# jinhojsk515/spmm

Measured on AMD Instinct MI355X. Metric: pretrain molecules/sec, higher is better.
Workload: dtype bf16; 1 GPU; SPMM pretrain step, text 12 layers (fusion at 6) + PV 6 layers, H=768, 12 heads, queue 36864, train mode (dropout 0.1), fwd+bwd+clip+AdamW+EMA; global_batch=128, seq_len=128, parallelism=dp1, schedule=eager launches on three HIP streams, packed text rows

## Files before the change

### include/spmm_hip.h

```cpp
#ifndef SPMM_HIP_H
#define SPMM_HIP_H

#include <stdint.h>

#ifdef __HIPCC__
#include <hip/hip_runtime.h>
typedef hipStream_t spmm_stream_t;
#else
typedef void* spmm_stream_t;
#endif

#ifdef __cplusplus
extern "C" {
#endif

int spmm_version(void);
const char* spmm_last_error(void);

#define SPMM_EPI_BF16 0
#define SPMM_EPI_GELU 1
#define SPMM_EPI_F32 2
#define SPMM_EPI_F32_ATOMIC 3
#define SPMM_EPI_GELU_GRAD 4
#define SPMM_EPI_F32_ACC 5
#define SPMM_EPI_GELU_DERIV 6
#define SPMM_EPI_MUL 7

#define SPMM_GEMM_AUTO 0
#define SPMM_GEMM_K128 1
#define SPMM_GEMM_K256x128 2
#define SPMM_GEMM_K256 3
#define SPMM_GEMM_K128PC 5
#define SPMM_GEMM_K256P8 8
#define SPMM_GEMM_K256P8_TILES 9
#define SPMM_GEMM_AUTO_TILES 16
int spmm_gemm_nt(const void* A, long lda, const void* W, long ldw, int M, int N, int K, int splits, const float* bias,
                 const float* div_ptr, float alpha, const void* R, long ldr, const void* G, long ldg, void* C, long ldc,
                 void* C2, long ldc2, int epi, float* colsum, int kernel, const int* M_dev, spmm_stream_t stream);
long spmm_gemm_tn_workspace_bytes(int M, int N, int K, int splits);
int spmm_gemm_tn_splits(int M, int N, int K, int kernel);
int spmm_gemm_tn(const void* A, long lda, const void* B, long ldb, int M, int N, int K, int splits, float alpha, float* C,
                 long ldc, float* workspace, int kernel, const int* M_dev, spmm_stream_t stream);
int spmm_gemm_tn_reduce(const float* ws, int ns, int N, int K, float* C, long ldc, spmm_stream_t stream);
int spmm_colsum_bf16(const void* x, long ld, int R, int C, float* out, const int* R_dev, spmm_stream_t stream);

int spmm_attn_fwd(const void* Q, long ldq, const void* K, long ldk, const void* V, long ldv, const int* kmask,
                  const int* kv_seq, const int* q_row0, const int* q_len, const int* kv_row0, const int* kv_len, void* O,
                  long ldo, float* LSE, int nseq, int nH, int Lq, int Lkv, int causal_from, int is_cross, float dropout_p,
                  const uint64_t* seed_ptr, uint64_t seed_salt, int q_off, int kv_off, spmm_stream_t stream);
int spmm_attn_bwd(const void* Q, long ldq, const void* K, long ldk, const void* V, long ldv, const int* kmask,
                  const int* kv_seq, const int* q_row0, const int* q_len, const int* kv_row0, const int* kv_len,
                  const void* O, long ldo, const float* LSE, const void* dO, long lddo, void* dQ,
                  long lddq, void* dK, long lddk, void* dV, long lddv, int nseq, int nH, int Lq, int Lkv, int causal_from,
                  int is_cross, float dropout_p, const uint64_t* seed_ptr, uint64_t seed_salt, int q_off, int kv_off, int d_mode,
                  float* Dbuf, spmm_stream_t stream);

int spmm_xattn_supported(int H, int nH, int Lq, int Lkv);
int spmm_xattn_pack_wo(const void* W, long ldw, void* out, int H, spmm_stream_t stream);
int spmm_xattn_fwd(const void* Q, long ldq, const void* K, long ldk, const void* V, long ldv, const int* kmask,
                   const int* kv_seq, const int* q_row0, const int* q_len, const int* kv_row0, const int* kv_len,
                   const void* WoF, const float* bo, const void* R, long ldr, const float* gamma, const float* beta, float eps,
                   void* Y, long ldy, void* Z, long ldz, float* mean, float* rstd, void* CTX, long ldc, float* LSE,
                   int nseq, int nH, int Lq, int Lkv, float attn_dropout_p, uint64_t salt_a, float hidden_dropout_p,
                   uint64_t salt_h, const uint64_t* seed_ptr, long row_base, spmm_stream_t stream);
int spmm_segment_sum_bf16(const void* src, const int* start, const int* list, void* out, int U, long W, spmm_stream_t stream);

int spmm_ln_fwd(const void* x, const void* res, const float* gamma, const float* beta, void* y, void* zout, float* mean,
                float* rstd, long rows, int H, float eps, float dropout_p, const uint64_t* seed_ptr, uint64_t salt,
                const int* rows_dev, spmm_stream_t stream);
int spmm_ln_fwd_r32(const void* x, const float* res32, const float* gamma, const float* beta, void* y, float* y32, void* zout,
                    float* mean, float* rstd, long rows, int H, float eps, float dropout_p, const uint64_t* seed_ptr,
                    uint64_t salt, spmm_stream_t stream);
int spmm_ln_bwd(const void* dy, const void* dy2, const void* z, const float* mean, const float* rstd, const float* gamma,
                void* dz, void* dx, float* dgamma, float* dbeta, long rows, int H, float dropout_p,
                const uint64_t* seed_ptr, uint64_t salt, int drop_on_dy, float* dxsum, const int* rows_dev,
                const float* beta_from_y, spmm_stream_t stream);

int spmm_embed_step_ln_fwd(const int* ids, int pos_index, const int* pos_ptr, const float* word, const float* pos, const float* type0,
                           const float* gamma, const float* beta, void* y, long rows, int H, float eps, spmm_stream_t stream);

int spmm_decode_attn(const void* q, long ldq, const void* K, const void* V, long seq_stride, long tok_stride, long head_stride, const int* anc,
                     int anc_ld, int kv_div, int group, void* out, long ldo, int R, int nH, int Lkv, float scale,
                     const int* t_ptr, const void* knew, const void* vnew, long ldn, const int* rowmap, spmm_stream_t stream);

int spmm_decode_xattn(const void* q, long ldq, const void* K, const void* V, long ldkv, const int* kv_seq, const int* kv_row0,
                      const int* kv_len, int group, void* out, long ldo, int R, int nH, int Lkv_max, float scale, spmm_stream_t stream);

int spmm_beam_step(const float* logits, long ldl, int N, int k, int V, int Lmax, int F, int t, const int* t_ptr, int t_off,
                   int* tokens, float* cur_p, float* fin_p, int* fin_len, int* fin_tok, int* fin_n, unsigned char* done,
                   int* anc, int anc_ld, int* ids_out, int* parent_out, int* n_done, const int* mol, const int* rowmap,
                   spmm_stream_t stream);

int spmm_beam_step_until(const float* logits, long ldl, int N, int k, int V, int Lmax, int F, int t, const int* t_ptr, int t_off,
                         int* tokens, float* cur_p, float* fin_p, int* fin_len, int* fin_tok, int* fin_n, unsigned char* done,
                         int* anc, int anc_ld, int* ids_out, int* parent_out, int* n_done, const int* mol, const int* rowmap,
                         int need, spmm_stream_t stream);

int spmm_beam_step_sampled(const float* logits, long ldl, int N, int k, int V, int Lmax, int F, int t, const int* t_ptr, int t_off,
                           int* tokens, float* cur_p, float* fin_p, int* fin_len, int* fin_tok, int* fin_n, unsigned char* done,
                           int* anc, int anc_ld, int* ids_out, int* parent_out, int* n_done, const int* mol, const int* rowmap,
                           const float* noise, long ldn, spmm_stream_t stream);

int spmm_gumbel_noise(const uint64_t* seed_ptr, uint64_t salt, int N, int k, int V, int Lmax, int t, const int* t_ptr, int t_off,
                      const int* mol, long mol_base, float* out, long ldo, spmm_stream_t stream);

int spmm_logit_warp(const float* lc, const float* lu, long ld, int R, int V, float w, float temperature, int top_k, float top_p,
                    int min_keep, float* out, long ldo, spmm_stream_t stream);

#define SPMM_SYNTAX_MASKED (-1e30f)
int spmm_smiles_mask(float* logits, float* logits2, long ld, int R, int V, const int* tokens, long tok_ld, int hist_rows, int k,
                     const int* mol, int Lmax, int t, const int* t_ptr, int t_off, int t_last, const int* table, int* state_out,
                     spmm_stream_t stream);

int spmm_kv_prefill(const void* K, const void* V, long ld, long src_rows, const int* row0, const int* len, const int* dst_row, int E,
                    void* Kc, void* Vc, int R, int nH, int Lmax, spmm_stream_t stream);

int spmm_embed_ln_fwd(int mode, const int* ids, const float* word, const float* pos, const float* type0, const float* pv_x,
                      const float* pv_mask, const float* pv_w, const float* pv_b, const float* pv_cls,
                      const float* pv_masktok, int src_mod, const float* gamma, const float* beta, void* y, void* zout,
                      float* mean, float* rstd, long nseq, int L, int H, float eps, float dropout_p,
                      const uint64_t* seed_ptr, uint64_t salt, spmm_stream_t stream);
int spmm_embed_bwd(int mode, const void* dz, const int* ids, const float* pv_x, const float* pv_mask, int src_mod,
                   float* dword, float* dpos, float* dtype0, float* d_w, float* d_b, float* d_cls, float* d_masktok,
                   long nseq, int L, int H, spmm_stream_t stream);

int spmm_transpose_bf16(const void* in, long ldi, void* out, long ldo, int R, int C, int Rpad, float* colsum,
                        spmm_stream_t stream);
int spmm_cast_transpose(const float* in, void* out, void* outT, int R, int C, spmm_stream_t stream);
long spmm_cast_transpose_desc_bytes(void);
int spmm_cast_transpose_multi(const void* descs_dev, int ndesc, int total_tiles, spmm_stream_t stream);
int spmm_cast_f32_bf16(const float* in, void* out, long n, spmm_stream_t stream);
int spmm_cast_bf16_f32(const void* in, float* out, long n, spmm_stream_t stream);
int spmm_acc_rows(float* dst, long ldd, const void* src, long lds, const long* idx, long rows, int H, int atomic,
                  spmm_stream_t stream);
int spmm_gather_rows(void* dst, const void* src, const long* idx, long rows, int H, spmm_stream_t stream);

int spmm_gather_rows2(void* dst, const void* srcA, const void* srcB, const long* idx, long rows, int H, spmm_stream_t stream);
int spmm_add_rows_bf16(void* dst, const long* idx, const void* src, long rows, int H, spmm_stream_t stream);
int spmm_zero_bytes(void* p, long nbytes, spmm_stream_t stream);
int spmm_zero_rows(void* p, long rows, long row_bytes, long stride_bytes, spmm_stream_t stream);
int spmm_gelu_bwd(const void* dz, const void* pre, void* out, long n, spmm_stream_t stream);
int spmm_pack_plan(const int* mask, int B, int Lt, int M, int* lens32, int* row0_32, long* row0_64, long* rows, long* gidx2,
                   long* gidx4, long* inv, long* idx_m, int* bad, spmm_stream_t stream);
int spmm_fusion_plan(const long* neg, const int* lens32, const int* row0_32, int B, int Lt, int Lp, int M,
                     long* idx6, long* neg_rows, long* idx_top, int* small32, spmm_stream_t stream);

int spmm_l2norm_fwd(const float* x, long ldx, float* y, float* nrm, void* a3, void* w3, void* yT, long ldt, int rows, int E,
                    spmm_stream_t stream);
int spmm_l2norm_bwd(const float* dy, const float* y, const float* nrm, const float* gscale, void* dx, int rows, int E,
                    spmm_stream_t stream);
int spmm_ita_rows(const float* S, const float* SM, long ldj, int nrows, int B, int J, const float* alpha_ptr,
                  const float* temp_ptr, void* dS, long ldd, int Jpad, float* losses, int loss_slot, float* dtemp,
                  int* nan_flag, spmm_stream_t stream);
int spmm_sample_neg(const float* S, long ldj, int B, const long* forced, const uint64_t* seed_ptr, uint64_t salt, long* out,
                    long out_offset, spmm_stream_t stream);
int spmm_lm_loss(const float* logits, const float* logits_m, long ldl, const int* ids, long nseq, int L, int V,
                 const float* alpha_ptr, int* n_nonpad_ws, const float* gscale, void* dlogits, long ldd, int Vpad,
                 float* losses, int loss_slot, spmm_stream_t stream);
int spmm_s2s_loss(const float* logits, long ldl, const int* ids, const long* row_of, long rows, long nseq, int L, int V,
                  int* n_label_ws, const float* gscale, void* dlogits, long ldd, int Vpad, float* losses, int loss_slot,
                  spmm_stream_t stream);
int spmm_lm_score(const void* y, long ldy, const void* Wd, long ldw, const float* bias, const int* ids, const long* row_of, long rows,
                  long nseq, int L, int V, int H, const int* seq_row0, const int* seq_len, float* tok_lp, float* seq_lp, int* seq_n,
                  spmm_stream_t stream);
int spmm_itm_head(const void* xa, long stride_a, const void* xb, long stride_b, int H, const float* W, const float* bias,
                  int n, int B, const float* gscale, float* losses, int loss_slot, float* logits_out, void* dxa, void* dxb,
                  float* dW, float* db, int do_bwd, int x_is_f32, spmm_stream_t stream);
int spmm_task_head(const void* A, long lda, int B, int W, const float* W2, const float* b2, int C, int kind, const void* target,
                   const float* gscale, float* logits, float* loss, void* dA, long ldda, float* dW2, float* db2, int do_bwd,
                   spmm_stream_t stream);
int spmm_s2p_append(const void* y, long ldy, const float* w3, const float* b3, const float* pe_w, const float* pe_b, const float* pos,
                    const float* type0, const float* gamma, const float* beta, float eps, float* pred, long ldp, void* xcache,
                    long rows, int H, int n_props, int i, spmm_stream_t stream);
int spmm_mpm_head(const void* h, int Lp, int H, const float* w, const float* bias, const float* target, const float* mask,
                  int B, int* n_keep_ws, const float* gscale, float* losses, int loss_slot, float* pred_out, void* dh,
                  float* dw, float* db, int do_bwd, int x_is_f32, spmm_stream_t stream);
int spmm_rows_linear(const void* x, int x_is_bf16, long ldx, const float* W, const float* bias, float* out, long ldo, long rows,
                     int N, int K, int act, spmm_stream_t stream);
long spmm_sim_topk_workspace_bytes(int Q, long n, int k);
int spmm_sim_topk(const float* q, long ldq, const float* f, long ldf, long base, int Q, long n, int E, int k, float* scores, long* index,
                  int merge, const float* cut_scores, const long* cut_index, void* workspace, long workspace_bytes, spmm_stream_t stream);
int spmm_enqueue(const float* feats, int n, int E, float* queue, int Q, void* w3, void* qT, long ldt, int Bloc, long* ptr,
                 int advance, const int* skip_flag, spmm_stream_t stream);
int spmm_queue_shadow(const float* queue, int E, int Q, void* w3, void* qT, long ldt, int Bloc, spmm_stream_t stream);
int spmm_clamp_scalar(float* p, float lo, float hi, spmm_stream_t stream);

long spmm_adam_scalars_bytes(void);
long spmm_grad_sqnorm_workspace_bytes(void);
int spmm_grad_sqnorm(const float* g, long n, float* out_zeroed, float* workspace, spmm_stream_t stream);
int spmm_adamw_step(float* p, const float* g, float* m, float* v, void* bf16_shadow, long n, const float* lr_ptr,
                    float beta1, float beta2, float eps, float weight_decay, const float* normsq, float max_norm, int* step,
                    const int* nan_flag, void* scalars_ws, spmm_stream_t stream);
int spmm_ema_update(float* pm, const float* p, void* bf16_shadow, long n, float momentum, spmm_stream_t stream);
int spmm_axpy_scalar(float* dst, const float* src, const float* scale_ptr, float scale, int n, spmm_stream_t stream);

#ifdef __cplusplus
}
#endif
#endif
```

### spmm_amd/csrc/gemm.hip

```cpp
#include "common.h"
#include "../../include/spmm_hip.h"

namespace {

constexpr int BM = 128, BN = 128, BK = 64;
constexpr int TILE_BYTES = BM * BK * 2;
constexpr int STAGE_BYTES = 2 * TILE_BYTES;

enum Epi { EPI_BF16 = 0, EPI_GELU = 1, EPI_F32 = 2, EPI_F32_ATOMIC = 3, EPI_GELU_GRAD = 4, EPI_F32_ACC = 5, EPI_GELU_DERIV = 6, EPI_MUL = 7 };
constexpr bool epi_is_bf16(int e) { return e == EPI_BF16 || e == EPI_GELU || e == EPI_GELU_GRAD || e == EPI_GELU_DERIV || e == EPI_MUL; }

struct GemmP {
  const bf16* A; long lda;
  const bf16* W; long ldw;
  int M, N, K;
  int ksplit;
  const float* bias;
  const float* div_ptr;
  float alpha;
  const bf16* R; long ldr;
  const bf16* G; long ldg;
  void* C; long ldc;
  bf16* C2; long ldc2;
  float* colsum;
  int order;
  const int* M_ptr;
};

#define GEMM_DYN_M(P)                                          \
  do {                                                         \
    if ((P).M_ptr) {                                           \
      const int m_ = *(P).M_ptr;                               \
      (P).M = m_ < (P).M ? (m_ > 0 ? m_ : 1) : (P).M;          \
    }                                                          \
  } while (0)

__device__ __forceinline__ void stage_tile_dma(const bf16* __restrict__ src, long ld, int row0, int nrows, int k0,
                                               char* lds_tile, int tid) {
#pragma unroll
  for (int c = 0; c < 4; ++c) {
    const int id = c * 256 + tid;
    const int row = id >> 3, ps = id & 7;
    const int ls = ps ^ ((row >> 1) & 7);
    int grow = row0 + row;
    grow = grow < nrows ? grow : nrows - 1;
    const bf16* g = src + (long)grow * ld + k0 + ls * 8;
    const int wave_base = __builtin_amdgcn_readfirstlane((c * 256 + (tid & ~63)) * 16);
    __builtin_amdgcn_global_load_lds((const GLOBAL_AS void*)g, (LDS_AS void*)(lds_tile + wave_base), 16, 0, 0);
  }
}

template <int EPI>
__device__ __forceinline__ void epi_convert(const GemmP& p, f32x16 (&acc)[2][2], char* t0, char* t1, int n_base, int lane) {
  float scale = p.alpha;
  if (p.div_ptr) scale /= *p.div_ptr;
#pragma unroll
  for (int ni = 0; ni < 2; ++ni)
#pragma unroll
    for (int mi = 0; mi < 2; ++mi) {
      const int row = mi * 32 + (lane & 31);
#pragma unroll
      for (int g = 0; g < 4; ++g) {
        const int col = ni * 32 + 8 * g + 4 * (lane >> 5);
        float v[4];
#pragma unroll
        for (int j = 0; j < 4; ++j) v[j] = acc[ni][mi][g * 4 + j] * scale;
        if (p.bias) {
          const int n = n_base + col;
          if (n < p.N) {
            const f32x4 b = *(const f32x4*)(p.bias + n);
#pragma unroll
            for (int j = 0; j < 4; ++j) v[j] += b[j];
          }
        }
        const int off = row * 128 + ((((col >> 3) ^ (row & 7)) << 4) | ((col & 4) << 1));
        if constexpr (EPI == EPI_GELU) {
          if (p.C2) *(bf16x4*)(t1 + off) = to_bf16x4(v[0], v[1], v[2], v[3]);
          *(bf16x4*)(t0 + off) = to_bf16x4(gelu_erf(v[0]), gelu_erf(v[1]), gelu_erf(v[2]), gelu_erf(v[3]));
        } else if constexpr (EPI == EPI_GELU_DERIV) {
          float gv[4], dv[4];
#pragma unroll
          for (int j = 0; j < 4; ++j) gelu_erf_both(v[j], gv[j], dv[j]);
          if (p.C2) *(bf16x4*)(t1 + off) = to_bf16x4(dv[0], dv[1], dv[2], dv[3]);
          *(bf16x4*)(t0 + off) = to_bf16x4(gv[0], gv[1], gv[2], gv[3]);
        } else {
          *(bf16x4*)(t0 + off) = to_bf16x4(v[0], v[1], v[2], v[3]);
        }
      }
    }
}

template <int EPI>
__device__ __forceinline__ void epi_store(const GemmP& p, const char* t0, const char* t1, int m_base, int n_base, int lane,
                                          float* cs_carry = nullptr, bool flush = true) {
  bf16x8 rr[8], gg[8];
  if (p.R || EPI == EPI_GELU_GRAD || EPI == EPI_MUL) {
#pragma unroll
    for (int it = 0; it < 8; ++it) {
      const int row = it * 8 + (lane >> 3), c16 = lane & 7;
      const int m = m_base + row, n = n_base + c16 * 8;
#pragma unroll
      for (int e = 0; e < 8; ++e) { rr[it][e] = (bf16)0.f; gg[it][e] = (bf16)0.f; }
      if (m >= p.M || n >= p.N) continue;
      const bool full = n + 8 <= p.N;
      if (p.R) {
        if (full) rr[it] = *(const bf16x8*)(p.R + (long)m * p.ldr + n);
        else { const bf16x4 h4 = *(const bf16x4*)(p.R + (long)m * p.ldr + n); rr[it][0] = h4[0]; rr[it][1] = h4[1]; rr[it][2] = h4[2]; rr[it][3] = h4[3]; }
      }
      if constexpr (EPI == EPI_GELU_GRAD || EPI == EPI_MUL) {
        if (full) gg[it] = *(const bf16x8*)(p.G + (long)m * p.ldg + n);
// ... 65 lines not shown

template <int EPI>
__device__ __forceinline__ void epilogue_bf16(const GemmP& p, f32x16 (&acc)[2][2], char* wtile, int m_base, int n_base, int lane,
                                              float* cs_carry = nullptr, bool flush = true) {
  epi_convert<EPI>(p, acc, wtile, wtile + 8192, n_base, lane);
  epi_store<EPI>(p, wtile, wtile + 8192, m_base, n_base, lane, cs_carry, flush);
}

template <int EPI>
__device__ __forceinline__ void tile128_out(const GemmP& p, f32x16 (&acc)[2][2], char* smem, int wave, int m0, int n0, int wm, int wn, int lane) {
  if constexpr (epi_is_bf16(EPI)) {
    epilogue_bf16<EPI>(p, acc, smem + wave * 16384, m0 + wm * 64, n0 + wn * 64, lane);
    return;
  }
  float scale = p.alpha;
  if (p.div_ptr) scale /= *p.div_ptr;
#pragma unroll
  for (int ni = 0; ni < 2; ++ni)
#pragma unroll
    for (int mi = 0; mi < 2; ++mi) {
      const int m = m0 + wm * 64 + mi * 32 + (lane & 31);
      if (m >= p.M) continue;
#pragma unroll
      for (int g = 0; g < 4; ++g) {
        const int n = n0 + wn * 64 + ni * 32 + 8 * g + 4 * (lane >> 5);
        if (n >= p.N) continue;
        float v[4];
#pragma unroll
        for (int j = 0; j < 4; ++j) v[j] = acc[ni][mi][g * 4 + j] * scale;
        if (p.bias && (EPI != EPI_F32_ATOMIC || blockIdx.z == 0)) {
          const f32x4 b = *(const f32x4*)(p.bias + n);
#pragma unroll
          for (int j = 0; j < 4; ++j) v[j] += b[j];
        }
        if (p.R && (EPI != EPI_F32_ATOMIC || blockIdx.z == 0)) {
          const bf16x4 r = *(const bf16x4*)(p.R + (long)m * p.ldr + n);
#pragma unroll
          for (int j = 0; j < 4; ++j) v[j] += (float)r[j];
        }
        if constexpr (EPI == EPI_BF16) {
          *(bf16x4*)((bf16*)p.C + (long)m * p.ldc + n) = to_bf16x4(v[0], v[1], v[2], v[3]);
        } else if constexpr (EPI == EPI_GELU) {
          *(bf16x4*)(p.C2 + (long)m * p.ldc2 + n) = to_bf16x4(v[0], v[1], v[2], v[3]);
          *(bf16x4*)((bf16*)p.C + (long)m * p.ldc + n) =
              to_bf16x4(gelu_erf(v[0]), gelu_erf(v[1]), gelu_erf(v[2]), gelu_erf(v[3]));
        } else if constexpr (EPI == EPI_GELU_GRAD) {
          const bf16x4 x = *(const bf16x4*)(p.G + (long)m * p.ldg + n);
          *(bf16x4*)((bf16*)p.C + (long)m * p.ldc + n) =
              to_bf16x4(v[0] * gelu_erf_grad((float)x[0]), v[1] * gelu_erf_grad((float)x[1]),
                        v[2] * gelu_erf_grad((float)x[2]), v[3] * gelu_erf_grad((float)x[3]));
        } else if constexpr (EPI == EPI_F32) {
          f32x4 o = {v[0], v[1], v[2], v[3]};
          *(f32x4*)((float*)p.C + (long)m * p.ldc + n) = o;
        } else if constexpr (EPI == EPI_F32_ACC) {
          f32x4* dst = (f32x4*)((float*)p.C + (long)m * p.ldc + n);
          f32x4 o = *dst;
          o[0] += v[0]; o[1] += v[1]; o[2] += v[2]; o[3] += v[3];
          *dst = o;
        } else {
          float* dst = (float*)p.C + (long)m * p.ldc + n;
#pragma unroll
          for (int j = 0; j < 4; ++j) atomicAdd(dst + j, v[j]);
        }
      }
    }
}

template <int EPI>
__global__ __launch_bounds__(256) void gemm_nt_kernel(GemmP p) {
  __shared__ __attribute__((aligned(16))) char smem[2 * STAGE_BYTES];
  const int tid = threadIdx.x, lane = tid & 63, wave = tid >> 6;
  const int wm = wave >> 1, wn = wave & 1;

  GEMM_DYN_M(p);
  const int ntm = (p.M + BM - 1) / BM, ntn = (p.N + BN - 1) / BN, nt = ntm * ntn;
  int t;
  {
    const int b = blockIdx.x, q = nt >> 3, r = nt & 7, xcd = b & 7, i = b >> 3;
    if (i >= (xcd < r ? q + 1 : q)) return;
    t = (xcd < r ? xcd * (q + 1) : r * (q + 1) + (xcd - r) * q) + i;
  }
  const int tile_m = t / ntn, tile_n = t % ntn;
  const int m0 = tile_m * BM, n0 = tile_n * BN;
  const int kbeg = blockIdx.z * p.ksplit;
  const int kend = min(p.K, kbeg + p.ksplit);
  const int nk = (kend - kbeg) / BK;

  f32x16 acc[2][2];
#pragma unroll
  for (int i = 0; i < 2; ++i)
#pragma unroll
    for (int j = 0; j < 2; ++j)
#pragma unroll
      for (int r = 0; r < 16; ++r) acc[i][j][r] = 0.f;

  if (nk > 0) {
    stage_tile_dma(p.A, p.lda, m0, p.M, kbeg, smem, tid);
    stage_tile_dma(p.W, p.ldw, n0, p.N, kbeg, smem + TILE_BYTES, tid);
  }
  for (int kt = 0; kt < nk; ++kt) {
    __syncthreads();
    char* cur = smem + (kt & 1) * STAGE_BYTES;
    char* nxt = smem + ((kt + 1) & 1) * STAGE_BYTES;
    if (kt + 1 < nk) {
      stage_tile_dma(p.A, p.lda, m0, p.M, kbeg + (kt + 1) * BK, nxt, tid);
      stage_tile_dma(p.W, p.ldw, n0, p.N, kbeg + (kt + 1) * BK, nxt + TILE_BYTES, tid);
    }
    const char* As = cur;
    const char* Ws = cur + TILE_BYTES;
#pragma unroll
    for (int kk = 0; kk < 4; ++kk) {
      const int s = kk * 2 + (lane >> 5);
      bf16x8 af[2], wf[2];
#pragma unroll
      for (int i = 0; i < 2; ++i) {
        const int ar = wm * 64 + i * 32 + (lane & 31);
        af[i] = *(const bf16x8*)(As + ar * 128 + ((s ^ ((ar >> 1) & 7)) << 4));
        const int wr = wn * 64 + i * 32 + (lane & 31);
        wf[i] = *(const bf16x8*)(Ws + wr * 128 + ((s ^ ((wr >> 1) & 7)) << 4));
      }
#pragma unroll
      for (int ni = 0; ni < 2; ++ni)
#pragma unroll
        for (int mi = 0; mi < 2; ++mi)
          acc[ni][mi] = __builtin_amdgcn_mfma_f32_32x32x16_bf16(wf[ni], af[mi], acc[ni][mi], 0, 0, 0);
    }
  }

  if constexpr (epi_is_bf16(EPI)) __syncthreads();
  tile128_out<EPI>(p, acc, smem, wave, m0, n0, wm, wn, lane);
}

#ifndef PC_AUTO
#define PC_AUTO 1
#endif
constexpr int PC_STAGES = 4;
constexpr int PC_LDS = PC_STAGES * STAGE_BYTES;
#ifndef PC_LOADERS
#define PC_LOADERS 4
#endif
constexpr int PC_LT = PC_LOADERS * 64;
constexpr int PC_NC = 1024 / PC_LT;
constexpr int PC_THREADS = 256 + PC_LT;

template <int EPI>
__global__ __launch_bounds__(PC_THREADS) void gemm_nt_pc_kernel(GemmP p) {
  extern __shared__ __attribute__((aligned(16))) char smem_pc[];
  const int tid = threadIdx.x, lane = tid & 63;
  const int wave = __builtin_amdgcn_readfirstlane(tid >> 6);
  GEMM_DYN_M(p);
  const int ntm = (p.M + BM - 1) / BM, ntn = (p.N + BN - 1) / BN, nt = ntm * ntn;
  int t;
  {
    const int b = blockIdx.x, q = nt >> 3, r = nt & 7, xcd = b & 7, i = b >> 3;
    if (i >= (xcd < r ? q + 1 : q)) return;
    t = (xcd < r ? xcd * (q + 1) : r * (q + 1) + (xcd - r) * q) + i;
  }
  const int tile_m = t / ntn, tile_n = t % ntn;
  const int m0 = tile_m * BM, n0 = tile_n * BN;
  const int kbeg = blockIdx.z * p.ksplit;
  const int kend = min(p.K, kbeg + p.ksplit);
  const int nk = (kend - kbeg) / BK;

  if (wave >= 4) {
    const int ltid = tid - 256;
    uint32_t offA[PC_NC], offW[PC_NC], dst[PC_NC];
#pragma unroll
    for (int c = 0; c < PC_NC; ++c) {
      const int id = c * PC_LT + ltid;
      const int row = id >> 3, ps = id & 7;
      const int ls = ps ^ ((row >> 1) & 7);
      int ga = m0 + row, gw = n0 + row;
      ga = ga < p.M ? ga : p.M - 1;
      gw = gw < p.N ? gw : p.N - 1;
      offA[c] = (uint32_t)ga * (uint32_t)(p.lda * 2) + (uint32_t)(ls * 16);
      offW[c] = (uint32_t)gw * (uint32_t)(p.ldw * 2) + (uint32_t)(ls * 16);
      dst[c] = (uint32_t)((c * PC_LT + (ltid & ~63)) * 16);
    }
    const uint32_t lds0 = (uint32_t)(uintptr_t)(LDS_AS char*)smem_pc;
    const char* gA = (const char*)p.A + (size_t)kbeg * 2;
    const char* gW = (const char*)p.W + (size_t)kbeg * 2;
#define PC_DMA(VOFF, SBASE, LDSDST)                                                                                          \
    asm volatile("s_mov_b32 m0, %2\n\ts_nop 0\n\tglobal_load_lds_dwordx4 %0, %1" ::"v"(VOFF), "s"(SBASE), "s"(LDSDST) : "memory", "m0")
#define PC_STAGE(KT)                                                                                                         \
    do {                                                                                                                     \
      const uint32_t st_ = lds0 + (uint32_t)(((KT) % PC_STAGES) * STAGE_BYTES);                                              \
      const char* a_ = gA + (size_t)(KT) * (BK * 2);                                                                         \
      const char* w_ = gW + (size_t)(KT) * (BK * 2);                                                                         \
      _Pragma("unroll") for (int c = 0; c < PC_NC; ++c) {                                                                    \
        const uint32_t d_ = __builtin_amdgcn_readfirstlane(st_ + dst[c]);                                                    \
        PC_DMA(offA[c], a_, d_);                                                                                             \
      }                                                                                                                      \
      _Pragma("unroll") for (int c = 0; c < PC_NC; ++c) {                                                                    \
        const uint32_t d_ = __builtin_amdgcn_readfirstlane(st_ + (uint32_t)TILE_BYTES + dst[c]);                             \
        PC_DMA(offW[c], w_, d_);                                                                                             \
      }                                                                                                                      \
    } while (0)
#define PC_WAIT(NEWER)                                                                                                       \
    do {                                                                                                                     \
      if ((NEWER) >= 3) asm volatile("s_waitcnt vmcnt(%0)" ::"n"(6 * PC_NC) : "memory");                                     \
      else if ((NEWER) == 2) asm volatile("s_waitcnt vmcnt(%0)" ::"n"(4 * PC_NC) : "memory");                                \
      else if ((NEWER) == 1) asm volatile("s_waitcnt vmcnt(%0)" ::"n"(2 * PC_NC) : "memory");                                \
      else asm volatile("s_waitcnt vmcnt(0)" ::: "memory");                                                                  \
    } while (0)
    constexpr int AHEAD = PC_STAGES - 1;
    const int pre = nk < AHEAD ? nk : AHEAD;
    for (int k = 0; k < pre; ++k) PC_STAGE(k);
    PC_WAIT(pre - 1);
    __builtin_amdgcn_s_barrier();
    for (int kt = 0; kt < nk; ++kt) {
      if (kt + AHEAD < nk) PC_STAGE(kt + AHEAD);
      const int last = kt + AHEAD < nk ? kt + AHEAD : nk - 1;
      PC_WAIT(last - (kt + 1));
      __builtin_amdgcn_s_barrier();
    }
#undef PC_DMA
#undef PC_STAGE
#undef PC_WAIT
    return;
  }

  const int wm = wave >> 1, wn = wave & 1;
  f32x16 acc[2][2];
#pragma unroll
  for (int i = 0; i < 2; ++i)
#pragma unroll
    for (int j = 0; j < 2; ++j)
#pragma unroll
      for (int r = 0; r < 16; ++r) acc[i][j][r] = 0.f;
  int aoff[2], woff[2];
#pragma unroll
  for (int i = 0; i < 2; ++i) {
    aoff[i] = (wm * 64 + i * 32 + (lane & 31)) * 128;
    woff[i] = TILE_BYTES + (wn * 64 + i * 32 + (lane & 31)) * 128;
  }
  const int sw0 = ((wm * 64 + (lane & 31)) >> 1) & 7, sw1 = ((wn * 64 + (lane & 31)) >> 1) & 7;
  const int hi = lane >> 5;
#define PC_FRAGS(KK, BUF)                                                                                          \
  do {                                                                                                             \
    const int sa_ = (((KK) * 2 + hi) ^ sw0) << 4, sw_ = (((KK) * 2 + hi) ^ sw1) << 4;                              \
    _Pragma("unroll") for (int i = 0; i < 2; ++i) {                                                                \
      af[BUF][i] = *(const bf16x8*)(st + aoff[i] + sa_);                                                           \
      wf[BUF][i] = *(const bf16x8*)(st + woff[i] + sw_);                                                           \
    }                                                                                                              \
  } while (0)
  __builtin_amdgcn_s_barrier();
  for (int kt = 0; kt < nk; ++kt) {
    const char* st = smem_pc + (kt % PC_STAGES) * STAGE_BYTES;
    bf16x8 af[2][2], wf[2][2];
    PC_FRAGS(0, 0);
#pragma unroll
    for (int kk = 0; kk < 4; ++kk) {
      if (kk < 3) PC_FRAGS(kk + 1, (kk + 1) & 1);
#pragma unroll
      for (int ni = 0; ni < 2; ++ni)
#pragma unroll
        for (int mi = 0; mi < 2; ++mi)
          acc[ni][mi] = __builtin_amdgcn_mfma_f32_32x32x16_bf16(wf[kk & 1][ni], af[kk & 1][mi], acc[ni][mi], 0, 0, 0);
    }
    __builtin_amdgcn_s_barrier();
  }
#undef PC_FRAGS
  tile128_out<EPI>(p, acc, smem_pc, wave, m0, n0, wm, wn, lane);
}

constexpr int BM2 = 256;
constexpr int A2_BYTES = BM2 * BK * 2;
constexpr int STAGE2_BYTES = A2_BYTES + TILE_BYTES;
constexpr int LDS2_BYTES = 3 * STAGE2_BYTES;

__device__ __forceinline__ void stage2_dma(const bf16* __restrict__ src, long ld, int row0, int nrows, int k0, char* lds_tile, int tid,
                                           int nchunks_per_thread) {
  for (int c = 0; c < nchunks_per_thread; ++c) {
    const int id = c * 512 + tid;
    const int row = id >> 3, ps = id & 7;
    const int ls = ps ^ ((row >> 1) & 7);
    int grow = row0 + row;
    grow = grow < nrows ? grow : nrows - 1;
    const bf16* g = src + (long)grow * ld + k0 + ls * 8;
    const int wave_base = __builtin_amdgcn_readfirstlane((c * 512 + (tid & ~63)) * 16);
    __builtin_amdgcn_global_load_lds((const GLOBAL_AS void*)g, (LDS_AS void*)(lds_tile + wave_base), 16, 0, 0);
  }
}

template <int EPI>
__global__ __launch_bounds__(512) void gemm_nt_v2_kernel(GemmP p) {
  extern __shared__ __attribute__((aligned(16))) char smem2[];
  const int tid = threadIdx.x, lane = tid & 63, wave = tid >> 6;
  const int wm = wave >> 1, wn = wave & 1;
  GEMM_DYN_M(p);
  const int ntm = (p.M + BM2 - 1) / BM2, ntn = (p.N + BN - 1) / BN, nt = ntm * ntn;
  int t;
  {
    const int b = blockIdx.x, q = nt >> 3, r = nt & 7, xcd = b & 7, i = b >> 3;
    if (i >= (xcd < r ? q + 1 : q)) return;
    t = (xcd < r ? xcd * (q + 1) : r * (q + 1) + (xcd - r) * q) + i;
  }
  const int tile_m = t / ntn, tile_n = t % ntn;
  const int m0 = tile_m * BM2, n0 = tile_n * BN;
  const int nk = p.K / BK;

  f32x16 acc[2][2];
#pragma unroll
  for (int i = 0; i < 2; ++i)
#pragma unroll
    for (int j = 0; j < 2; ++j)
#pragma unroll
      for (int r = 0; r < 16; ++r) acc[i][j][r] = 0.f;

#define STAGE2(kt_)                                                                           \
  do {                                                                                        \
    char* b_ = smem2 + ((kt_) % 3) * STAGE2_BYTES;                                            \
    stage2_dma(p.A, p.lda, m0, p.M, (kt_) * BK, b_, tid, 4);                                  \
    stage2_dma(p.W, p.ldw, n0, p.N, (kt_) * BK, b_ + A2_BYTES, tid, 2);                       \
  } while (0)

  STAGE2(0);
  if (nk > 1) STAGE2(1);
  for (int kt = 0; kt < nk; ++kt) {
    if (kt + 1 < nk) asm volatile("s_waitcnt vmcnt(6)" ::: "memory");
    else asm volatile("s_waitcnt vmcnt(0)" ::: "memory");
    __builtin_amdgcn_s_barrier();
    if (kt + 2 < nk) STAGE2(kt + 2);
    const char* As = smem2 + (kt % 3) * STAGE2_BYTES;
    const char* Ws = As + A2_BYTES;
    const int ar0 = wm * 64 + (lane & 31), wr0 = wn * 64 + (lane & 31);
#pragma unroll
    for (int kk = 0; kk < 4; ++kk) {
      const int s = kk * 2 + (lane >> 5);
      bf16x8 af[2], wf[2];
#pragma unroll
      for (int i = 0; i < 2; ++i) {
        const int ar = ar0 + i * 32, wr = wr0 + i * 32;
        af[i] = *(const bf16x8*)(As + ar * 128 + ((s ^ ((ar >> 1) & 7)) << 4));
        wf[i] = *(const bf16x8*)(Ws + wr * 128 + ((s ^ ((wr >> 1) & 7)) << 4));
      }
#pragma unroll
      for (int ni = 0; ni < 2; ++ni)
#pragma unroll
        for (int mi = 0; mi < 2; ++mi)
          acc[ni][mi] = __builtin_amdgcn_mfma_f32_32x32x16_bf16(wf[ni], af[mi], acc[ni][mi], 0, 0, 0);
    }
  }
#undef STAGE2

  if constexpr (epi_is_bf16(EPI)) {
    __builtin_amdgcn_s_barrier();
    epilogue_bf16<EPI>(p, acc, smem2 + wave * 16384, m0 + wm * 64, n0 + wn * 64, lane);
    return;
  }
  float scale = p.alpha;
  if (p.div_ptr) scale /= *p.div_ptr;
#pragma unroll
  for (int ni = 0; ni < 2; ++ni)
#pragma unroll
    for (int mi = 0; mi < 2; ++mi) {
      const int m = m0 + wm * 64 + mi * 32 + (lane & 31);
      if (m >= p.M) continue;
#pragma unroll
      for (int g = 0; g < 4; ++g) {
        const int n = n0 + wn * 64 + ni * 32 + 8 * g + 4 * (lane >> 5);
        if (n >= p.N) continue;
        float v[4];
#pragma unroll
        for (int j = 0; j < 4; ++j) v[j] = acc[ni][mi][g * 4 + j] * scale;
        if (p.bias) {
          const f32x4 b = *(const f32x4*)(p.bias + n);
#pragma unroll
          for (int j = 0; j < 4; ++j) v[j] += b[j];
        }
        if (p.R) {
          const bf16x4 r = *(const bf16x4*)(p.R + (long)m * p.ldr + n);
#pragma unroll
          for (int j = 0; j < 4; ++j) v[j] += (float)r[j];
        }
        if constexpr (EPI == EPI_BF16) {
          *(bf16x4*)((bf16*)p.C + (long)m * p.ldc + n) = to_bf16x4(v[0], v[1], v[2], v[3]);
        } else if constexpr (EPI == EPI_GELU) {
          *(bf16x4*)(p.C2 + (long)m * p.ldc2 + n) = to_bf16x4(v[0], v[1], v[2], v[3]);
          *(bf16x4*)((bf16*)p.C + (long)m * p.ldc + n) =
              to_bf16x4(gelu_erf(v[0]), gelu_erf(v[1]), gelu_erf(v[2]), gelu_erf(v[3]));
        } else if constexpr (EPI == EPI_GELU_GRAD) {
          const bf16x4 x = *(const bf16x4*)(p.G + (long)m * p.ldg + n);
          *(bf16x4*)((bf16*)p.C + (long)m * p.ldc + n) =
              to_bf16x4(v[0] * gelu_erf_grad((float)x[0]), v[1] * gelu_erf_grad((float)x[1]),
                        v[2] * gelu_erf_grad((float)x[2]), v[3] * gelu_erf_grad((float)x[3]));
        } else if constexpr (EPI == EPI_F32) {
          f32x4 o = {v[0], v[1], v[2], v[3]};
          *(f32x4*)((float*)p.C + (long)m * p.ldc + n) = o;
        } else {
          f32x4* dst = (f32x4*)((float*)p.C + (long)m * p.ldc + n);
          f32x4 o = *dst;
          o[0] += v[0]; o[1] += v[1]; o[2] += v[2]; o[3] += v[3];
          *dst = o;
        }
      }
    }
}

__device__ __forceinline__ void tile_of(int t, int ntm, int ntn, int order, int& tm, int& tn) {
  if (order == 1) { tn = t / ntm; tm = t - tn * ntm; return; }
  if (order == 2) {
    const int gn = (ntn % 4 == 0) ? 4 : (ntn % 3 == 0 ? 3 : (ntn % 2 == 0 ? 2 : 1));
    const int sr = t / (8 * ntn);
    const int rows = min(8, ntm - sr * 8);
    const int r = t - sr * 8 * ntn;
    const int nb = r / (rows * gn), rr = r - nb * rows * gn;
    tm = sr * 8 + rr % rows;
    tn = nb * gn + rr / rows;
    return;
  }
  if (order >= 3 && ntn >= 8) {
    const int ng = order == 3 ? 2 : 4, base = ntn / ng, rem = ntn - base * ng;
    int c0 = 0, u = t;
#pragma unroll
    for (int g = 0; g < 4; ++g) {
      if (g >= ng) break;
      const int cg = base + (g < rem ? 1 : 0), sz = ntm * cg;
      if (u < sz || g == ng - 1) { tm = u / cg; tn = c0 + (u - tm * cg); return; }
      u -= sz; c0 += cg;
    }
  }
  tm = t / ntn; tn = t - tm * ntn;
}

constexpr int BM3 = 256, BN3 = 256;
constexpr int T3_BYTES = 256 * BK * 2;
constexpr int STAGE3_BYTES = 2 * T3_BYTES;
constexpr int LDS3_BYTES = 2 * STAGE3_BYTES;

template <int EPI>
__global__ __launch_bounds__(512) void gemm_nt_v3_kernel(GemmP p) {
  extern __shared__ __attribute__((aligned(16))) char smem3[];
  const int tid = threadIdx.x, lane = tid & 63, wave = tid >> 6;
  const int wm = wave >> 2, wn = wave & 3;
  GEMM_DYN_M(p);
  const int ntm = (p.M + BM3 - 1) / BM3, ntn = (p.N + BN3 - 1) / BN3, nt = ntm * ntn;
  int t;
  {
    const int b = blockIdx.x, q = nt >> 3, r = nt & 7, xcd = b & 7, i = b >> 3;
    if (i >= (xcd < r ? q + 1 : q)) return;
    t = (xcd < r ? xcd * (q + 1) : r * (q + 1) + (xcd - r) * q) + i;
  }
  int tile_m, tile_n;
  tile_of(t, ntm, ntn, p.order, tile_m, tile_n);
  const int m0 = tile_m * BM3, n0 = tile_n * BN3;
  const int nk = p.K / BK;

  f32x16 acc[2][2][2];
#pragma unroll
  for (int h = 0; h < 2; ++h)
#pragma unroll
    for (int i = 0; i < 2; ++i)
#pragma unroll
      for (int j = 0; j < 2; ++j)
#pragma unroll
        for (int r = 0; r < 16; ++r) acc[h][i][j][r] = 0.f;

#define STAGE3(kt_)                                                                           \
  do {                                                                                        \
    char* b_ = smem3 + ((kt_) & 1) * STAGE3_BYTES;                                            \
    stage2_dma(p.A, p.lda, m0, p.M, (kt_) * BK, b_, tid, 4);                                  \
    stage2_dma(p.W, p.ldw, n0, p.N, (kt_) * BK, b_ + T3_BYTES, tid, 4);                       \
  } while (0)

  STAGE3(0);
  for (int kt = 0; kt < nk; ++kt) {
    __syncthreads();
    if (kt + 1 < nk) STAGE3(kt + 1);
    const char* As = smem3 + (kt & 1) * STAGE3_BYTES;
    const char* Ws = As + T3_BYTES;
#pragma unroll
    for (int kk = 0; kk < 4; ++kk) {
      const int s = kk * 2 + (lane >> 5);
      bf16x8 af[4], wf[2];
#pragma unroll
      for (int i = 0; i < 4; ++i) {
        const int ar = wm * 128 + i * 32 + (lane & 31);
        af[i] = *(const bf16x8*)(As + ar * 128 + ((s ^ ((ar >> 1) & 7)) << 4));
      }
#pragma unroll
      for (int i = 0; i < 2; ++i) {
        const int wr = wn * 64 + i * 32 + (lane & 31);
        wf[i] = *(const bf16x8*)(Ws + wr * 128 + ((s ^ ((wr >> 1) & 7)) << 4));
      }
#pragma unroll
      for (int h = 0; h < 2; ++h)
#pragma unroll
        for (int ni = 0; ni < 2; ++ni)
#pragma unroll
          for (int mi = 0; mi < 2; ++mi)
            acc[h][ni][mi] = __builtin_amdgcn_mfma_f32_32x32x16_bf16(wf[ni], af[h * 2 + mi], acc[h][ni][mi], 0, 0, 0);
    }
  }
#undef STAGE3
  __syncthreads();
  char* wt = smem3 + wave * 16384;
  float cs_carry[8] = {0.f, 0.f, 0.f, 0.f, 0.f, 0.f, 0.f, 0.f};
#pragma unroll
  for (int h = 0; h < 2; ++h)
    epilogue_bf16<EPI>(p, acc[h], wt, m0 + wm * 128 + h * 64, n0 + wn * 64, lane, cs_carry, h == 1);
}

constexpr int P8_HT = 128 * BK * 2;
constexpr int P8_BUF = 4 * P8_HT;
constexpr int P8_LDS = 2 * P8_BUF;
constexpr int P8_XLDS = 8 * 4096;

template <int OFF>
__device__ __forceinline__ void p8_dsr(bf16x8& d, uint32_t addr) {
  asm volatile("ds_read_b128 %0, %1 offset:%2" : "=v"(d) : "v"(addr), "n"(OFF) : "memory");
}

struct P8Out { uint32_t d[4]; };
__device__ __forceinline__ uint32_t p8_pack2(float a, float b) {
  typedef __bf16 bf16x2 __attribute__((ext_vector_type(2)));
  bf16x2 v; v[0] = (bf16)a; v[1] = (bf16)b;
  return __builtin_bit_cast(uint32_t, v);
}
__device__ __forceinline__ float p8_lo(uint32_t w) { return __builtin_bit_cast(float, w << 16); }
__device__ __forceinline__ float p8_hi(uint32_t w) { return __builtin_bit_cast(float, w & 0xffff0000u); }
typedef uint32_t u32x2 __attribute__((ext_vector_type(2)));
typedef uint32_t u32x4 __attribute__((ext_vector_type(4)));
template <int OFF>
__device__ __forceinline__ void p8_dsw64(uint32_t addr, uint32_t a, uint32_t b) {
  u32x2 v = {a, b};
  asm volatile("ds_write_b64 %0, %1 offset:%2" :: "v"(addr), "v"(v), "n"(OFF) : "memory");
}
template <int OFF>
// ... 121 lines not shown
        if (p.colsum) {
#pragma unroll
          for (int d = 0; d < 4; ++d) {
            if (ok1) { cs[2 * d] += p8_lo(o1[d]); cs[2 * d + 1] += p8_hi(o1[d]); }
            if (ok2) { cs[2 * d] += p8_lo(o2[d]); cs[2 * d + 1] += p8_hi(o2[d]); }
          }
        }
      }
#ifdef P8_NOSTORE
      if (p.M < 0) {
#endif
#ifdef P8_STORE_POLICY
      if (ok1) asm volatile("global_store_dwordx4 %0, %1, off " P8_STORE_POLICY :: "v"(cp + (long)blk * 16 * p.ldc), "v"(o1) : "memory");
      if (ok2) asm volatile("global_store_dwordx4 %0, %1, off " P8_STORE_POLICY :: "v"(cp + (long)blk * 16 * p.ldc + 8 * p.ldc), "v"(o2) : "memory");
#else
      if (ok1) *(u32x4*)(cp + (long)blk * 16 * p.ldc) = o1;
      if (ok2) *(u32x4*)(cp + (long)blk * 16 * p.ldc + 8 * p.ldc) = o2;
#endif
#ifdef P8_NOSTORE
      }
#endif
      hook(blk);
      if constexpr (HAS_EX && EPI == EPI_GELU_GRAD) {
        if (blk == 3) { P8_LOAD_EX(1); }
      } else if constexpr (HAS_EX) {
        if (h == 0) {
#pragma unroll
          for (int i_ = 2 * mi; i_ < 2 * mi + 2; ++i_) {
            long r_ = row0 + 64 + i_ * 8;
            if (!INTERIOR) r_ = r_ < p.M ? r_ : p.M - 1;
            P8_EX_LOAD1(i_, r_);
          }
        }
      }
    }
#undef P8_LOAD_EX
#undef P8_EX_LOAD1
  if constexpr (!GELU2) {
    if (p.colsum) {
#pragma unroll
      for (int e = 0; e < 8; ++e) {
        float t = cs[e];
        t += __shfl_xor(t, 8, 64);
        t += __shfl_xor(t, 16, 64);
        t += __shfl_xor(t, 32, 64);
        cs[e] = t;
      }
      if (lane < 8 && n_ok) {
#pragma unroll
        for (int e = 0; e < 8; ++e) atomicAdd(p.colsum + n + e, cs[e]);
      }
    }
  }
}

template <int EPI>
__global__ __launch_bounds__(512) void gemm_nt_p8_kernel(GemmP p) {
  extern __shared__ __attribute__((aligned(16))) char smem8[];
  const int tid = threadIdx.x, lane = tid & 63;
  const int wave = __builtin_amdgcn_readfirstlane(tid >> 6);
  const int wr = wave >> 2, wc = wave & 3;
  GEMM_DYN_M(p);
  const int ntm = (p.M + BM3 - 1) / BM3, ntn = (p.N + BN3 - 1) / BN3, nt = ntm * ntn;
  if ((int)blockIdx.x >= nt) return;
  const int nk = p.K / BK;

  f32x4 acc[2][4][4];
#define P8_ZERO()                                                              \
  _Pragma("unroll") for (int h_ = 0; h_ < 2; ++h_)                             \
  _Pragma("unroll") for (int i_ = 0; i_ < 4; ++i_)                             \
  _Pragma("unroll") for (int j_ = 0; j_ < 4; ++j_) acc[h_][i_][j_] = f32x4{0.f, 0.f, 0.f, 0.f}
  P8_ZERO();

  uint32_t offA[2][2], offW[2][2];
  const uint32_t ls16 = (uint32_t)(((tid & 7) ^ ((tid >> 4) & 7)) * 16);
  int m0, n0;
#define P8_TILE(VB)                                                                                           \
  do {                                                                                                        \
    const int b_ = (VB), q_ = nt >> 3, r_ = nt & 7, xcd_ = b_ & 7, i_ = b_ >> 3;                              \
    const int t_ = (xcd_ < r_ ? xcd_ * (q_ + 1) : r_ * (q_ + 1) + (xcd_ - r_) * q_) + i_;                     \
    int tm_, tn_;                                                                                             \
    tile_of(t_, ntm, ntn, p.order, tm_, tn_);                                                                 \
    m0 = tm_ * BM3; n0 = tn_ * BN3;                                                                           \
    _Pragma("unroll") for (int h_ = 0; h_ < 2; ++h_)                                                          \
    _Pragma("unroll") for (int j_ = 0; j_ < 2; ++j_) {                                                        \
      int row_ = m0 + j_ * 128 + h_ * 64 + (tid >> 3);                                                        \
      row_ = row_ < p.M ? row_ : p.M - 1;                     \
      offA[h_][j_] = (uint32_t)row_ * (uint32_t)(p.lda * 2) + ls16;                                                      \
      int col_ = n0 + (j_ * 2 + (tid >> 8)) * 64 + h_ * 32 + ((tid >> 3) & 31);                               \
      col_ = col_ < p.N ? col_ : p.N - 1;                                                                     \
      offW[h_][j_] = (uint32_t)col_ * (uint32_t)(p.ldw * 2) + ls16;                                                      \
    }                                                                                                         \
  } while (0)
  const char* gA = (const char*)p.A;
  const char* gW = (const char*)p.W;
  const uint32_t lds0 = (uint32_t)(uintptr_t)(LDS_AS char*)smem8;
#define P8_STG(GB, O, SLOT)                                                                                               \
  do {                                                                                                                    \
    const uint32_t d_ = lds0 + (SLOT) + wave * 1024;                                                                      \
    asm volatile("s_mov_b32 m0, %2\n\ts_nop 0\n\tglobal_load_lds_dwordx4 %0, %1" :: "v"((O)[0]), "s"(GB), "s"(d_) : "memory", "m0");          \
    asm volatile("s_mov_b32 m0, %2\n\ts_nop 0\n\tglobal_load_lds_dwordx4 %0, %1" :: "v"((O)[1]), "s"(GB), "s"(d_ + 8192) : "memory", "m0");   \
  } while (0)
#define P8_STG_A(H, BUF, KT) P8_STG((const char*)(gA + (size_t)(KT) * (BK * 2)), offA[H], (BUF) * P8_BUF + (H) * P8_HT)
#define P8_STG_W(H, BUF, KT) P8_STG((const char*)(gW + (size_t)(KT) * (BK * 2)), offW[H], (BUF) * P8_BUF + (2 + (H)) * P8_HT)
#define P8_PROLOGUE()                                                                        \
  do {                                                                                       \
    P8_STG_A(0, 0, 0); P8_STG_W(0, 0, 0); P8_STG_W(1, 0, 0); P8_STG_A(1, 0, 0);              \
    P8_STG_W(0, 1, 1); P8_STG_A(0, 1, 1); P8_STG_W(1, 1, 1);                                 \
  } while (0)

  uint32_t aad[2][2], wad[2][2];
  {
    const uint32_t sw = (uint32_t)((lane >> 1) & 7), r16 = (uint32_t)(lane & 15), q = (uint32_t)(lane >> 4);
#pragma unroll
    for (int kk = 0; kk < 2; ++kk) {
      const uint32_t slot = ((((uint32_t)kk * 4 + q) ^ sw) << 4);
      aad[0][kk] = lds0 + ((uint32_t)wr * 64 + r16) * 128 + slot;
      wad[0][kk] = lds0 + 2 * P8_HT + ((uint32_t)wc * 32 + r16) * 128 + slot;
      aad[1][kk] = aad[0][kk] + P8_BUF;
      wad[1][kk] = wad[0][kk] + P8_BUF;
    }
  }
  bf16x8 fa[4][2], fw0[2][2], fw1[2][2];
#define P8_RD_A(BUF, H)                                                                       \
  do {                                                                                        \
    p8_dsr<(H) * P8_HT + 0 * 2048>(fa[0][0], aad[BUF][0]);                                    \
    p8_dsr<(H) * P8_HT + 1 * 2048>(fa[1][0], aad[BUF][0]);                                    \
    p8_dsr<(H) * P8_HT + 2 * 2048>(fa[2][0], aad[BUF][0]);                                    \
    p8_dsr<(H) * P8_HT + 3 * 2048>(fa[3][0], aad[BUF][0]);                                    \
    p8_dsr<(H) * P8_HT + 0 * 2048>(fa[0][1], aad[BUF][1]);                                    \
    p8_dsr<(H) * P8_HT + 1 * 2048>(fa[1][1], aad[BUF][1]);                                    \
    p8_dsr<(H) * P8_HT + 2 * 2048>(fa[2][1], aad[BUF][1]);                                    \
    p8_dsr<(H) * P8_HT + 3 * 2048>(fa[3][1], aad[BUF][1]);                                    \
  } while (0)
#define P8_RD_W(BUF, H, FW)                                                                   \
  do {                                                                                        \
    p8_dsr<(H) * P8_HT + 0 * 2048>(FW[0][0], wad[BUF][0]);                                    \
    p8_dsr<(H) * P8_HT + 1 * 2048>(FW[1][0], wad[BUF][0]);                                    \
    p8_dsr<(H) * P8_HT + 0 * 2048>(FW[0][1], wad[BUF][1]);                                    \
    p8_dsr<(H) * P8_HT + 1 * 2048>(FW[1][1], wad[BUF][1]);                                    \
  } while (0)
#define P8_MM(H, NH, FW)                                                                                        \
  do {                                                                                                          \
    _Pragma("unroll") for (int kk_ = 0; kk_ < 2; ++kk_)                                                         \
    _Pragma("unroll") for (int mi_ = 0; mi_ < 4; ++mi_)                                                         \
    _Pragma("unroll") for (int ni_ = 0; ni_ < 2; ++ni_)                                                         \
      acc[H][mi_][(NH) * 2 + ni_] =                                                                             \
          __builtin_amdgcn_mfma_f32_16x16x32_bf16(FW[ni_][kk_], fa[mi_][kk_], acc[H][mi_][(NH) * 2 + ni_], 0, 0, 0); \
  } while (0)
#define P8_BAR() __builtin_amdgcn_s_barrier()
#define P8_SB() __builtin_amdgcn_sched_barrier(0)
#define P8_LGKM0() asm volatile("s_waitcnt lgkmcnt(0)" ::: "memory")
#define P8_COMPUTE(H, NH, FW)                    \
  do {                                           \
    P8_BAR();                                    \
    P8_LGKM0();                                  \
    P8_SB();                                     \
    __builtin_amdgcn_s_setprio(1);               \
    P8_MM(H, NH, FW);                            \
    __builtin_amdgcn_s_setprio(0);               \
    P8_SB();                                     \
    P8_BAR();                                    \
    P8_SB();                                     \
  } while (0)

#ifdef P8_PROFILE
  unsigned long long* prof = (unsigned long long*)p.colsum + (size_t)blockIdx.x * 16 * 8;
  p.colsum = nullptr;
  int prof_i = 0;
#define P8_STAMP(K) do { if (prof && tid == 0 && prof_i < 16) prof[prof_i * 8 + (K)] = __builtin_readcyclecounter(); } while (0)
#else
#define P8_STAMP(K) do { } while (0)
#endif
  int vb = blockIdx.x;
  bool pre = false;
  P8_TILE(vb);
  P8_PROLOGUE();
  asm volatile("s_waitcnt vmcnt(6)" ::: "memory");
  P8_BAR();
  P8_SB();
  if (wr == 1) P8_BAR();
  for (;;) {
    P8_STAMP(0);
    const int cm0 = m0, cn0 = n0;
    const int vbn = vb + (int)gridDim.x;
    const bool has_next = vbn < nt;
    const bool pre_next = has_next && cm0 + BM3 <= p.M && cn0 + BN3 <= p.N;
    for (int kt = 0; kt < nk; kt += 2) {
      const bool last = kt + 2 >= nk;
      const bool more = !last || has_next;
      int kn = kt + 2;
      P8_RD_W(0, 0, fw0); P8_SB(); P8_RD_A(0, 0);
      if (!(pre && kt == 0)) P8_STG_A(1, 1, kt + 1);
      asm volatile("s_waitcnt lgkmcnt(8)" ::: "memory");
      P8_COMPUTE(0, 0, fw0);
      if (last && has_next) { P8_TILE(vbn); kn = 0; }
      P8_RD_W(0, 1, fw1);
      if (more) P8_STG_W(0, 0, kn);
      P8_COMPUTE(0, 1, fw1);
      P8_RD_A(0, 1);
      if (more) P8_STG_A(0, 0, kn);
      P8_COMPUTE(1, 1, fw1);
      if (more) {
        P8_STG_W(1, 0, kn);
        if (pre && kt == 0) asm volatile("s_waitcnt vmcnt(22)" ::: "memory");
        else asm volatile("s_waitcnt vmcnt(6)" ::: "memory");
      } else {
        asm volatile("s_waitcnt vmcnt(0)" ::: "memory");
      }
      P8_COMPUTE(1, 0, fw0);
      P8_RD_W(1, 0, fw0); P8_SB(); P8_RD_A(1, 0);
      if (more) P8_STG_A(1, 0, kn);
      asm volatile("s_waitcnt lgkmcnt(8)" ::: "memory");
      P8_COMPUTE(0, 0, fw0);
      P8_RD_W(1, 1, fw1);
      if (more) P8_STG_W(0, 1, kn + 1);
      P8_COMPUTE(0, 1, fw1);
      P8_RD_A(1, 1);
      if (more) P8_STG_A(0, 1, kn + 1);
      P8_COMPUTE(1, 1, fw1);
      if (more) {
        P8_STG_W(1, 1, kn + 1);
        if (last && pre_next) {
          P8_STG_A(1, 1, kn + 1);
          asm volatile("s_waitcnt vmcnt(8)" ::: "memory");
        } else {
          asm volatile("s_waitcnt vmcnt(6)" ::: "memory");
        }
      }
      P8_COMPUTE(1, 0, fw0);
    }
    P8_STAMP(2);

    if (wr == 0) P8_BAR();
    P8_SB();
    {
      int lane_e = lane;
      asm volatile("" : "+v"(lane_e));
      GemmP q = p;
      asm volatile("" : "+s"(q.C), "+s"(q.ldc), "+s"(q.C2), "+s"(q.ldc2));
      asm volatile("" : "+s"(q.R), "+s"(q.ldr), "+s"(q.G), "+s"(q.ldg));
      asm volatile("" : "+s"(q.bias), "+s"(q.colsum), "+s"(q.div_ptr), "+s"(q.alpha), "+s"(q.M), "+s"(q.N));
      auto hook = [](int) {};
      const uint32_t xb = lds0 + P8_LDS + wave * 4096;
      const int mb = cm0 + wr * 128, nb = cn0 + wc * 64;
      const bool interior = cm0 + BM3 <= q.M && cn0 + BN3 <= q.N;
      if constexpr (EPI == EPI_GELU_GRAD || EPI == EPI_MUL) {
        if (interior) p8_epilogue_blocks<EPI, true, true>(q, acc, xb, mb, nb, lane_e, hook);
        else p8_epilogue_blocks<EPI, false, true>(q, acc, xb, mb, nb, lane_e, hook);
      } else if (EPI == EPI_BF16 && q.R != nullptr) {
        if (interior) p8_epilogue_blocks<EPI, true, true>(q, acc, xb, mb, nb, lane_e, hook);
        else p8_epilogue_blocks<EPI, false, true>(q, acc, xb, mb, nb, lane_e, hook);
      } else {
        if (interior) p8_epilogue_blocks<EPI, true, false>(q, acc, xb, mb, nb, lane_e, hook);
        else p8_epilogue_blocks<EPI, false, false>(q, acc, xb, mb, nb, lane_e, hook);
      }
    }
    P8_SB();
    if (wr == 1) P8_BAR();
    P8_STAMP(4);
#ifdef P8_PROFILE
    ++prof_i;
#endif
    if (!has_next) break;
    vb = vbn;
    pre = pre_next;
    P8_SB();
  }
  if (wr == 0) P8_BAR();
#undef P8_ZERO
#undef P8_STAMP
#undef P8_TILE
#undef P8_PROLOGUE
#undef P8_STG
#undef P8_STG_A
#undef P8_STG_W
#undef P8_RD_A
#undef P8_RD_W
#undef P8_MM
#undef P8_COMPUTE
#undef P8_BAR
#undef P8_SB
#undef P8_LGKM0
}

template <typename K>
int raise_lds(K kernel, int bytes, const char* what) {
  hipError_t e = hipFuncSetAttribute((const void*)kernel, hipFuncAttributeMaxDynamicSharedMemorySize, bytes);
  if (e != hipSuccess) {
    spmm_set_error("spmm_gemm_nt: cannot raise the dynamic LDS of %s to %d: %s", what, bytes, hipGetErrorString(e));
    return SPMM_ERR_LAUNCH;
  }
  return SPMM_OK;
}

template <int EPI>
int launch_p8_one(const GemmP& p, hipStream_t st, bool persist) {
  static const int rc = raise_lds(gemm_nt_p8_kernel<EPI>, P8_LDS + P8_XLDS, "the 8-phase kernel");
  if (rc != SPMM_OK) return rc;
  const int nt = ((p.M + BM3 - 1) / BM3) * ((p.N + BN3 - 1) / BN3);
  static const int ncu = [] { int dev = 0, n = 0; (void)hipGetDevice(&dev); (void)hipDeviceGetAttribute(&n, hipDeviceAttributeMultiprocessorCount, dev); return n > 0 ? n & ~7 : 256; }();
  dim3 grid(persist && nt > ncu ? ncu : nt);
  hipLaunchKernelGGL((gemm_nt_p8_kernel<EPI>), grid, dim3(512), P8_LDS + P8_XLDS, st, p);
  return SPMM_OK;
}
int launch_p8(int epi, const GemmP& p, hipStream_t st, bool persist) {
  switch (epi) {
    case EPI_BF16: return launch_p8_one<EPI_BF16>(p, st, persist);
    case EPI_GELU: return launch_p8_one<EPI_GELU>(p, st, persist);
    case EPI_GELU_GRAD: return launch_p8_one<EPI_GELU_GRAD>(p, st, persist);
    case EPI_GELU_DERIV: return launch_p8_one<EPI_GELU_DERIV>(p, st, persist);
    case EPI_MUL: return launch_p8_one<EPI_MUL>(p, st, persist);
    default: return -1;
  }
}

template <int EPI>
int launch_v3_one(const GemmP& p, hipStream_t st) {
  static const int rc = raise_lds(gemm_nt_v3_kernel<EPI>, LDS3_BYTES, "the 256x256 kernel");
  if (rc != SPMM_OK) return rc;
  dim3 grid(((p.M + BM3 - 1) / BM3) * ((p.N + BN3 - 1) / BN3));
  hipLaunchKernelGGL((gemm_nt_v3_kernel<EPI>), grid, dim3(512), LDS3_BYTES, st, p);
  return SPMM_OK;
}
int launch_v3(int epi, const GemmP& p, hipStream_t st) {
  switch (epi) {
    case EPI_BF16: return launch_v3_one<EPI_BF16>(p, st);
    case EPI_GELU: return launch_v3_one<EPI_GELU>(p, st);
    case EPI_GELU_GRAD: return launch_v3_one<EPI_GELU_GRAD>(p, st);
    case EPI_GELU_DERIV: return launch_v3_one<EPI_GELU_DERIV>(p, st);
    case EPI_MUL: return launch_v3_one<EPI_MUL>(p, st);
    default: return -1;
  }
}

template <int EPI>
int launch_v2_one(const GemmP& p, hipStream_t st) {
  static const int rc = raise_lds(gemm_nt_v2_kernel<EPI>, LDS2_BYTES, "the 256x128 kernel");
  if (rc != SPMM_OK) return rc;
  dim3 grid(((p.M + BM2 - 1) / BM2) * ((p.N + BN - 1) / BN));
  hipLaunchKernelGGL((gemm_nt_v2_kernel<EPI>), grid, dim3(512), LDS2_BYTES, st, p);
  return SPMM_OK;
}
int launch_v2(int epi, const GemmP& p, hipStream_t st) {
  switch (epi) {
    case EPI_BF16: return launch_v2_one<EPI_BF16>(p, st);
    case EPI_GELU: return launch_v2_one<EPI_GELU>(p, st);
    case EPI_F32: return launch_v2_one<EPI_F32>(p, st);
    case EPI_GELU_GRAD: return launch_v2_one<EPI_GELU_GRAD>(p, st);
    case EPI_GELU_DERIV: return launch_v2_one<EPI_GELU_DERIV>(p, st);
    case EPI_MUL: return launch_v2_one<EPI_MUL>(p, st);
    case EPI_F32_ACC: return launch_v2_one<EPI_F32_ACC>(p, st);
    default: return -1;
  }
}

template <typename K>
int pc_attr(K kernel) {
  static const hipError_t e = hipFuncSetAttribute((const void*)kernel, hipFuncAttributeMaxDynamicSharedMemorySize, PC_LDS);
  return e == hipSuccess ? 0 : 1;
}
#define PC_LAUNCH(E)                                                                                   \
  case E:                                                                                              \
    if (pc_attr(gemm_nt_pc_kernel<E>)) { spmm_set_error("spmm_gemm_nt: cannot raise the LDS limit of the loader/compute kernel"); return SPMM_ERR_LAUNCH; } \
    hipLaunchKernelGGL((gemm_nt_pc_kernel<E>), grid, dim3(PC_THREADS), PC_LDS, st, p);                        \
    break
int launch_pc(int epi, const GemmP& p, dim3 grid, hipStream_t st) {
  switch (epi) {
    PC_LAUNCH(EPI_BF16); PC_LAUNCH(EPI_GELU); PC_LAUNCH(EPI_F32); PC_LAUNCH(EPI_F32_ATOMIC); PC_LAUNCH(EPI_GELU_GRAD); PC_LAUNCH(EPI_F32_ACC);
    PC_LAUNCH(EPI_GELU_DERIV); PC_LAUNCH(EPI_MUL);
    default: return -1;
  }
  return 0;
}
#undef PC_LAUNCH

int launch_v1(int epi, const GemmP& p, dim3 grid, hipStream_t st) {
  switch (epi) {
    case EPI_BF16: hipLaunchKernelGGL((gemm_nt_kernel<EPI_BF16>), grid, dim3(256), 0, st, p); break;
    case EPI_GELU: hipLaunchKernelGGL((gemm_nt_kernel<EPI_GELU>), grid, dim3(256), 0, st, p); break;
    case EPI_F32: hipLaunchKernelGGL((gemm_nt_kernel<EPI_F32>), grid, dim3(256), 0, st, p); break;
    case EPI_F32_ATOMIC: hipLaunchKernelGGL((gemm_nt_kernel<EPI_F32_ATOMIC>), grid, dim3(256), 0, st, p); break;
    case EPI_GELU_GRAD: hipLaunchKernelGGL((gemm_nt_kernel<EPI_GELU_GRAD>), grid, dim3(256), 0, st, p); break;
    case EPI_F32_ACC: hipLaunchKernelGGL((gemm_nt_kernel<EPI_F32_ACC>), grid, dim3(256), 0, st, p); break;
    case EPI_GELU_DERIV: hipLaunchKernelGGL((gemm_nt_kernel<EPI_GELU_DERIV>), grid, dim3(256), 0, st, p); break;
    case EPI_MUL: hipLaunchKernelGGL((gemm_nt_kernel<EPI_MUL>), grid, dim3(256), 0, st, p); break;
    default: return -1;
  }
  return SPMM_OK;
}

inline bool is_bf16_epi(int epi) { return epi_is_bf16(epi); }
inline bool p8_ok(const GemmP& p, int epi) {
  return is_bf16_epi(epi) && p.K % 128 == 0 && p.N % 8 == 0 && (unsigned long)p.M * (unsigned long)p.lda * 2ul < (1ul << 32) &&
         (unsigned long)p.N * (unsigned long)p.ldw * 2ul < (1ul << 32);
}

int pick_tile(int M, int N, int epi) {
  const bool bf = is_bf16_epi(epi);
  if (M >= 6000) {
    const long t3 = (long)((M + 255) / 256) * ((N + 255) / 256);
    if (bf && t3 >= 96) return 3;
    return (epi != EPI_F32_ATOMIC) ? 2 : 1;
  }
  auto tiles = [&](int bm, int bn) { return (double)((M + bm - 1) / bm) * ((N + bn - 1) / bn); };
  auto fill = [](double t) { const double w = (double)(long)((t + 255) / 256); return t / (256.0 * w); };
  const double t3 = tiles(256, 256), t2 = tiles(256, 128), t1 = tiles(128, 128);
  const double s3 = bf ? 1.20 * fill(t3) : 0.0;
  const double s2 = (M >= 512 && epi != EPI_F32_ATOMIC) ? 0.85 * fill(t2) : 0.0;
  const double s1 = 0.80 * (t1 < 256 ? t1 / 256.0 : 1.0);
  if (s3 >= s2 && s3 >= s1) return 3;
  return s2 >= s1 ? 2 : 1;
}

}

extern "C" int spmm_gemm_nt(const void* A, long lda, const void* W, long ldw, int M, int N, int K, int splits,
                            const float* bias, const float* div_ptr, float alpha, const void* R, long ldr,
                            const void* G, long ldg, void* C, long ldc, void* C2, long ldc2, int epi, float* colsum,
                            int kernel, const int* M_dev, hipStream_t stream) {
  SPMM_CHECK_SHAPE(M > 0 && N > 0 && K > 0, "spmm_gemm_nt: empty problem M=%d N=%d K=%d", M, N, K);
  SPMM_CHECK_SHAPE(K % 64 == 0, "spmm_gemm_nt: K=%d must be a multiple of 64", K);
  SPMM_CHECK_SHAPE(N % 4 == 0, "spmm_gemm_nt: N=%d must be a multiple of 4", N);
  SPMM_CHECK_SHAPE(lda % 8 == 0 && ldw % 8 == 0, "spmm_gemm_nt: lda/ldw must be multiples of 8 elements");
  SPMM_CHECK_SHAPE(ldc % 4 == 0, "spmm_gemm_nt: ldc must be a multiple of 4");
  SPMM_CHECK_SHAPE(!is_bf16_epi(epi) || (ldc % 8 == 0 && (!R || ldr % 8 == 0) && (!G || ldg % 8 == 0) && (!C2 || ldc2 % 8 == 0) && (uintptr_t)C % 16 == 0),
                   "spmm_gemm_nt: bf16 outputs need 16-B aligned rows (ldc/ldr/ldg/ldc2 multiples of 8)");
  SPMM_CHECK_SHAPE(is_bf16_epi(epi) || !R || (ldr % 4 == 0 && (uintptr_t)R % 8 == 0),
                   "spmm_gemm_nt: R of an fp32-output epilogue is read 4 columns at a time (ldr a multiple of 4, R 8-B aligned)");
  SPMM_CHECK_SHAPE(((uintptr_t)A % 16 == 0) && ((uintptr_t)W % 16 == 0), "spmm_gemm_nt: A/W must be 16-B aligned");
  SPMM_CHECK_SHAPE(epi >= EPI_BF16 && epi <= EPI_MUL, "spmm_gemm_nt: unknown epilogue %d", epi);
  if (splits < 1) splits = 1;
  SPMM_CHECK_SHAPE(splits == 1 || epi == EPI_F32_ATOMIC, "spmm_gemm_nt: split-K needs the atomic epilogue");
  SPMM_CHECK_SHAPE((epi != EPI_GELU_GRAD && epi != EPI_MUL) || G != nullptr, "spmm_gemm_nt: the GELU-grad / multiply epilogues need G");
  SPMM_CHECK_SHAPE(colsum == nullptr || epi == EPI_BF16 || epi == EPI_GELU_GRAD || epi == EPI_MUL, "spmm_gemm_nt: colsum is only fused into the bf16 / GELU-grad / multiply epilogues");
  int ksplit = ((K / 64 + splits - 1) / splits) * 64;
  splits = (K + ksplit - 1) / ksplit;
  GemmP p;
  p.A = (const bf16*)A; p.lda = lda; p.W = (const bf16*)W; p.ldw = ldw;
  p.M = M; p.N = N; p.K = K; p.ksplit = ksplit; p.bias = bias; p.div_ptr = div_ptr; p.alpha = alpha;
  p.R = (const bf16*)R; p.ldr = ldr; p.G = (const bf16*)G; p.ldg = ldg; p.C = C; p.ldc = ldc;
  p.C2 = (bf16*)C2; p.ldc2 = ldc2; p.colsum = colsum;
  p.M_ptr = nullptr;
  p.order = K > 1024 ? 0 : 2;

  int k = kernel == SPMM_GEMM_AUTO_TILES ? 0 : kernel;
  if (k == 0) {
    const int tile = splits > 1 ? 1 : pick_tile(M, N, epi);
    k = tile == 3 ? (p8_ok(p, epi) ? (kernel == SPMM_GEMM_AUTO_TILES ? 9 : 8) : 3) : tile;
    if (k == 2 && (epi == EPI_F32_ATOMIC || M < 512)) k = 1;
  }
  const bool pc_fits = (unsigned long)p.M * (unsigned long)p.lda * 2ul < (1ul << 32) && (unsigned long)p.N * (unsigned long)p.ldw * 2ul < (1ul << 32);
  const long t128 = (long)((M + BM - 1) / BM) * ((N + BN - 1) / BN) * splits;
  if (k == 1 && kernel != 1 && pc_fits && PC_AUTO && t128 <= 256 && ksplit >= 4 * BK) k = 5;
  SPMM_CHECK_SHAPE(k == 1 || k == 2 || k == 3 || k == 5 || k == 8 || k == 9, "spmm_gemm_nt: unknown kernel selector %d", kernel);
  SPMM_CHECK_SHAPE(k != 5 || pc_fits, "spmm_gemm_nt: kernel 5 addresses its operands with 32-bit byte offsets (< 4 GiB each)");
  SPMM_CHECK_SHAPE((k != 8 && k != 9) || p8_ok(p, epi), "spmm_gemm_nt: the 8-phase kernel needs a bf16-output epilogue, K %% 128 == 0, N %% 8 == 0 and operands < 4 GiB");
  SPMM_CHECK_SHAPE(k != 3 || is_bf16_epi(epi), "spmm_gemm_nt: the 256x256 kernel has bf16-output epilogues only");
  SPMM_CHECK_SHAPE(k != 2 || epi != EPI_F32_ATOMIC, "spmm_gemm_nt: the 256x128 kernel has no atomic epilogue");
  SPMM_CHECK_SHAPE(k == 1 || k == 5 || splits == 1, "spmm_gemm_nt: split-K runs on the 128x128 kernels only");
  p.M_ptr = M_dev;
  int rc;
  if (k == 8 || k == 9) rc = launch_p8(epi, p, stream, k == 8);
  else if (k == 3) rc = launch_v3(epi, p, stream);
  else if (k == 2) rc = launch_v2(epi, p, stream);
  else if (k == 5) rc = launch_pc(epi, p, dim3(((M + BM - 1) / BM) * ((N + BN - 1) / BN), 1, splits), stream);
  else rc = launch_v1(epi, p, dim3(((M + BM - 1) / BM) * ((N + BN - 1) / BN), 1, splits), stream);
  if (rc > 0) return rc;
  if (rc < 0) { spmm_set_error("spmm_gemm_nt: epilogue %d is not built for kernel %d", epi, k); return SPMM_ERR_UNSUPPORTED; }
  SPMM_LAUNCH_CHECK("spmm_gemm_nt");
  return SPMM_OK;
}
```

### spmm_amd/csrc/rowops.hip

```cpp
#include "common.h"
#include <stdlib.h>
#include "../../include/spmm_hip.h"

namespace {

constexpr int MAXC = 4;

struct RowVec {
  float v[MAXC][4];
};

__device__ __forceinline__ void load_row_bf16(const bf16* __restrict__ p, int H, int lane, RowVec& r) {
#pragma unroll
  for (int i = 0; i < MAXC; ++i) {
    const int c = (lane + 64 * i) * 4;
    if (c < H) {
      const bf16x4 t = *(const bf16x4*)(p + c);
      r.v[i][0] = (float)t[0]; r.v[i][1] = (float)t[1]; r.v[i][2] = (float)t[2]; r.v[i][3] = (float)t[3];
    } else {
      r.v[i][0] = r.v[i][1] = r.v[i][2] = r.v[i][3] = 0.f;
    }
  }
}
__device__ __forceinline__ void store_row_bf16(bf16* __restrict__ p, int H, int lane, const RowVec& r) {
// ... 460 lines not shown
    float acc = 0.f, accw = 0.f, accb = 0.f, accm = 0.f;
    for (long s = s_beg; s < s_end; ++s) {
      const long row = s * p.L + l;
      const float g = (float)p.dz[row * p.H + c];
      acc += g;
      if (p.mode == 0) {
        const int id = p.ids[row];
        if (id != 0) atomicAdd(p.dword + (long)id * p.H + c, g);
      } else if (l > 0) {
        const long src = (s % p.src_mod) * (p.L - 1) + (l - 1);
        const float m = p.pv_mask[src];
        accw += g * (1.f - m) * p.pv_x[src];
        accb += g * (1.f - m);
        accm += g * m;
      }
    }
    atomicAdd(p.dpos + (long)l * p.H + c, acc);
    atomicAdd(p.dtype0 + c, acc);
    if (p.mode == 1) {
      if (l == 0) {
        atomicAdd(p.d_cls + c, acc);
      } else {
        atomicAdd(p.d_w + c, accw);
        atomicAdd(p.d_b + c, accb);
        atomicAdd(p.d_masktok + c, accm);
      }
    }
  }
}

__global__ __launch_bounds__(256) void transpose_bf16_kernel(const bf16* __restrict__ in, long ldi, bf16* __restrict__ out,
                                                             long ldo, int R, int C, int Rpad, float* __restrict__ colsum) {
  __shared__ bf16 tile[64][66];
  const int r0 = blockIdx.y * 64, c0 = blockIdx.x * 64;
  const int tx = threadIdx.x & 63, ty = threadIdx.x >> 6;
  float cs = 0.f;
#pragma unroll
  for (int i = 0; i < 16; ++i) {
    const int r = r0 + ty * 16 + i, c = c0 + tx;
    const bf16 v = (r < R && c < C) ? in[(long)r * ldi + c] : (bf16)0.f;
    tile[ty * 16 + i][tx] = v;
    cs += (float)v;
  }
  if (colsum) {
    __shared__ float part[4][64];
    part[ty][tx] = cs;
    __syncthreads();
    if (ty == 0 && c0 + tx < C) atomicAdd(colsum + c0 + tx, part[0][tx] + part[1][tx] + part[2][tx] + part[3][tx]);
  } else {
    __syncthreads();
  }
#pragma unroll
  for (int i = 0; i < 16; ++i) {
    const int c = c0 + ty * 16 + i, r = r0 + tx;
    if (c < C && r < Rpad) out[(long)c * ldo + r] = tile[tx][ty * 16 + i];
  }
}

__global__ __launch_bounds__(256) void cast_transpose_kernel(const float* __restrict__ in, bf16* __restrict__ out,
                                                             bf16* __restrict__ outT, int R, int C) {
  __shared__ bf16 tile[64][66];
  const int r0 = blockIdx.y * 64, c0 = blockIdx.x * 64;
  const int tx = threadIdx.x & 63, ty = threadIdx.x >> 6;
#pragma unroll
  for (int i = 0; i < 16; ++i) {
    const int r = r0 + ty * 16 + i, c = c0 + tx;
    bf16 v = (bf16)0.f;
    if (r < R && c < C) {
      v = (bf16)in[(long)r * C + c];
      if (out) out[(long)r * C + c] = v;
    }
    tile[ty * 16 + i][tx] = v;
  }
  __syncthreads();
  if (outT) {
#pragma unroll
    for (int i = 0; i < 16; ++i) {
      const int c = c0 + ty * 16 + i, r = r0 + tx;
      if (c < C && r < R) outT[(long)c * R + r] = tile[tx][ty * 16 + i];
    }
  }
}

struct CtDesc { const float* src; bf16* dstT; int R, C; int tile0, ntc; };
__global__ __launch_bounds__(256) void cast_transpose_multi_kernel(const CtDesc* __restrict__ descs, int ndesc) {
  __shared__ bf16 tile[64][66];
  int lo = 0, hi = ndesc - 1;
  while (lo < hi) {
    const int mid = (lo + hi + 1) >> 1;
    if (descs[mid].tile0 <= (int)blockIdx.x) lo = mid; else hi = mid - 1;
  }
  const CtDesc d = descs[lo];
  const int tt = blockIdx.x - d.tile0;
  const int r0 = (tt / d.ntc) * 64, c0 = (tt % d.ntc) * 64;
  const int tx = threadIdx.x & 63, ty = threadIdx.x >> 6;
#pragma unroll
  for (int i = 0; i < 16; ++i) {
    const int r = r0 + ty * 16 + i, c = c0 + tx;
    tile[ty * 16 + i][tx] = (r < d.R && c < d.C) ? (bf16)d.src[(long)r * d.C + c] : (bf16)0.f;
  }
  __syncthreads();
#pragma unroll
  for (int i = 0; i < 16; ++i) {
    const int c = c0 + ty * 16 + i, r = r0 + tx;
    if (c < d.C && r < d.R) d.dstT[(long)c * d.R + r] = tile[tx][ty * 16 + i];
  }
}

__global__ void cast_f32_bf16_kernel(const float* __restrict__ in, bf16* __restrict__ out, long n4) {
  for (long i = (long)blockIdx.x * blockDim.x + threadIdx.x; i < n4; i += (long)gridDim.x * blockDim.x) {
    const f32x4 v = *(const f32x4*)(in + i * 4);
    *(bf16x4*)(out + i * 4) = to_bf16x4(v[0], v[1], v[2], v[3]);
  }
}
__global__ void cast_bf16_f32_kernel(const bf16* __restrict__ in, float* __restrict__ out, long n4) {
  for (long i = (long)blockIdx.x * blockDim.x + threadIdx.x; i < n4; i += (long)gridDim.x * blockDim.x) {
    const bf16x4 v = *(const bf16x4*)(in + i * 4);
    f32x4 o = {(float)v[0], (float)v[1], (float)v[2], (float)v[3]};
    *(f32x4*)(out + i * 4) = o;
  }
}

__global__ void acc_rows_kernel(float* __restrict__ dst, long ldd, const bf16* __restrict__ src, long lds,
                                const long* __restrict__ idx, long rows, int H, int atomic) {
  const int h4 = H / 4;
  for (long i = (long)blockIdx.x * blockDim.x + threadIdx.x; i < rows * h4; i += (long)gridDim.x * blockDim.x) {
    const long r = i / h4;
    const int c = (int)(i - r * h4) * 4;
    const long dr = idx ? idx[r] : r;
    if (dr < 0) continue;
    const bf16x4 v = *(const bf16x4*)(src + r * lds + c);
    float* d = dst + dr * ldd + c;
    if (atomic) {
#pragma unroll
      for (int j = 0; j < 4; ++j) atomicAdd(d + j, (float)v[j]);
    } else {
      f32x4 o = *(f32x4*)d;
      o[0] += (float)v[0]; o[1] += (float)v[1]; o[2] += (float)v[2]; o[3] += (float)v[3];
      *(f32x4*)d = o;
    }
  }
}
__global__ void gather_rows_kernel(bf16* __restrict__ dst, const bf16* __restrict__ src, const long* __restrict__ idx,
                                   long rows, int H) {
  const int h8 = H / 8;
  for (long i = (long)blockIdx.x * blockDim.x + threadIdx.x; i < rows * h8; i += (long)gridDim.x * blockDim.x) {
    const long r = i / h8;
    const int c = (int)(i - r * h8) * 8;
    *(bf16x8*)(dst + r * H + c) = *(const bf16x8*)(src + idx[r] * H + c);
  }
}

int grid_for(long work, int block) {
  long g = (work + block - 1) / block;
  return (int)(g < 1 ? 1 : (g > 2048 ? 2048 : g));
}


}

extern "C" int spmm_ln_fwd(const void* x, const void* res, const float* gamma, const float* beta, void* y, void* zout,
                           float* mean, float* rstd, long rows, int H, float eps, float dropout_p,
                           const uint64_t* seed_ptr, uint64_t salt, const int* rows_dev, hipStream_t stream) {
  SPMM_CHECK_SHAPE(rows > 0 && H > 0 && H % 4 == 0 && H <= 1024, "spmm_ln_fwd: rows=%ld H=%d (need H%%4==0, H<=1024)", rows, H);
  SPMM_CHECK_SHAPE(dropout_p == 0.f || seed_ptr, "spmm_ln_fwd: dropout needs a device seed");
  SPMM_CHECK_SHAPE(x && gamma && beta && y, "spmm_ln_fwd: null x / gamma / beta / y");
  SPMM_CHECK_SHAPE((mean == nullptr) == (rstd == nullptr), "spmm_ln_fwd: mean and rstd come together");
  const uint32_t th = (uint32_t)(dropout_p * 65536.f + 0.5f);
  const float ds = 1.f / (1.f - dropout_p);
#define LN_FWD16(NC)                                                                                                          \
  hipLaunchKernelGGL(ln_fwd16_kernel<NC>, dim3((rows + 7) / 8), dim3(256), 0, stream, (const bf16*)x, (const bf16*)res, gamma, \
                     beta, (bf16*)y, (bf16*)zout, mean, rstd, rows, eps, th, ds, seed_ptr, salt, rows_dev)
  if (H == 768) LN_FWD16(3);
  else if (H == 1024) LN_FWD16(4);
  else if (H == 512) LN_FWD16(2);
  else if (H == 256) LN_FWD16(1);
  else
    hipLaunchKernelGGL(ln_fwd_kernel, dim3((rows + 3) / 4), dim3(256), 0, stream, (const bf16*)x, (const bf16*)res, gamma, beta,
                       (bf16*)y, (bf16*)zout, mean, rstd, rows, H, eps, th, ds, seed_ptr, salt, rows_dev);
#undef LN_FWD16
  SPMM_LAUNCH_CHECK("spmm_ln_fwd");
  return SPMM_OK;
}

extern "C" int spmm_ln_fwd_r32(const void* x, const float* res32, const float* gamma, const float* beta, void* y, float* y32, void* zout,
                               float* mean, float* rstd, long rows, int H, float eps, float dropout_p, const uint64_t* seed_ptr,
                               uint64_t salt, hipStream_t stream) {
  SPMM_CHECK_SHAPE(rows > 0 && H > 0 && H % 4 == 0 && H <= 1024, "spmm_ln_fwd_r32: rows=%ld H=%d (need H%%4==0, H<=1024)", rows, H);
  SPMM_CHECK_SHAPE(dropout_p == 0.f || seed_ptr, "spmm_ln_fwd_r32: dropout needs a device seed");
  SPMM_CHECK_SHAPE((mean == nullptr) == (rstd == nullptr), "spmm_ln_fwd_r32: mean and rstd come together");
  hipLaunchKernelGGL(ln_fwd_r32_kernel, dim3((rows + 3) / 4), dim3(256), 0, stream, (const bf16*)x, res32, gamma, beta, (bf16*)y, y32,
                     (bf16*)zout, mean, rstd, rows, H, eps, (uint32_t)(dropout_p * 65536.f + 0.5f), 1.f / (1.f - dropout_p), seed_ptr, salt);
  SPMM_LAUNCH_CHECK("spmm_ln_fwd_r32");
  return SPMM_OK;
}

extern "C" int spmm_ln_bwd(const void* dy, const void* dy2, const void* z, const float* mean, const float* rstd,
                           const float* gamma, void* dz, void* dx, float* dgamma, float* dbeta, long rows, int H,
                           float dropout_p, const uint64_t* seed_ptr, uint64_t salt, int drop_on_dy, float* dxsum, const int* rows_dev,
                           const float* beta_from_y, hipStream_t stream) {
  SPMM_CHECK_SHAPE(rows > 0 && H > 0 && H % 4 == 0 && H <= 1024, "spmm_ln_bwd: rows=%ld H=%d", rows, H);
  SPMM_CHECK_SHAPE(beta_from_y != nullptr || mean != nullptr, "spmm_ln_bwd: the row means are required unless `z` holds the LayerNorm output (beta_from_y)");
  SPMM_CHECK_SHAPE(beta_from_y == nullptr || !drop_on_dy, "spmm_ln_bwd: the output of a LayerNorm followed by dropout does not determine the normalised values");
  SPMM_CHECK_SHAPE(dropout_p == 0.f || seed_ptr, "spmm_ln_bwd: dropout needs a device seed");
  SPMM_CHECK_SHAPE(dy && z && rstd && gamma && dz, "spmm_ln_bwd: null dy / z / rstd / gamma / dz");
  long g = (rows + 3) / 4;
  static const long genv = getenv("SPMM_LN_BWD_GRID") ? atol(getenv("SPMM_LN_BWD_GRID")) : 0;
  long gmax = genv > 0 ? genv : rows / 64;
  if (genv <= 0) gmax = gmax < 256 ? 256 : (gmax > 512 ? 512 : gmax);
  if (g > gmax) g = gmax;
  const uint32_t th = (uint32_t)(dropout_p * 65536.f + 0.5f);
  const float ds = 1.f / (1.f - dropout_p);
  const bool hot = !dy2 && dx && dgamma && dbeta && dxsum && th && !drop_on_dy;
#define LN_BWD_LAUNCH(NC, EX, HOT, FY)                                                                                                \
  hipLaunchKernelGGL((ln_bwd_kernel<NC, EX, HOT, FY>), dim3(g), dim3(256), 0, stream, (const bf16*)dy, (const bf16*)dy2, (const bf16*)z, \
                     mean, rstd, gamma, beta_from_y, (bf16*)dz, (bf16*)dx, dgamma, dbeta, rows, H, th, ds, seed_ptr, salt, drop_on_dy, dxsum, rows_dev)
  if (beta_from_y != nullptr) {
    if (H == 768 && hot) LN_BWD_LAUNCH(3, true, true, true);
    else if (H <= 768) LN_BWD_LAUNCH(3, false, false, true);
    else LN_BWD_LAUNCH(4, false, false, true);
  } else {
    if (H == 768 && hot) LN_BWD_LAUNCH(3, true, true, false);
    else if (H <= 768) LN_BWD_LAUNCH(3, false, false, false);
    else LN_BWD_LAUNCH(4, false, false, false);
  }
#undef LN_BWD_LAUNCH
  SPMM_LAUNCH_CHECK("spmm_ln_bwd");
  return SPMM_OK;
}

extern "C" int spmm_embed_ln_fwd(int mode, const int* ids, const float* word, const float* pos, const float* type0,
                                 const float* pv_x, const float* pv_mask, const float* pv_w, const float* pv_b,
                                 const float* pv_cls, const float* pv_masktok, int src_mod, const float* gamma,
                                 const float* beta, void* y, void* zout, float* mean, float* rstd, long nseq, int L, int H,
                                 float eps, float dropout_p, const uint64_t* seed_ptr, uint64_t salt, hipStream_t stream) {
  SPMM_CHECK_SHAPE(nseq > 0 && L > 0 && H > 0 && H % 4 == 0 && H <= 1024, "spmm_embed_ln_fwd: nseq=%ld L=%d H=%d (need 0 < H <= 1024, H%%4==0)", nseq, L, H);
  SPMM_CHECK_SHAPE(mode >= 0 && mode <= 2, "spmm_embed_ln_fwd: unknown mode %d", mode);
  SPMM_CHECK_SHAPE(pos && type0 && gamma && beta && y, "spmm_embed_ln_fwd: null pos / type0 / gamma / beta / y");
  SPMM_CHECK_SHAPE((mean == nullptr) == (rstd == nullptr), "spmm_embed_ln_fwd: mean and rstd come together");
  SPMM_CHECK_SHAPE(mode == 0 ? (ids && word) : mode == 2 ? (pv_x != nullptr) : (pv_x && pv_mask && pv_w && pv_b && pv_cls && pv_masktok && src_mod > 0),
                   "spmm_embed_ln_fwd: missing inputs for mode %d", mode);
  SPMM_CHECK_SHAPE(dropout_p == 0.f || seed_ptr, "spmm_embed_ln_fwd: dropout needs a device seed");
  EmbedP p = {};
  p.ids = ids; p.word = word; p.pos = pos; p.type0 = type0; p.pv_x = pv_x; p.pv_mask = pv_mask; p.pv_w = pv_w; p.pv_b = pv_b;
  p.pv_cls = pv_cls; p.pv_masktok = pv_masktok; p.src_mod = src_mod; p.gamma = gamma; p.beta = beta; p.y = (bf16*)y;
  p.zout = (bf16*)zout; p.mean_o = mean; p.rstd_o = rstd; p.nseq = nseq; p.L = L; p.H = H; p.mode = mode; p.eps = eps;
  p.thresh16 = (uint32_t)(dropout_p * 65536.f + 0.5f); p.dscale = 1.f / (1.f - dropout_p); p.seed_ptr = seed_ptr; p.salt = salt;
  hipLaunchKernelGGL(embed_ln_fwd_kernel, dim3((nseq * L + 3) / 4), dim3(256), 0, stream, p);
  SPMM_LAUNCH_CHECK("spmm_embed_ln_fwd");
  return SPMM_OK;
}

extern "C" int spmm_embed_step_ln_fwd(const int* ids, int pos_index, const int* pos_ptr, const float* word, const float* pos, const float* type0,
                                      const float* gamma, const float* beta, void* y, long rows, int H, float eps,
                                      hipStream_t stream) {
  SPMM_CHECK_SHAPE(rows > 0 && pos_index >= 0 && H % 4 == 0 && H <= 1024, "spmm_embed_step_ln_fwd: rows=%ld pos=%d H=%d", rows, pos_index, H);
  SPMM_CHECK_SHAPE(ids && word && pos && type0 && gamma && beta && y, "spmm_embed_step_ln_fwd: null argument");
  EmbedP p = {};
  p.ids = ids; p.word = word; p.pos = pos; p.type0 = type0; p.gamma = gamma; p.beta = beta; p.y = (bf16*)y;
  p.nseq = rows; p.L = 1; p.H = H; p.mode = 0; p.eps = eps; p.pos0 = pos_index; p.pos_ptr = pos_ptr; p.dscale = 1.f;
  hipLaunchKernelGGL(embed_ln_fwd_kernel, dim3((rows + 3) / 4), dim3(256), 0, stream, p);
  SPMM_LAUNCH_CHECK("spmm_embed_step_ln_fwd");
  return SPMM_OK;
}

extern "C" int spmm_embed_bwd(int mode, const void* dz, const int* ids, const float* pv_x, const float* pv_mask, int src_mod,
                              float* dword, float* dpos, float* dtype0, float* d_w, float* d_b, float* d_cls,
                              float* d_masktok, long nseq, int L, int H, hipStream_t stream) {
  SPMM_CHECK_SHAPE(nseq > 0 && L > 0 && H > 0, "spmm_embed_bwd: nseq=%ld L=%d H=%d", nseq, L, H);
  SPMM_CHECK_SHAPE(mode == 0 || mode == 1, "spmm_embed_bwd: mode %d (0 = text, 1 = PV; inputs_embeds has no backward)", mode);
  SPMM_CHECK_SHAPE(dz && dpos && dtype0, "spmm_embed_bwd: null dz / dpos / dtype0");
  SPMM_CHECK_SHAPE(mode != 0 || (ids && dword), "spmm_embed_bwd: mode 0 needs ids and dword");
  SPMM_CHECK_SHAPE(mode != 1 || (pv_x && pv_mask && d_w && d_b && d_cls && d_masktok), "spmm_embed_bwd: mode 1 needs pv_x, pv_mask, d_w, d_b, d_cls and d_masktok");
  SPMM_CHECK_SHAPE(mode != 1 || src_mod > 0, "spmm_embed_bwd: mode 1 needs src_mod > 0, got src_mod=%d", src_mod);
  EmbedBwdP p = {(const bf16*)dz, ids, pv_x, pv_mask, src_mod, dword, dpos, dtype0, d_w, d_b, d_cls, d_masktok, nseq, L, H, mode};
  hipLaunchKernelGGL(embed_bwd_kernel, dim3(L, nseq >= 32 ? 16 : 1), dim3(256), 0, stream, p);
  SPMM_LAUNCH_CHECK("spmm_embed_bwd");
  return SPMM_OK;
}

namespace {
__global__ __launch_bounds__(256) void segment_sum_kernel(const bf16* __restrict__ src, const int* __restrict__ start,
                                                          const int* __restrict__ list, bf16* __restrict__ out, long W) {
  const int u = blockIdx.y;
  const long c = ((long)blockIdx.x * 256 + threadIdx.x) * 8;
  if (c >= W) return;
  const int k0 = start[u], k1 = start[u + 1];
  float acc[8] = {0.f, 0.f, 0.f, 0.f, 0.f, 0.f, 0.f, 0.f};
  for (int k = k0; k < k1; ++k) {
    const bf16x8 v = *(const bf16x8*)(src + (long)list[k] * W + c);
#pragma unroll
    for (int e = 0; e < 8; ++e) acc[e] += (float)v[e];
  }
  bf16x8 o;
#pragma unroll
  for (int e = 0; e < 8; ++e) o[e] = (bf16)acc[e];
  *(bf16x8*)(out + (long)u * W + c) = o;
}
}

extern "C" int spmm_segment_sum_bf16(const void* src, const int* start, const int* list, void* out, int U, long W, hipStream_t stream) {
  SPMM_CHECK_SHAPE(U > 0 && U <= 65535 && W > 0 && W % 8 == 0, "spmm_segment_sum_bf16: U=%d W=%ld (W %% 8 == 0)", U, W);
  SPMM_CHECK_SHAPE(src && start && list && out, "spmm_segment_sum_bf16: null src / start / list / out");
  hipLaunchKernelGGL(segment_sum_kernel, dim3((unsigned)((W / 8 + 255) / 256), U), dim3(256), 0, stream, (const bf16*)src, start, list,
                     (bf16*)out, W);
  SPMM_LAUNCH_CHECK("spmm_segment_sum_bf16");
  return SPMM_OK;
}

extern "C" int spmm_transpose_bf16(const void* in, long ldi, void* out, long ldo, int R, int C, int Rpad, float* colsum,
                                   hipStream_t stream) {
  SPMM_CHECK_SHAPE(R > 0 && C > 0 && Rpad >= R && ldo >= Rpad, "spmm_transpose_bf16: R=%d C=%d Rpad=%d ldo=%ld", R, C, Rpad, ldo);
  SPMM_CHECK_SHAPE(ldi >= C, "spmm_transpose_bf16: ldi=%ld is shorter than a row of C=%d", ldi, C);
  SPMM_CHECK_SHAPE(in && out, "spmm_transpose_bf16: null in / out");
  hipLaunchKernelGGL(transpose_bf16_kernel, dim3((C + 63) / 64, (Rpad + 63) / 64), dim3(256), 0, stream, (const bf16*)in, ldi,
                     (bf16*)out, ldo, R, C, Rpad, colsum);
  SPMM_LAUNCH_CHECK("spmm_transpose_bf16");
  return SPMM_OK;
}

extern "C" int spmm_cast_transpose(const float* in, void* out, void* outT, int R, int C, hipStream_t stream) {
  SPMM_CHECK_SHAPE(R > 0 && C > 0, "spmm_cast_transpose: R=%d C=%d", R, C);
  SPMM_CHECK_SHAPE(in && (out || outT), "spmm_cast_transpose: null in, or neither out nor outT");
  hipLaunchKernelGGL(cast_transpose_kernel, dim3((C + 63) / 64, (R + 63) / 64), dim3(256), 0, stream, in, (bf16*)out, (bf16*)outT, R, C);
  SPMM_LAUNCH_CHECK("spmm_cast_transpose");
  return SPMM_OK;
}

extern "C" long spmm_cast_transpose_desc_bytes(void) { return sizeof(CtDesc); }
extern "C" int spmm_cast_transpose_multi(const void* descs_dev, int ndesc, int total_tiles, hipStream_t stream) {
  SPMM_CHECK_SHAPE(ndesc > 0 && total_tiles > 0, "spmm_cast_transpose_multi: ndesc=%d tiles=%d", ndesc, total_tiles);
  hipLaunchKernelGGL(cast_transpose_multi_kernel, dim3(total_tiles), dim3(256), 0, stream, (const CtDesc*)descs_dev, ndesc);
  SPMM_LAUNCH_CHECK("spmm_cast_transpose_multi");
  return SPMM_OK;
}

extern "C" int spmm_cast_f32_bf16(const float* in, void* out, long n, hipStream_t stream) {
  SPMM_CHECK_SHAPE(n > 0 && n % 4 == 0, "spmm_cast_f32_bf16: n=%ld must be a positive multiple of 4", n);
  SPMM_CHECK_SHAPE(in && out, "spmm_cast_f32_bf16: null in / out");
  hipLaunchKernelGGL(cast_f32_bf16_kernel, dim3(grid_for(n / 4, 256)), dim3(256), 0, stream, in, (bf16*)out, n / 4);
  SPMM_LAUNCH_CHECK("spmm_cast_f32_bf16");
  return SPMM_OK;
}
extern "C" int spmm_cast_bf16_f32(const void* in, float* out, long n, hipStream_t stream) {
  SPMM_CHECK_SHAPE(n > 0 && n % 4 == 0, "spmm_cast_bf16_f32: n=%ld must be a positive multiple of 4", n);
  SPMM_CHECK_SHAPE(in && out, "spmm_cast_bf16_f32: null in / out");
  hipLaunchKernelGGL(cast_bf16_f32_kernel, dim3(grid_for(n / 4, 256)), dim3(256), 0, stream, (const bf16*)in, out, n / 4);
  SPMM_LAUNCH_CHECK("spmm_cast_bf16_f32");
  return SPMM_OK;
}

extern "C" int spmm_acc_rows(float* dst, long ldd, const void* src, long lds, const long* idx, long rows, int H, int atomic,
                             hipStream_t stream) {
  SPMM_CHECK_SHAPE(rows > 0 && H > 0 && H % 4 == 0, "spmm_acc_rows: rows=%ld H=%d", rows, H);
  SPMM_CHECK_SHAPE(dst && src, "spmm_acc_rows: null dst / src");
  SPMM_CHECK_SHAPE(rows == 1 || (ldd >= H && lds >= H), "spmm_acc_rows: ldd=%ld lds=%ld are shorter than a row of H=%d", ldd, lds, H);
  hipLaunchKernelGGL(acc_rows_kernel, dim3(grid_for(rows * (H / 4), 256)), dim3(256), 0, stream, dst, ldd, (const bf16*)src, lds,
                     idx, rows, H, atomic);
  SPMM_LAUNCH_CHECK("spmm_acc_rows");
  return SPMM_OK;
}
extern "C" int spmm_gather_rows(void* dst, const void* src, const long* idx, long rows, int H, hipStream_t stream) {
  SPMM_CHECK_SHAPE(rows > 0 && H > 0 && H % 8 == 0 && idx, "spmm_gather_rows: rows=%ld H=%d", rows, H);
  SPMM_CHECK_SHAPE(dst && src, "spmm_gather_rows: null dst / src");
  hipLaunchKernelGGL(gather_rows_kernel, dim3(grid_for(rows * (H / 8), 256)), dim3(256), 0, stream, (bf16*)dst, (const bf16*)src,
                     idx, rows, H);
  SPMM_LAUNCH_CHECK("spmm_gather_rows");
  return SPMM_OK;
}
```

### spmm_amd/engine.py

```python
from __future__ import annotations

import contextlib
import functools
from dataclasses import dataclass
from typing import List, NamedTuple, Optional

import numpy as np
import torch

from . import ops, streams
from .config import BertConfig, SPMMConfig
from .options import EngineOptions
from .params import ParamStore

BF = torch.bfloat16
LOSS_MLM, LOSS_MPM, LOSS_ITA, LOSS_ITM = 0, 1, 2, 3


def _ceil(x, m):
    return (x + m - 1) // m * m


class KVSource:

    def __init__(self, kv: torch.Tensor, U: int, Lkv: int, row0=None, length=None, pack_idx=None, proj=None):
        self.kv, self.U, self.Lkv, self.row0, self.len, self.pack_idx = kv, U, Lkv, row0, length, pack_idx
        self.proj = proj
        self._idx: List[torch.Tensor] = []
        self.nseq = 0
        self.start = self.list = None

    def add(self, idx: torch.Tensor) -> int:
        off = self.nseq
        self._idx.append(idx)
        self.nseq += idx.numel()
        return off

    def preset(self, nseq: int, start: torch.Tensor, lst: torch.Tensor):
        self.nseq, self.start, self.list = nseq, start, lst
        return self

    def finalize(self):
        idx = torch.cat(self._idx)
        order = torch.sort(idx, stable=True).indices
        start = torch.zeros(self.U + 1, dtype=torch.int32, device=idx.device)
        counts = torch.zeros(self.U, dtype=torch.int64, device=idx.device).index_add_(0, idx, torch.ones_like(idx))
        start[1:] = torch.cumsum(counts, 0)
        self.start, self.list = start, order.to(torch.int32)
        return self


@dataclass
class SelfKV:
    x: torch.Tensor
    dx: Optional[torch.Tensor] = None
    rows_dev: Optional[torch.Tensor] = None


@dataclass
class Group:
    row0: int
    nseq: int
    L: int
    kmask: Optional[torch.Tensor]
    causal_from: int
    kv: Optional[torch.Tensor] = None
    Lkv: int = 0
    kv_mask: Optional[torch.Tensor] = None
    q_row0: Optional[torch.Tensor] = None
    q_len: Optional[torch.Tensor] = None
    nrows: int = -1
    src: Optional[KVSource] = None
    kv_idx: Optional[torch.Tensor] = None
    kv_off: int = 0
    self_src: Optional[SelfKV] = None
    skv_row0: Optional[torch.Tensor] = None
    skv_len: Optional[torch.Tensor] = None
    skv_L: int = 0

    @property
    def rows(self):
        n = self.nrows if self.nrows >= 0 else self.nseq * self.L
        return slice(self.row0, self.row0 + n)

    def bind(self, src: KVSource, kv_idx: torch.Tensor, kv_off: int) -> "Group":
        self.src, self.Lkv, self.kv_idx, self.kv_off = src, src.Lkv, kv_idx, kv_off
        return self

    def attend(self, src: KVSource, idx: torch.Tensor) -> "Group":
        self.src, self.Lkv = src, src.Lkv
        self.kv_off = src.add(idx)
        self.kv_idx = idx.to(torch.int32)
        return self

    def cross_layout(self) -> dict:
        src = self.src
        return dict(kmask=self.kv_mask, kv_seq=self.kv_idx, q_row0=self.q_row0, q_len=self.q_len,
                    kv_row0=None if src is None else src.row0, kv_len=None if src is None else src.len)


@dataclass
class Batch:
    groups: List[Group]
    rows_dev: Optional[torch.Tensor] = None

    def __iter__(self):
        return iter(self.groups)

    def __len__(self):
        return len(self.groups)


@dataclass
class LnTape:
    z: Optional[torch.Tensor]
    y: Optional[torch.Tensor]
    mean: Optional[torch.Tensor]
    rstd: Optional[torch.Tensor]
    salt: int = 0


@dataclass
class HeadTape:
    dense: str
    norm: str
    X: torch.Tensor
    pre: Optional[torch.Tensor]
    ln: LnTape


def _prefix_lens(mask_h: torch.Tensor) -> Optional[torch.Tensor]:
    lens = mask_h.sum(1)
# ... 251 lines not shown
                           zout=x if (save and not from_y) else None, mean=mean, rstd=rstd, eps=eps, dropout_p=ph, seed=self.seed, salt=salt)
        return y, LnTape(None if from_y else x, y, mean, rstd, salt), y32

    def _proj_ln_bwd(self, op, tape, dY, A, ph, md=None):
        P, (M, H) = self.P, dY.shape
        dz = self._new(M, H)
        dx = self._new(M, H) if ph > 0 else dz
        from_y = tape.z is None
        ops.ln_bwd(dY, tape.y if from_y else tape.z, tape.mean, tape.rstd, P.w(op + "LayerNorm.weight"), dz, dx=dx if ph > 0 else None,
                   dgamma=P.g(op + "LayerNorm.weight"), dbeta=P.g(op + "LayerNorm.bias"), dropout_p=ph, seed=self.seed, salt=tape.salt,
                   dxsum=P.g(op + "dense.bias"), rows_dev=md, beta_from_y=P.w(op + "LayerNorm.bias") if from_y else None)
        self._wgrad(dx, A, P.g(op + "dense.weight"), md=md)
        return dz, dx

    def _attn_block_fwd(self, pfx, c, X, groups, save, cross, X32=None, kv_tap=None):
        P, H, nH = self.P, c.hidden_size, c.num_attention_heads
        salts_a = [self._next_salt() for _ in groups]
        salt_h = self._next_salt()
        sv = {"X": X, "salt_a": salts_a, "cross": cross}
        if not cross:
            ctx, core = self._self_attn_fwd(pfx, c, X, groups, save, salts_a, kv_tap)
        else:
            sv["Qc"] = Qc = ops.gemm_nt(X, P.wb(pfx + ".self.query.weight"), self._new(X.shape[0], H), bias=P.w(pfx + ".self.query.bias"),
                                        M_dev=groups.rows_dev)
            done = {id(g.src): g.src.proj[pfx] for g in groups if g.src is not None and g.src.proj and pfx in g.src.proj}
            kv_of = functools.partial(self._xattn_kv, P.fused(pfx + ".self.", ("key", "value"), "weight"),
                                      P.fused(pfx + ".self.", ("key", "value"), "bias", what="w"), done)
            fx = self.opt.fused_xattn
            fused = ((fx is True or fx == "all" or (fx == "nograd" and not save)) and not self._xattn_off and X32 is None
                     and groups.rows_dev is None and all(ops.xattn_supported(H, nH, g.L, g.Lkv) for g in groups))
            if fused:
                y, out = self._xattn_fused_fwd(pfx, c, X, Qc, kv_of, groups, save, salts_a, salt_h)
                g0 = groups.groups[0]
                if not self._xattn_checked and not ops._DRY_RUN and g0.row0 == 0:
                    self._xattn_checked = True
                    agrees, dmax, dmean = self._xattn_agrees(pfx, c, X, Qc, out["KV"][0], g0, y, salts_a[0], salt_h)
                    if not agrees:
                        import warnings
                        warnings.warn(f"spmm_amd: the fused cross-attention kernel disagrees with the composite launches (max |dy| {dmax:.3g}, "
                                      f"mean {dmean:.3g}); falling back to the composite for this process (SPMM_FUSED_XATTN=off)")
                        streams.note("fused cross-attention kernel failed its one-time self-check: composite launches used instead")
                        self._xattn_off = True
                        fused = False
                if fused:
                    sv.update(out)
                    return y, (sv if save else None), None
            ctx, core = self._xattn_core_fwd(c, Qc, kv_of, groups, save, salts_a)
        y, ln, y32 = self._proj_ln(pfx + ".output.", ctx, X, X32, save=save, eps=c.layer_norm_eps, ph=self._p_hidden(c), salt=salt_h,
                                   md=groups.rows_dev)
        sv.update(core, ctx=ctx, ln=ln)
        return y, (sv if save else None), y32

    def _self_attn_fwd(self, pfx, c, X, groups, save, salts, kv_tap=None):
        P, H, nH, M = self.P, c.hidden_size, c.num_attention_heads, X.shape[0]
        Wqkv = P.fused(pfx + ".self.", ("query", "key", "value"), "weight")
        bqkv = P.fused(pfx + ".self.", ("query", "key", "value"), "bias", what="w")
        QKV = ops.gemm_nt(X, Wqkv, self._new(M, 3 * H), bias=bqkv, M_dev=groups.rows_dev)
        if kv_tap is not None:
            kv_tap(QKV)
        ctx, lses = self._new(M, H), []
        skv = {}
        for g, salt in zip(groups, salts):
            lse = self._new(g.nseq, nH, g.L, dtype=torch.float32) if save else None
            r = g.rows
            kw = dict(nseq=g.nseq, nH=nH, Lq=g.L, dropout_p=self._p_attn(c), seed=self.seed, salt=salt, q_row0=g.q_row0, q_len=g.q_len)
            if g.self_src is not None:
                if id(g.self_src) not in skv:
                    skv[id(g.self_src)] = ops.gemm_nt(g.self_src.x, Wqkv[H:], self._new(g.self_src.x.shape[0], 2 * H), bias=bqkv[H:],
                                                      M_dev=g.self_src.rows_dev)
                KVs = skv[id(g.self_src)]
                ops.attn_fwd_long(QKV[r, :H], KVs[:, :H], KVs[:, H:], ctx[r], lse, Lkv=g.skv_L, kmask=None, causal_from=g.nseq,
                                  kv_row0=g.skv_row0, kv_len=g.skv_len, **kw)
            else:
                ops.attn_fwd_long(QKV[r, :H], QKV[r, H:2 * H], QKV[r, 2 * H:], ctx[r], lse, Lkv=g.L, kmask=g.kmask, causal_from=g.causal_from,
                                  kv_row0=g.q_row0, kv_len=g.q_len, **kw)
            lses.append(lse)
        return ctx, dict(QKV=QKV, SKV=skv, lse=lses)

    def _xattn_kv(self, Wkv, bkv, done, g):
        key, kv = (id(g), g.kv) if g.src is None else (id(g.src), g.src.kv)
        if key not in done:
            done[key] = ops.gemm_nt(kv, Wkv, self._new(kv.shape[0], Wkv.shape[0]), bias=bkv)
        return done[key]

    def _xattn_core_fwd(self, c, Qc, kv_of, groups, save, salts):
        H, nH = c.hidden_size, c.num_attention_heads
        ctx, KVs, lses = self._new(Qc.shape[0], H), [], []
        for g, salt in zip(groups, salts):
            KV = kv_of(g)
            lse = self._new(g.nseq, nH, g.L, dtype=torch.float32) if save else None
            ops.attn_fwd_long(Qc[g.rows], KV[:, :H], KV[:, H:], ctx[g.rows], lse, nseq=g.nseq, nH=nH, Lq=g.L, Lkv=g.Lkv, is_cross=True,
                              dropout_p=self._p_attn(c), seed=self.seed, salt=salt, **g.cross_layout())
            KVs.append(KV)
            lses.append(lse)
        return ctx, dict(KV=KVs, lse=lses)

    def _xattn_fused_fwd(self, pfx, c, X, Qc, kv_of, groups, save, salts, salt_h):
        P, H, nH, M = self.P, c.hidden_size, c.num_attention_heads, X.shape[0]
        y = self._new(M, H)
        z, ctx = (self._new(M, H), self._new(M, H)) if save else (None, None)
        mean, rstd = self._stats(M, save)
        WoF = P.wF(pfx + ".output.dense.weight")
        KVs, lses = [], []
        for g, salt in zip(groups, salts):
            KV = kv_of(g)
            lse = self._new(g.nseq, nH, g.L, dtype=torch.float32) if save else None
            r = g.rows
            ops.xattn_fwd(Qc[r], KV[:, :H], KV[:, H:], WoF, P.w(pfx + ".output.dense.bias"), X[r], P.w(pfx + ".output.LayerNorm.weight"),
                          P.w(pfx + ".output.LayerNorm.bias"), y[r], nseq=g.nseq, nH=nH, Lq=g.L, Lkv=g.Lkv, eps=c.layer_norm_eps,
                          Z=None if z is None else z[r], mean=None if mean is None else mean[r.start:r.stop],
                          rstd=None if rstd is None else rstd[r.start:r.stop], CTX=None if ctx is None else ctx[r], lse=lse,
                          attn_dropout_p=self._p_attn(c), salt_a=salt, hidden_dropout_p=self._p_hidden(c), salt_h=salt_h, seed=self.seed,
                          row_base=r.start, **g.cross_layout())
            KVs.append(KV)
            lses.append(lse)
        return y, dict(KV=KVs, lse=lses, ctx=ctx, ln=LnTape(z, y, mean, rstd, salt_h))

    def _xattn_agrees(self, pfx, c, X, Qc, KV, g, y, salt_a, salt_h):
        H, r = c.hidden_size, g.rows
        c2 = self._new(r.stop, H)
        ops.attn_fwd_long(Qc[r], KV[:, :H], KV[:, H:], c2, None, nseq=g.nseq, nH=c.num_attention_heads, Lq=g.L, Lkv=g.Lkv, is_cross=True,
                          dropout_p=self._p_attn(c), seed=self.seed, salt=salt_a, **g.cross_layout())
        y2, _, _ = self._proj_ln(pfx + ".output.", c2, X[r], None, save=False, eps=c.layer_norm_eps, ph=self._p_hidden(c), salt=salt_h)
        d = (y[r].float() - y2.float()).abs()
        dmax, dmean = float(d.max()), float(d.mean())
        scale = max(1.0, float(y2.float().abs().max()) / 8.0)
        return dmax < 0.25 * scale and dmean < 5e-3 * scale, dmax, dmean

    def _attn_block_bwd(self, pfx, c, sv, dY, groups, dkv_acc):
        P, H, nH = self.P, c.hidden_size, c.num_attention_heads
        X, M, md = sv["X"], sv["X"].shape[0], groups.rows_dev
        pa, ph = self._p_attn(c), self._p_hidden(c)
        dz, dx = self._proj_ln_bwd(pfx + ".output.", sv["ln"], dY, sv["ctx"], ph, md)
        dctx = self._new(M, H)
        ops.gemm_nt(dx, self._wT(pfx + ".output.dense", P.w(pfx + ".output.dense.weight")), dctx, M_dev=md)
        dX = self._new(M, H)
        if not sv["cross"]:
            QKV = sv["QKV"]
            dQKV = self._new(M, 3 * H)
            gWqkv = P.fused(pfx + ".self.", ("query", "key", "value"), "weight", what="g")
            gbqkv = P.fused(pfx + ".self.", ("query", "key", "value"), "bias", what="g")
            dskv = {}
            for i, g in enumerate(groups):
                r = g.rows
                kw = dict(nseq=g.nseq, nH=nH, Lq=g.L, dropout_p=pa, seed=self.seed, salt=sv["salt_a"][i], q_row0=g.q_row0, q_len=g.q_len)
                if g.self_src is not None:
                    if id(g.self_src) not in dskv:
                        dskv[id(g.self_src)] = (g.self_src, self._zeros(g.self_src.x.shape[0], 2 * H))
                    KVs, dKVs = sv["SKV"][id(g.self_src)], dskv[id(g.self_src)][1]
                    ops.attn_bwd_long(QKV[r, :H], KVs[:, :H], KVs[:, H:], sv["ctx"][r], sv["lse"][i], dctx[r], dQKV[r, :H], dKVs[:, :H], dKVs[:, H:],
                                      Lkv=g.skv_L, kmask=None, causal_from=g.nseq, kv_row0=g.skv_row0, kv_len=g.skv_len, **kw)
                    ops.zero_(dQKV[r, H:])
                    continue
                ops.attn_bwd_long(QKV[r, :H], QKV[r, H:2 * H], QKV[r, 2 * H:], sv["ctx"][r], sv["lse"][i], dctx[r], dQKV[r, :H],
                                  dQKV[r, H:2 * H], dQKV[r, 2 * H:], Lkv=g.L, kmask=g.kmask, causal_from=g.causal_from,
                                  kv_row0=g.q_row0, kv_len=g.q_len, **kw)
            self._wgrad(dQKV, X, gWqkv, gbqkv, md=md)
            WT = self._wT(pfx + ".self.qkv", P.fused(pfx + ".self.", ("query", "key", "value"), "weight", what="w"))
            for src, dKVs in dskv.values():
                self._wgrad(dKVs, src.x, gWqkv[H:], gbqkv[H:], md=src.rows_dev)
                ops.gemm_nt(dKVs, WT[:, H:], src.dx, M_dev=src.rows_dev)
            ops.gemm_nt(dQKV, WT, dX, R=dz, M_dev=md)
        else:
            Qc = sv["Qc"]
            dQc = self._new(M, H)
            gWkv = P.fused(pfx + ".self.", ("key", "value"), "weight", what="g")
            gbkv = P.fused(pfx + ".self.", ("key", "value"), "bias", what="g")
            WkvT = self._wT(pfx + ".self.kv", P.fused(pfx + ".self.", ("key", "value"), "weight", what="w"))
            pool = {}
            for i, g in enumerate(groups):
                r = g.rows
                KV = sv["KV"][i]
                src = g.src
                if src is not None:
                    if id(src) not in pool:
                        pool[id(src)] = (src, self._new(src.nseq * src.Lkv, 2 * H))
                    dKV = pool[id(src)][1][g.kv_off * g.Lkv:(g.kv_off + g.nseq) * g.Lkv]
                else:
                    dKV = self._new(g.nseq * g.Lkv, 2 * H)
                ops.attn_bwd_long(Qc[r], KV[:, :H], KV[:, H:], sv["ctx"][r], sv["lse"][i], dctx[r], dQc[r], dKV[:, :H], dKV[:, H:],
                                  nseq=g.nseq, nH=nH, Lq=g.L, Lkv=g.Lkv, is_cross=True, dropout_p=pa, seed=self.seed, salt=sv["salt_a"][i],
                                  **g.cross_layout())
                if src is None:
                    self._wgrad(dKV, g.kv, gWkv, gbkv)
                    ops.gemm_nt(dKV, WkvT, dkv_acc[i], epi=ops.EPI_F32_ACC)
            for src, dKV in pool.values():
                W = src.Lkv * 2 * H
                dKVu = ops.segment_sum_bf16(dKV.view(src.nseq, W), src.start, src.list, self._new(src.U, W)).view(-1, 2 * H)
                if src.pack_idx is not None:
                    dKVu = ops.gather_rows(self._new(src.pack_idx.numel(), 2 * H), dKVu, src.pack_idx)
                self._wgrad(dKVu, src.kv, gWkv, gbkv)
                ops.gemm_nt(dKVu, WkvT, dkv_acc[id(src)], epi=ops.EPI_F32_ACC)
            self._wgrad(dQc, X, P.g(pfx + ".self.query.weight"), P.g(pfx + ".self.query.bias"), md=md)
            ops.gemm_nt(dQc, self._wT(pfx + ".self.query", P.w(pfx + ".self.query.weight")), dX, R=dz, M_dev=md)
        return dX

    def _layer_fwd(self, lp, c, has_cross, X, groups, save, X32=None, kv_tap=None):
        P, H, I, M = self.P, c.hidden_size, c.intermediate_size, X.shape[0]
        tap = {} if kv_tap is None else {"kv_tap": kv_tap}
        a, sv1, a32 = self._attn_block_fwd(lp + "attention", c, X, groups, save, cross=False, X32=X32, **tap)
        sv2 = None
        if has_cross:
            a, sv2, a32 = self._attn_block_fwd(lp + "crossattention", c, a, groups, save, cross=True, X32=a32)
        h = self._new(M, I)
        dact = self._new(M, I) if save else None
        ops.gemm_nt(a, P.wb(lp + "intermediate.dense.weight"), h, bias=P.w(lp + "intermediate.dense.bias"),
                    epi=ops.EPI_GELU_DERIV if save else ops.EPI_GELU, C2=dact, M_dev=groups.rows_dev)
        salt = self._next_salt()
        y, ln, y32 = self._proj_ln(lp + "output.", h, a, a32, save=save, eps=c.layer_norm_eps, ph=self._p_hidden(c), salt=salt, md=groups.rows_dev)
        sv = dict(att=sv1, cross=sv2, a=a, h=h, dact=dact, ln=ln) if save else None
        return y, sv, y32

    def _layer_bwd(self, lp, c, sv, dY, groups, dkv_acc):
        P, H, I, M, md = self.P, c.hidden_size, c.intermediate_size, dY.shape[0], groups.rows_dev
        dz, dx = self._proj_ln_bwd(lp + "output.", sv["ln"], dY, sv["h"], self._p_hidden(c), md)
        dpre = self._new(M, I)
        ops.gemm_nt(dx, self._wT(lp + "output.dense", P.w(lp + "output.dense.weight")), dpre,
                    epi=ops.EPI_MUL, G=sv["dact"], colsum=P.g(lp + "intermediate.dense.bias"), M_dev=md)
        self._wgrad(dpre, sv["a"], P.g(lp + "intermediate.dense.weight"), md=md)
        da = self._new(M, H)
        ops.gemm_nt(dpre, self._wT(lp + "intermediate.dense", P.w(lp + "intermediate.dense.weight")), da, R=dz, M_dev=md)
        if sv["cross"] is not None:
            da = self._attn_block_bwd(lp + "crossattention", c, sv["cross"], da, groups, dkv_acc)
        return self._attn_block_bwd(lp + "attention", c, sv["att"], da, groups, None)

    def stack_fwd(self, pfx, c, layers, has_cross, X, groups, save, X32=None, kv_tap=None):
        tape = []
        for i in layers:
            tap = None if kv_tap is None else functools.partial(kv_tap, i)
            X, sv, X32 = self._layer_fwd(f"{pfx}encoder.layer.{i}.", c, has_cross and i >= c.fusion_layer, X, groups, save, X32=X32, kv_tap=tap)
            tape.append(sv)
        return X, tape, X32

    def stack_bwd(self, pfx, c, layers, tape, dY, groups, dkv_acc=None):
        for i, sv in zip(reversed(list(layers)), reversed(tape)):
            dY = self._layer_bwd(f"{pfx}encoder.layer.{i}.", c, sv, dY, groups, dkv_acc)
            if self.layer_done_cb is not None:
                self._layer_done(f"{pfx}encoder.layer.{i}.")
        return dY

    def _layer_done(self, prefix):
        ws = self._wg_stream if (self._wg_pending and self.wgrad_async) else None
        if ws is None:
            self.wgrad_join()
            return self.layer_done_cb(prefix)
        streams.after(ws, torch.cuda.current_stream())
        with torch.cuda.stream(ws):
            return self.layer_done_cb(prefix)

    def _embed(self, mode, pfx, c, nseq, L, save, salt, **src):
        P, H = self.P, c.hidden_size
        y = self._new(nseq * L, H)
        z = self._new(nseq * L, H) if save else None
        mean, rstd = self._stats(nseq * L, save)
        ops.embed_ln_fwd(mode, y, nseq=nseq, L=L, H=H, pos=P.w(pfx + "embeddings.position_embeddings.weight"),
                         type0=P.w(pfx + "embeddings.token_type_embeddings.weight"), gamma=P.w(pfx + "embeddings.LayerNorm.weight"),
                         beta=P.w(pfx + "embeddings.LayerNorm.bias"), zout=z, mean=mean, rstd=rstd, eps=c.layer_norm_eps,
                         dropout_p=self._p_hidden(c), seed=self.seed, salt=salt, **src)
        return y, LnTape(z, None, mean, rstd, salt)

    def embed_text(self, pfx, c, ids32, nseq, L, save):
        return self._embed(0, pfx, c, nseq, L, save, self._next_salt(), ids=ids32, word=self.P.w(pfx + "embeddings.word_embeddings.weight"))

    def embed_pv(self, pfx, c, prop, mpm_mask, nseq, src_mod, save):
        P = self.P
        return self._embed(1, pfx, c, nseq, self.cfg.n_props + 1, save, self._next_salt(), pv_x=prop, pv_mask=mpm_mask,
                           pv_w=P.w("property_embed.weight"), pv_b=P.w("property_embed.bias"), pv_cls=P.w("property_cls"),
                           pv_masktok=P.w("property_mask"), src_mod=src_mod)

    def embed_generic(self, pfx, c, inputs_embeds_f32, nseq, L):
        return self._embed(2, pfx, c, nseq, L, False, self._next_salt(), pv_x=inputs_embeds_f32)[0]

    def _embed_ln_bwd(self, pfx, c, tape, dY):
        P = self.P
        dz = self._new(*dY.shape)
# ... 86 lines not shown
```

### spmm_amd/ops.py

```python
import ctypes
import os

import torch

from ._lib import lib

EPI_BF16, EPI_GELU, EPI_F32, EPI_F32_ATOMIC, EPI_GELU_GRAD, EPI_F32_ACC, EPI_GELU_DERIV, EPI_MUL = range(8)
BF16 = torch.bfloat16


_DRY_RUN = False
_dry_log = []


def _p(t):
    return None if t is None else ctypes.c_void_p(t.data_ptr())


def _st():
    if _DRY_RUN:
        return None
    return ctypes.c_void_p(torch.cuda.current_stream().cuda_stream)


_DEBUG_SYNC = os.environ.get("SPMM_DEBUG_SYNC") == "1"


def _call(name, *args):
    if not _DRY_RUN:
        if _DEBUG_SYNC:
            import sys
            r = lib().call(name, *args)
            print(f"[launch] {name} {[a for a in args if isinstance(a, int) and not isinstance(a, bool)][:8]}", file=sys.stderr, flush=True)
            torch.cuda.synchronize()
            return r
        return lib().call(name, *args)
    res, argtypes = lib().protos[name]
    if len(args) != len(argtypes):
        raise TypeError(f"{name}: {len(args)} arguments, header declares {len(argtypes)}")
    for i, (a, t) in enumerate(zip(args, argtypes)):
        try:
            t(a) if not isinstance(a, ctypes.c_void_p) else None
        except Exception as e:
            raise TypeError(f"{name}: argument {i} = {a!r} is not a {t.__name__}") from e
        if t is ctypes.c_void_p and not (a is None or isinstance(a, (ctypes.c_void_p, int))):
            raise TypeError(f"{name}: argument {i} must be a pointer, got {type(a)}")
    _dry_log.append(name)


def _row_stride(t):
    assert t.dim() == 2 and (t.stride(1) == 1 or t.shape[1] == 1), (t.shape, t.stride())
    return t.stride(0)


GEMM_AUTO, GEMM_AUTO_TILES = 0, 16
_nt_auto = GEMM_AUTO


class nt_tiles_per_workgroup:

    def __init__(self, on=True):
        self.on = on

    def __enter__(self):
        global _nt_auto
        self._prev = _nt_auto
        if self.on:
            _nt_auto = GEMM_AUTO_TILES
        return self

    def __exit__(self, *exc):
        global _nt_auto
        _nt_auto = self._prev
        return False


def gemm_nt(A, W, C, *, bias=None, epi=EPI_BF16, R=None, G=None, C2=None, alpha=1.0, div=None, splits=1, K=None, colsum=None, kernel=0,
            M_dev=None):
    if kernel == 0:
        kernel = _nt_auto
    M, Ka = A.shape
    N = W.shape[0]
    K = Ka if K is None else K
    assert A.dtype == BF16 and W.dtype == BF16 and W.shape[1] >= K and C.shape[0] >= M and C.shape[1] >= N
    if epi in (EPI_BF16, EPI_GELU, EPI_GELU_GRAD, EPI_GELU_DERIV, EPI_MUL):
        assert C.dtype == BF16
    else:
        assert C.dtype == torch.float32
    _call("spmm_gemm_nt", _p(A), _row_stride(A), _p(W), _row_stride(W), M, N, K, splits, _p(bias), _p(div),
               float(alpha), _p(R), 0 if R is None else _row_stride(R), _p(G), 0 if G is None else _row_stride(G),
               _p(C), _row_stride(C), _p(C2), 0 if C2 is None else _row_stride(C2), epi, _p(colsum), int(kernel), _p(M_dev), _st())
    return C


def gemm_tn(A, B, C, *, alpha=1.0, splits=None, kernel=0, M_dev=None):
    M, N = A.shape
    K = B.shape[1]
    assert A.dtype == BF16 and B.dtype == BF16 and C.dtype == torch.float32 and B.shape[0] == M and tuple(C.shape) == (N, K)
    if splits is None:
        splits = 1 if _DRY_RUN else lib().cdll.spmm_gemm_tn_splits(M, N, K, int(kernel))
    ws = torch.empty(splits * N * K, dtype=torch.float32, device=C.device) if splits > 1 else None
    _call("spmm_gemm_tn", _p(A), _row_stride(A), _p(B), _row_stride(B), M, N, K, splits, float(alpha), _p(C), _row_stride(C), _p(ws),
          int(kernel), _p(M_dev), _st())
    return C


def colsum_bf16(x, out, *, R_dev=None):
    R, C = x.shape
    _call("spmm_colsum_bf16", _p(x), _row_stride(x), R, C, _p(out), _p(R_dev), _st())
    return out


def attn_fwd(Q, K, V, O, lse, *, nseq, nH, Lq, Lkv, kmask=None, causal_from=None, is_cross=False, dropout_p=0.0,
             seed=None, salt=0, kv_seq=None, q_row0=None, q_len=None, kv_row0=None, kv_len=None, q_off=0, kv_off=0):
    cf = nseq if causal_from is None else causal_from
    _call("spmm_attn_fwd", _p(Q), _row_stride(Q), _p(K), _row_stride(K), _p(V), _row_stride(V), _p(kmask), _p(kv_seq), _p(q_row0),
               _p(q_len), _p(kv_row0), _p(kv_len), _p(O),
               _row_stride(O), _p(lse), nseq, nH, Lq, Lkv, cf, int(is_cross), float(dropout_p), _p(seed), salt, int(q_off), int(kv_off), _st())
    return O


def attn_bwd(Q, K, V, O, lse, dO, dQ, dK, dV, *, nseq, nH, Lq, Lkv, kmask=None, causal_from=None, is_cross=False,
             dropout_p=0.0, seed=None, salt=0, kv_seq=None, q_row0=None, q_len=None, kv_row0=None, kv_len=None, q_off=0, kv_off=0,
             d_mode=0, dbuf=None):
    cf = nseq if causal_from is None else causal_from
    _call("spmm_attn_bwd", _p(Q), _row_stride(Q), _p(K), _row_stride(K), _p(V), _row_stride(V), _p(kmask), _p(kv_seq), _p(q_row0),
               _p(q_len), _p(kv_row0), _p(kv_len), _p(O),
               _row_stride(O), _p(lse), _p(dO), _row_stride(dO), _p(dQ), _row_stride(dQ), _p(dK), _row_stride(dK), _p(dV),
               _row_stride(dV), nseq, nH, Lq, Lkv, cf, int(is_cross), float(dropout_p), _p(seed), salt, int(q_off), int(kv_off), int(d_mode),
               _p(dbuf), _st())


def xattn_supported(H, nH, Lq, Lkv):
    return bool(_DRY_RUN or lib().cdll.spmm_xattn_supported(int(H), int(nH), int(Lq), int(Lkv)))


def xattn_pack_wo(W, out=None):
    H = W.shape[0]
    assert W.dtype == BF16 and W.shape[1] == H
    out = torch.empty(H * H, dtype=BF16, device=W.device) if out is None else out
    _call("spmm_xattn_pack_wo", _p(W), _row_stride(W), _p(out), H, _st())
    return out


def xattn_fwd(Q, K, V, WoF, bo, R, gamma, beta, Y, *, nseq, nH, Lq, Lkv, eps=1e-12, kmask=None, kv_seq=None, q_row0=None, q_len=None,
              kv_row0=None, kv_len=None, Z=None, mean=None, rstd=None, CTX=None, lse=None, attn_dropout_p=0.0, salt_a=0,
              hidden_dropout_p=0.0, salt_h=0, seed=None, row_base=0):
    _call("spmm_xattn_fwd", _p(Q), _row_stride(Q), _p(K), _row_stride(K), _p(V), _row_stride(V), _p(kmask), _p(kv_seq), _p(q_row0), _p(q_len),
          _p(kv_row0), _p(kv_len), _p(WoF), _p(bo), _p(R), _row_stride(R), _p(gamma), _p(beta), float(eps), _p(Y), _row_stride(Y), _p(Z),
          0 if Z is None else _row_stride(Z), _p(mean), _p(rstd), _p(CTX), 0 if CTX is None else _row_stride(CTX), _p(lse), nseq, nH, Lq, Lkv,
          float(attn_dropout_p), salt_a, float(hidden_dropout_p), salt_h, _p(seed), int(row_base), _st())
    return Y


def ln_fwd(x, res, gamma, beta, y, *, zout=None, mean=None, rstd=None, eps=1e-12, dropout_p=0.0, seed=None, salt=0, rows_dev=None):
    rows, H = x.shape
    _call("spmm_ln_fwd", _p(x), _p(res), _p(gamma), _p(beta), _p(y), _p(zout), _p(mean), _p(rstd), rows, H, float(eps),
               float(dropout_p), _p(seed), salt, _p(rows_dev), _st())
    return y


def ln_fwd_r32(x, res32, gamma, beta, y, *, y32=None, zout=None, mean=None, rstd=None, eps=1e-12, dropout_p=0.0, seed=None, salt=0):
    rows, H = x.shape
    assert res32 is None or res32.dtype == torch.float32
    assert y32 is None or y32.dtype == torch.float32
    _call("spmm_ln_fwd_r32", _p(x), _p(res32), _p(gamma), _p(beta), _p(y), _p(y32), _p(zout), _p(mean), _p(rstd), rows, H, float(eps),
          float(dropout_p), _p(seed), salt, _st())
    return y


def ln_bwd(dy, z, mean, rstd, gamma, dz, *, dy2=None, dx=None, dgamma=None, dbeta=None, dropout_p=0.0, seed=None, salt=0,
           drop_on_dy=False, dxsum=None, rows_dev=None, beta_from_y=None):
    rows, H = dy.shape
    _call("spmm_ln_bwd", _p(dy), _p(dy2), _p(z), _p(mean), _p(rstd), _p(gamma), _p(dz), _p(dx), _p(dgamma), _p(dbeta),
               rows, H, float(dropout_p), _p(seed), salt, int(drop_on_dy), _p(dxsum), _p(rows_dev), _p(beta_from_y), _st())
    return dz


def embed_ln_fwd(mode, y, *, nseq, L, H, pos, type0, gamma, beta, ids=None, word=None, pv_x=None, pv_mask=None, pv_w=None,
                 pv_b=None, pv_cls=None, pv_masktok=None, src_mod=1, zout=None, mean=None, rstd=None, eps=1e-12,
                 dropout_p=0.0, seed=None, salt=0):
    _call("spmm_embed_ln_fwd", mode, _p(ids), _p(word), _p(pos), _p(type0), _p(pv_x), _p(pv_mask), _p(pv_w), _p(pv_b),
               _p(pv_cls), _p(pv_masktok), src_mod, _p(gamma), _p(beta), _p(y), _p(zout), _p(mean), _p(rstd), nseq, L, H,
               float(eps), float(dropout_p), _p(seed), salt, _st())
    return y


def embed_bwd(mode, dz, *, nseq, L, H, dpos, dtype0, ids=None, dword=None, pv_x=None, pv_mask=None, src_mod=1, d_w=None,
              d_b=None, d_cls=None, d_masktok=None):
    _call("spmm_embed_bwd", mode, _p(dz), _p(ids), _p(pv_x), _p(pv_mask), src_mod, _p(dword), _p(dpos), _p(dtype0),
               _p(d_w), _p(d_b), _p(d_cls), _p(d_masktok), nseq, L, H, _st())


def transpose_bf16(x, out, *, Rpad=None, colsum=None):
    R, C = x.shape
    Rpad = out.shape[1] if Rpad is None else Rpad
    _call("spmm_transpose_bf16", _p(x), _row_stride(x), _p(out), _row_stride(out), R, C, Rpad, _p(colsum), _st())
    return out


def cast_transpose(w32, out, outT):
    R, C = w32.shape
    _call("spmm_cast_transpose", _p(w32), _p(out), _p(outT), R, C, _st())


def cast_transpose_multi(descs_dev, ndesc, total_tiles):
    _call("spmm_cast_transpose_multi", _p(descs_dev), ndesc, total_tiles, _st())


def cast_f32_bf16(x, out):
    _call("spmm_cast_f32_bf16", _p(x), _p(out), x.numel(), _st())
    return out


def cast_bf16_f32(x, out):
    _call("spmm_cast_bf16_f32", _p(x), _p(out), x.numel(), _st())
    return out


def acc_rows(dst, src, *, idx=None, atomic=False):
    rows, H = src.shape
    _call("spmm_acc_rows", _p(dst), _row_stride(dst), _p(src), _row_stride(src), _p(idx), rows, H, int(atomic), _st())


def gather_rows(dst, src, idx):
    rows, H = dst.shape
    _call("spmm_gather_rows", _p(dst), _p(src), _p(idx), rows, H, _st())
    return dst


SRC_B = 1 << 40


def gather_rows2(dst, srcA, idx, srcB=None):
    rows, H = dst.shape
    assert idx.dtype == torch.int64 and idx.numel() >= rows and dst.is_contiguous() and srcA.is_contiguous() and (srcB is None or srcB.is_contiguous())
    assert dst.dtype == BF16 and srcA.dtype == BF16 and srcA.shape[1] == H and (srcB is None or (srcB.dtype == BF16 and srcB.shape[1] == H))
    _call("spmm_gather_rows2", _p(dst), _p(srcA), _p(srcB), _p(idx), rows, H, _st())
    return dst


def add_rows_bf16(dst, idx, src):
    rows, H = src.shape
    assert dst.dtype == BF16 and src.dtype == BF16 and idx.dtype == torch.int64 and dst.is_contiguous() and src.is_contiguous() and dst.shape[1] == H
    _call("spmm_add_rows_bf16", _p(dst), _p(idx), _p(src), rows, H, _st())
    return dst


def zero_(t):
    n = t.numel() * t.element_size()
    if n == 0:
        return t
    if not t.is_contiguous():
        es = t.element_size()
        if t.dim() == 2 and t.stride(1) == 1 and (t.shape[1] * es) % 16 == 0 and (t.stride(0) * es) % 16 == 0 and t.data_ptr() % 16 == 0:
            _call("spmm_zero_rows", _p(t), t.shape[0], t.shape[1] * es, t.stride(0) * es, _st())
            return t
        return t.zero_()
    if n % 16 or t.data_ptr() % 16:
        return t.zero_()
    _call("spmm_zero_bytes", _p(t), n, _st())
    return t


def gelu_bwd(dz, pre, out=None):
    assert dz.dtype == BF16 and pre.dtype == BF16 and dz.is_contiguous() and pre.is_contiguous() and dz.shape == pre.shape
    out = torch.empty_like(dz) if out is None else out
    _call("spmm_gelu_bwd", _p(dz), _p(pre), _p(out), dz.numel(), _st())
    return out


def pack_plan(mask32, M, bad):
    B, Lt = mask32.shape
    dev = mask32.device
    alloc = torch.zeros if _DRY_RUN else torch.empty
    i32 = alloc(2 * B, dtype=torch.int32, device=dev)
    i64 = alloc(B + M + (M + B * Lt) + 2 * M + 2 * B * Lt + (B + M), dtype=torch.int64, device=dev)
    o = [0]

    def cut(n):
        o[0] += n
        return i64[o[0] - n:o[0]]
    row0_64, rows, gidx2, gidx4, inv, idx_m = cut(B), cut(M), cut(M + B * Lt), cut(2 * M), cut(2 * B * Lt), cut(B + M)
    _call("spmm_pack_plan", _p(mask32), B, Lt, M, _p(i32[:B]), _p(i32[B:]), _p(row0_64), _p(rows), _p(gidx2), _p(gidx4), _p(inv), _p(idx_m), _p(bad), _st())
    return dict(M=M, rows=rows, row0=i32[B:], row0_64=row0_64, len=i32[:B], gidx2=gidx2, gidx4=gidx4, inv=inv, idx_m=idx_m)


FUSION_SMALL = dict(ar=(0, 1), kvidx_pv=(1, 3), kvidx_tp=(4, 2), qrow0_tp=(6, 2), qlen_tp=(8, 2), row0_8=(10, 1), len_8=(11, 1),
                    skv_row0_pv=(12, 3), skv_len_pv=(15, 3), skv_row0_tx=(18, 2), skv_len_tx=(20, 2), start_t=(22, 2), list_t=(24, 4),
                    start_p=(28, 2), list_p=(30, 4))


def fusion_plan(neg, pk, Lp):
    B = pk["len"].numel()
    Lt = (pk["inv"].numel() // 2) // B
    M, dev = pk["M"], neg.device
    Rcap = 4 * B * Lp + 2 * M + 2 * B * Lt
    ntop = 6 * B + B * Lt + B * Lp
    alloc = torch.zeros if _DRY_RUN else torch.empty
    i64 = alloc(Rcap + B * Lt + ntop, dtype=torch.int64, device=dev)
    idx6, neg_rows, idx_top = i64[:Rcap], i64[Rcap:Rcap + B * Lt], i64[Rcap + B * Lt:]
    small = alloc(35 * B + 2, dtype=torch.int32, device=dev)
    _call("spmm_fusion_plan", _p(neg), _p(pk["len"]), _p(pk["row0"]), B, Lt, Lp, M, _p(idx6), _p(neg_rows), _p(idx_top), _p(small), _st())
    out = dict(idx6=idx6, neg_rows=neg_rows, idx_top=idx_top, Rcap=Rcap, rows_dev=small[34 * B:34 * B + 1], mn_dev=small[34 * B + 1:34 * B + 2])
    for k, (o, n) in FUSION_SMALL.items():
        out[k] = small[o * B:(o + n) * B]
    out["start_t"], out["start_p"] = out["start_t"][:B + 1], out["start_p"][:B + 1]
    return out


# ... 229 lines not shown
    assert anc is None or (anc.dtype == torch.int32 and anc.shape[0] == N * k and anc.stride(1) == 1)
    if ids_out is None:
        ids_out = torch.empty(N * k, dtype=torch.int32, device=logits.device)
    args = (_p(logits), logits.stride(0), N, k, logits.shape[1], L, book.F, int(t), _p(t_ptr), int(t_off), _p(book.tokens),
            _p(book.cur_p), _p(book.fin_p), _p(book.fin_len), _p(book.fin_tok), _p(book.fin_n), _p(book.done), _p(anc),
            0 if anc is None else anc.stride(0), _p(ids_out), _p(parent_out), _p(book.n_done), _p(mol), _p(rowmap))
    until = need is not None
    need = int(getattr(book, "need", k) if need is None else need)
    if until or need != k:
        assert noise is None, "the sampled search ends at k finals"
        _call("spmm_beam_step_until", *args, need, _st())
    elif noise is None:
        _call("spmm_beam_step", *args, _st())
    else:
        assert noise.dtype == torch.float32 and noise.dim() == 2 and noise.stride(1) == 1 and noise.device == logits.device
        assert noise.shape[0] == N * k and noise.shape[1] >= logits.shape[1], (noise.shape, logits.shape)
        _call("spmm_beam_step_sampled", *args, _p(noise), noise.stride(0), _st())
    return ids_out


def gumbel_noise(seed, N, k, V, Lmax, *, salt=0, t=0, t_ptr=None, t_off=0, mol=None, mol_base=0, out=None):
    assert seed.dtype == torch.int64 and seed.numel() == 1
    assert mol is None or (mol.dtype == torch.int32 and mol.numel() == N and mol.is_contiguous())
    if out is None:
        out = torch.empty(N * k, V, dtype=torch.float32, device=seed.device)
    assert out.dtype == torch.float32 and out.dim() == 2 and out.shape[0] == N * k and out.shape[1] >= V and out.stride(1) == 1
    _call("spmm_gumbel_noise", _p(seed), int(salt), N, k, V, Lmax, int(t), _p(t_ptr), int(t_off), _p(mol), int(mol_base), _p(out), out.stride(0), _st())
    return out


def logit_warp(lc, lu=None, *, w=1.0, temperature=1.0, top_k=0, top_p=1.0, min_keep=1, out=None):
    assert lc.dtype == torch.float32 and lc.dim() == 2 and (lc.stride(1) == 1 or lc.shape[1] == 1)
    R, V = lc.shape
    if lu is not None:
        assert lu.dtype == torch.float32 and lu.shape == lc.shape and lu.device == lc.device and (R <= 1 or lu.stride(0) == lc.stride(0))
        assert lu.stride(1) == 1 or V == 1
    if out is None:
        out = lc
    assert out.dtype == torch.float32 and out.shape == lc.shape and out.device == lc.device and (out.stride(1) == 1 or V == 1)
    _call("spmm_logit_warp", _p(lc), _p(lu), lc.stride(0), R, V, float(w), float(temperature), int(top_k), float(top_p), int(min_keep),
          _p(out), out.stride(0), _st())
    return out


SYNTAX_MASKED = -1e30


def smiles_mask(logits, tokens, table, *, t=0, t_last, k=1, mol=None, Lmax=None, logits2=None, t_ptr=None, t_off=0, state_out=None):
    assert logits.dtype == torch.float32 and logits.dim() == 2 and (logits.stride(1) == 1 or logits.shape[1] == 1)
    R, V = logits.shape
    if logits2 is not None:
        assert logits2.dtype == torch.float32 and logits2.shape == logits.shape and logits2.device == logits.device
        assert (R <= 1 or logits2.stride(0) == logits.stride(0)) and (logits2.stride(1) == 1 or V == 1)
    assert tokens.dtype == torch.int32 and tokens.dim() in (2, 3) and tokens.stride(-1) == 1
    if tokens.dim() == 3:
        assert tokens.is_contiguous() and tokens.shape[1] == k
        tokens = tokens.view(-1, tokens.shape[2])
    if Lmax is None:
        Lmax = tokens.shape[1]
    assert tokens.shape[1] >= (t if t_ptr is None else t_last), (tokens.shape, t, t_last)
    assert table.dtype == torch.int32 and tuple(table.shape) == (V, 4) and table.is_contiguous() and table.device == logits.device
    assert mol is None or (mol.dtype == torch.int32 and mol.is_contiguous() and mol.numel() * k == R)
    assert state_out is None or (state_out.dtype == torch.int32 and tuple(state_out.shape) == (R, 4) and state_out.is_contiguous())
    _call("spmm_smiles_mask", _p(logits), _p(logits2), logits.stride(0), R, V, _p(tokens), tokens.stride(0), tokens.shape[0], int(k), _p(mol),
          int(Lmax), int(t), _p(t_ptr), int(t_off), int(t_last), _p(table), _p(state_out), _st())
    return logits


def kv_prefill(K, V, row0, length, dst_row, Kc, Vc):
    R, nH, Lmax, dh = Kc.shape
    assert K.dtype == BF16 and V.dtype == BF16 and Kc.dtype == BF16 and Vc.dtype == BF16 and dh == 64
    assert K.shape == V.shape and K.shape[1] == nH * 64 and _row_stride(K) == _row_stride(V)
    assert Kc.is_contiguous() and Vc.is_contiguous() and Vc.shape == Kc.shape
    E = row0.numel()
    assert all(t.dtype == torch.int32 and t.numel() == E and t.is_contiguous() and t.device == Kc.device for t in (row0, length, dst_row))
    _call("spmm_kv_prefill", _p(K), _p(V), _row_stride(K), K.shape[0], _p(row0), _p(length), _p(dst_row), E, _p(Kc), _p(Vc), R, nH, Lmax, _st())


def segment_sum_bf16(src, start, lst, out):
    U, W = out.shape
    assert src.dtype == BF16 and out.dtype == BF16 and src.shape[1] == W and src.is_contiguous() and out.is_contiguous()
    assert start.dtype == torch.int32 and lst.dtype == torch.int32 and start.numel() == U + 1
    _call("spmm_segment_sum_bf16", _p(src), _p(start), _p(lst), _p(out), U, W, _st())
    return out


ATTN_MAXL = 256


def _chunks(L, step=128):
    return [(o, min(step, L - o)) for o in range(0, L, step)]


def attn_fwd_long(Q, K, V, O, lse, *, nseq, nH, Lq, Lkv, kmask=None, causal_from=None, is_cross=False, dropout_p=0.0, seed=None,
                  salt=0, kv_seq=None, q_row0=None, q_len=None, kv_row0=None, kv_len=None):
    if Lq <= ATTN_MAXL and Lkv <= ATTN_MAXL:
        return attn_fwd(Q, K, V, O, lse, nseq=nseq, nH=nH, Lq=Lq, Lkv=Lkv, kmask=kmask, causal_from=causal_from, is_cross=is_cross,
                        dropout_p=dropout_p, seed=seed, salt=salt, kv_seq=kv_seq, q_row0=q_row0, q_len=q_len, kv_row0=kv_row0, kv_len=kv_len)
    if q_row0 is not None or kv_row0 is not None:
        raise ValueError("packed layouts are limited to %d-token sequences" % ATTN_MAXL)
    dev, H = Q.device, nH * 64
    nsrc = K.shape[0] // Lkv
    ar_q = torch.arange(nseq, dtype=torch.int32, device=dev)
    ar_k = torch.arange(nsrc, dtype=torch.int32, device=dev)
    Ov = O.view(nseq, Lq, nH, 64)
    for qi, (q0, ql) in enumerate(_chunks(Lq)):
        q_row0, q_len = ar_q * Lq + q0, torch.full((nseq,), ql, dtype=torch.int32, device=dev)
        outs, lses = [], []
        for ci, (k0, kl) in enumerate(_chunks(Lkv)):
            Oc = torch.empty(nseq * Lq, H, dtype=BF16, device=dev)
            lc = torch.empty(nseq, nH, ql, dtype=torch.float32, device=dev)
            attn_fwd(Q, K, V, Oc, lc, nseq=nseq, nH=nH, Lq=ql, Lkv=kl, kmask=None if kmask is None else kmask[:, k0:k0 + kl].contiguous(),
                     causal_from=causal_from, is_cross=is_cross, dropout_p=dropout_p, seed=seed, salt=salt + 7919 * (qi * 8 + ci + 1),
                     kv_seq=kv_seq, q_row0=q_row0, q_len=q_len, kv_row0=ar_k * Lkv + k0,
                     kv_len=torch.full((nsrc,), kl, dtype=torch.int32, device=dev), q_off=q0, kv_off=k0)
            outs.append(Oc.view(nseq, Lq, nH, 64)[:, q0:q0 + ql].float())
            lses.append(lc)
        L = torch.stack(lses)
        tot = torch.logsumexp(L, dim=0)
        acc = sum(o * torch.exp(l - tot).permute(0, 2, 1)[..., None] for o, l in zip(outs, lses))
        Ov[:, q0:q0 + ql] = acc.to(BF16)
        if lse is not None:
            lse[:, :, q0:q0 + ql] = tot
    return O


def attn_bwd_long(Q, K, V, O, lse, dO, dQ, dK, dV, *, nseq, nH, Lq, Lkv, kmask=None, causal_from=None, is_cross=False, dropout_p=0.0,
                  seed=None, salt=0, kv_seq=None, q_row0=None, q_len=None, kv_row0=None, kv_len=None):
    if Lq <= ATTN_MAXL and Lkv <= ATTN_MAXL:
        return attn_bwd(Q, K, V, O, lse, dO, dQ, dK, dV, nseq=nseq, nH=nH, Lq=Lq, Lkv=Lkv, kmask=kmask, causal_from=causal_from,
                        is_cross=is_cross, dropout_p=dropout_p, seed=seed, salt=salt, kv_seq=kv_seq, q_row0=q_row0, q_len=q_len,
                        kv_row0=kv_row0, kv_len=kv_len)
    if q_row0 is not None or kv_row0 is not None:
        raise ValueError("packed layouts are limited to %d-token sequences" % ATTN_MAXL)
    dev, H = Q.device, nH * 64
    nsrc = K.shape[0] // Lkv
    nkv_out = nseq if kv_seq is not None else nsrc
    ar_q = torch.arange(nseq, dtype=torch.int32, device=dev)
    ar_k = torch.arange(nsrc, dtype=torch.int32, device=dev)
    dQ32 = torch.zeros(nseq, Lq, H, dtype=torch.float32, device=dev)
    dK32 = torch.zeros(nkv_out, Lkv, H, dtype=torch.float32, device=dev)
    dV32 = torch.zeros(nkv_out, Lkv, H, dtype=torch.float32, device=dev)
    for qi, (q0, ql) in enumerate(_chunks(Lq)):
        q_row0, q_len = ar_q * Lq + q0, torch.full((nseq,), ql, dtype=torch.int32, device=dev)
        lse_i = lse[:, :, q0:q0 + ql].contiguous()
        calls = []
        for ci, (k0, kl) in enumerate(_chunks(Lkv)):
            calls.append(dict(nseq=nseq, nH=nH, Lq=ql, Lkv=kl, kmask=None if kmask is None else kmask[:, k0:k0 + kl].contiguous(),
                              causal_from=causal_from, is_cross=is_cross, dropout_p=dropout_p, seed=seed,
                              salt=salt + 7919 * (qi * 8 + ci + 1), kv_seq=kv_seq, q_row0=q_row0, q_len=q_len, kv_row0=ar_k * Lkv + k0,
                              kv_len=torch.full((nsrc,), kl, dtype=torch.int32, device=dev), q_off=q0, kv_off=k0))
        dQc = torch.empty(nseq * Lq, H, dtype=BF16, device=dev)
        D = torch.zeros(nseq, nH, ql, dtype=torch.float32, device=dev)
        for (k0, kl), kw in zip(_chunks(Lkv), calls):
            Dc = torch.empty_like(D)
            tmp = torch.empty((nseq if kv_seq is not None else nsrc) * (kl if kv_seq is not None else Lkv), H, dtype=BF16, device=dev)
            attn_bwd(Q, K, V, O, lse_i, dO, dQc, tmp, tmp, d_mode=1, dbuf=Dc, **kw)
            D += Dc
        for (k0, kl), kw in zip(_chunks(Lkv), calls):
            if kv_seq is not None:
                dKc = torch.zeros(nseq * kl, H, dtype=BF16, device=dev); dVc = torch.zeros_like(dKc)
            else:
                dKc = torch.zeros(nsrc * Lkv, H, dtype=BF16, device=dev); dVc = torch.zeros_like(dKc)
            attn_bwd(Q, K, V, O, lse_i, dO, dQc, dKc, dVc, d_mode=2, dbuf=D, **kw)
            dQ32[:, q0:q0 + ql] += dQc.view(nseq, Lq, H)[:, q0:q0 + ql].float()
            if kv_seq is not None:
# ... 7 lines not shown
```

### spmm_amd/options.py

```python
from __future__ import annotations

import dataclasses
import os
from dataclasses import dataclass

_ENV = {
    "pack_text": ("SPMM_PACK_TEXT", lambda s: s != "0"),
    "cls_only_top": ("SPMM_CLS_ONLY_TOP", lambda s: s != "0"),
    "multi_stream": ("SPMM_STREAMS", lambda s: s != "1"),
    "wgrad_stream": ("SPMM_WGRAD_STREAM", lambda s: s != "0"),
    "pv_wgrad_inline": ("SPMM_PV_WGRAD_INLINE", int),
    "ln_from_y": ("SPMM_LN_FROM_Y", lambda s: s != "0"),
    "resid_fp32": ("SPMM_RESID_FP32", lambda s: s == "1"),
    "fused_xattn": ("SPMM_FUSED_XATTN", lambda s: {"0": "off", "1": "all"}.get(s, s)),
    "grad_overlap": ("SPMM_GRAD_OVERLAP", lambda s: s != "0"),
    "grad_wire": ("SPMM_GRAD_WIRE", str),
    "nt_under_comm": ("SPMM_NT_UNDER_COMM", str),
    "force_dist": ("SPMM_FORCE_DIST", lambda s: s == "1"),
    "dp_four_streams": ("SPMM_DP_FOUR_STREAMS", lambda s: s != "0"),
    "probe_streams": ("SPMM_PROBE_STREAMS", lambda s: s != "0"),
    "schedule_check": ("SPMM_SCHEDULE_CHECK", lambda s: s != "0"),
}


@dataclass
class EngineOptions:
    pack_text: bool = True
    cls_only_top: bool = True
    multi_stream: bool = True
    wgrad_stream: bool = True
    pv_wgrad_inline: int = 4
    ln_from_y: bool = True
    fused_xattn: str = "nograd"
    resid_fp32: bool = False
    grad_overlap: bool = True
    grad_wire: str = "fp32"
    nt_under_comm: str = "auto"
    force_dist: bool = False
    dp_four_streams: bool = True
    schedule_check: bool = True
    probe_streams: bool = False

    @classmethod
    def from_env(cls, **overrides) -> "EngineOptions":
        kw = {}
        for field, (var, parse) in _ENV.items():
            if var in os.environ:
                kw[field] = parse(os.environ[var])
        kw.update(overrides)
        o = cls(**kw)
        if isinstance(o.fused_xattn, bool):
            o.fused_xattn = "all" if o.fused_xattn else "off"
        if o.fused_xattn not in ("off", "nograd", "all"):
            raise ValueError(f"fused_xattn must be off, nograd or all, not {o.fused_xattn!r}")
        if o.grad_wire not in ("fp32", "bf16"):
            raise ValueError(f"grad_wire must be fp32 or bf16, not {o.grad_wire!r}")
        if o.nt_under_comm not in ("tiles", "persistent", "auto"):
            raise ValueError(f"nt_under_comm must be tiles, persistent or auto, not {o.nt_under_comm!r}")
        return o

    def replace(self, **kw) -> "EngineOptions":
        return dataclasses.replace(self, **kw)
```

### spmm_amd/params.py

```python
from __future__ import annotations

import math
import struct
from typing import Dict, List, Optional

import torch

from . import ops
from .config import SPMMConfig, is_buffer, momentum_twin, state_spec, student_of

ALIGN = 64


def ct_descriptor_table(pairs):
    blob, tile0 = b"", 0
    for src, dstT in pairs:
        R, C = src.shape
        ntr, ntc = (R + 63) // 64, (C + 63) // 64
        blob += struct.pack("<QQiiii", src.data_ptr(), dstT.data_ptr(), R, C, tile0, ntc)
        tile0 += ntr * ntc
    assert len(blob) == len(pairs) * 32
    return blob, tile0


def _layout_order(spec) -> List[str]:
    names = [n for n, _, k in spec if not is_buffer(n) and student_of(n) is None and k not in ("tied_w", "tied_b")]
    done, out = set(), []
    for n in names:
        if n in done:
            continue
        if n.endswith(".self.query.weight"):
            base = n[:-len("query.weight")]
            grp = [base + f"{x}.{y}" for y in ("weight", "bias") for x in ("query", "key", "value")]
            out += grp
            done.update(grp)
        else:
            out.append(n)
            done.add(n)
    assert sorted(out) == sorted(names)
    return out


class ParamStore:
    def __init__(self, cfg: SPMMConfig, device, train: bool = True, spec=None):
        self.cfg, self.device, self.train = cfg, device, train
        twins = spec is None
        self.spec = state_spec(cfg) if twins else list(spec)
        self.shape = {n: s for n, s, _ in self.spec}
        self.kind = {n: k for n, _, k in self.spec}
        self.order = _layout_order(self.spec)
        self.offset: Dict[str, int] = {}
        off = 0
        for n in self.order:
            self.offset[n] = off
            numel = int(math.prod(self.shape[n])) if self.shape[n] else 1
            off += (numel + ALIGN - 1) // ALIGN * ALIGN
        self.total = off
        f32 = dict(dtype=torch.float32, device=device)
        self.flat = torch.zeros(self.total, **f32)
        self.flat_m = torch.zeros(self.total if twins else 0, **f32)
        self.shadow = torch.zeros(self.total, dtype=torch.bfloat16, device=device)
        self.shadow_m = torch.zeros(self.total if twins else 0, dtype=torch.bfloat16, device=device)
        if train:
            self.grad = torch.zeros(self.total, **f32)
            self.adam_m = torch.zeros(self.total, **f32)
            self.adam_v = torch.zeros(self.total, **f32)
        H, E, Q = cfg.text.hidden_size, cfg.embed_dim, cfg.queue_size
        self.buffers: Dict[str, torch.Tensor] = {}
        for n, s, k in self.spec:
            if k == "posid":
                self.buffers[n] = torch.arange(s[1], device=device).expand(1, -1).clone()
            elif k == "queue":
                self.buffers[n] = torch.zeros(s, **f32)
            elif k == "ptr":
                self.buffers[n] = torch.zeros(1, dtype=torch.long, device=device)
        self._wT: Dict[str, torch.Tensor] = {}
        self._wT_pad: Dict[str, str] = {}
        self._wF: Dict[str, tuple] = {}

    def _resolve(self, name: str):
        st = student_of(name)
        mom = st is not None
        base = st if mom else name
        if self.kind.get(base) == "tied_w":
            base = base.replace("cls.predictions.decoder.weight", "bert.embeddings.word_embeddings.weight")
        elif self.kind.get(base) == "tied_b":
            base = base.replace("cls.predictions.decoder.bias", "cls.predictions.bias")
        return mom, base

    def _view(self, buf: torch.Tensor, base: str, shape=None):
        shape = self.shape[base] if shape is None else shape
        n = int(math.prod(shape)) if shape else 1
        return buf[self.offset[base]: self.offset[base] + n].view(shape)

    def w(self, name: str) -> torch.Tensor:
        mom, base = self._resolve(name)
        return self._view(self.flat_m if mom else self.flat, base)

    def wb(self, name: str) -> torch.Tensor:
        mom, base = self._resolve(name)
        return self._view(self.shadow_m if mom else self.shadow, base)

    def g(self, name: str) -> torch.Tensor:
        mom, base = self._resolve(name)
        assert not mom
        return self._view(self.grad, base)

    def fused(self, prefix: str, names, kind: str, what: str = "wb") -> torch.Tensor:
        first = f"{prefix}{names[0]}.{kind}"
        mom, base = self._resolve(first)
        shp = self.shape[base]
        rows = sum(self.shape[self._resolve(f"{prefix}{n}.{kind}")[1]][0] for n in names)
        o = self.offset[base]
        for n in names:
            b = self._resolve(f"{prefix}{n}.{kind}")[1]
            assert self.offset[b] == o, (b, self.offset[b], o)
            o += int(math.prod(self.shape[b]))
        buf = {"wb": self.shadow_m if mom else self.shadow, "w": self.flat_m if mom else self.flat,
               "g": None if mom else getattr(self, "grad", None)}[what]
        full = (rows,) + tuple(shp[1:])
        return buf[self.offset[base]: self.offset[base] + int(math.prod(full))].view(full)

    def wT(self, key: str, src: Optional[torch.Tensor] = None) -> torch.Tensor:
        if key not in self._wT:
            assert src is not None
            R, C = src.shape
            self._wT[key] = torch.empty(C, R, dtype=torch.bfloat16, device=self.device)
            self._wT_src = getattr(self, "_wT_src", {})
            self._wT_src[key] = src
            ops.cast_transpose(src, None, self._wT[key])
        return self._wT[key]

    def wT_padded(self, key: str, name: str, cols: int) -> torch.Tensor:
        if key not in self._wT:
            self._wT[key] = torch.zeros(self.w(name).shape[1], cols, dtype=torch.bfloat16, device=self.device)
            self._wT_pad[key] = name
            self.refresh_padded_shadows()
        return self._wT[key]

    def refresh_padded_shadows(self):
        for key, name in self._wT_pad.items():
            w = self.w(name)
            self._wT[key][:, :w.shape[0]].copy_(w.t())

    def wF(self, name: str) -> torch.Tensor:
        if name not in self._wF:
            src = self.wb(name)
            self._wF[name] = (src, torch.empty(src.numel(), dtype=torch.bfloat16, device=self.device), student_of(name) is not None)
            ops.xattn_pack_wo(src, self._wF[name][1])
        return self._wF[name][1]

    def refresh_frag(self, momentum: bool):
        for src, out, mom in self._wF.values():
            if mom == momentum:
                ops.xattn_pack_wo(src, out)

    def refresh_shadows(self, transposed_only: bool = False, part: str = "all"):
        if not transposed_only:
            ops.cast_f32_bf16(self.flat, self.shadow)
            if self.flat_m.numel():
                ops.cast_f32_bf16(self.flat_m, self.shadow_m)
        if part in ("all", "forward"):
            self.refresh_frag(False)
            if not transposed_only:
                self.refresh_frag(True)
        if part == "forward":
            return
        srcs = getattr(self, "_wT_src", {})
        if not srcs:
            return
        if getattr(self, "_ct_n", -1) != len(srcs):
            blob, tiles = ct_descriptor_table([(src, self._wT[key]) for key, src in srcs.items()])
            self._ct_desc = torch.frombuffer(bytearray(blob), dtype=torch.uint8).to(self.device)
            self._ct_n, self._ct_tiles = len(srcs), tiles
        ops.cast_transpose_multi(self._ct_desc, self._ct_n, self._ct_tiles)

    def copy_params(self):
        self.flat_m.copy_(self.flat)
        self.shadow_m.copy_(self.shadow)

    def named_tensors(self):
        for n, _, _ in self.spec:
            yield n, (self.buffers[n] if n in self.buffers else self.w(n))

    def load_state_dict(self, sd: Dict[str, torch.Tensor], strict: bool = True):
        missing = [n for n, _, _ in self.spec if n not in sd]
        unexpected = [k for k in sd if k not in self.shape]
        bad = [k for k in sd if k in self.shape and tuple(sd[k].shape) != tuple(self.shape[k]) and sd[k].numel() != int(math.prod(self.shape[k]) if self.shape[k] else 1)]
        if bad:
            raise RuntimeError(f"size mismatch for {bad[:5]}")
        if strict and (missing or unexpected):
            raise KeyError(f"state_dict mismatch: missing {missing[:5]} unexpected {unexpected[:5]}")
        with torch.no_grad():
            for n, t in self.named_tensors():
                if n in sd:
                    if self.kind[n] in ("tied_w", "tied_b"):
                        continue
                    t.copy_(sd[n].to(t.device).reshape(t.shape))
        self.refresh_shadows()
        return missing, unexpected
```

### spmm_amd/step.py

```python
from __future__ import annotations

from typing import Callable, Optional, Tuple

import torch

from . import ops, streams
from .engine import STREAM_TOKENS_MAX, BF, LOSS_ITA, LOSS_ITM, LOSS_MLM, LOSS_MPM, Batch, Engine, Group, KVSource, SelfKV, _ceil


class PretrainStep(Engine):
    def _s6_forward_cls(self, B, Lt, M, pk, mask32, neg, y1, y2, prop_embeds, text_embeds, save):
        cfg = self.cfg
        ct = cfg.text
        H, Lp, f, n = ct.hidden_size, cfg.n_props + 1, ct.fusion_layer, ct.num_hidden_layers
        fp = ops.fusion_plan(neg, pk, Lp)
        o_tp = 3 * B * Lp
        o_lm = o_tp + 2 * M
        o_12 = o_lm + B * Lt
        o_8 = o_12 + B * Lp
        Rcap = fp["Rcap"]
        X6 = ops.gather_rows2(self._new(Rcap, H), y1, fp["idx6"], y2)
        src_pv = KVSource(prop_embeds.view(B * Lp, H), B, Lp).preset(4 * B, fp["start_p"], fp["list_p"])
        src_text = KVSource(text_embeds, B, Lt, row0=pk["row0"], length=pk["len"], pack_idx=pk["rows"]).preset(4 * B, fp["start_t"], fp["list_t"])
        ar = fp["ar"]
        g_lo = Batch([Group(0, 3 * B, Lp, None, 3 * B).bind(src_text, fp["kvidx_pv"], 0),
                      Group(o_tp, 2 * B, Lt, None, 2 * B, q_row0=fp["qrow0_tp"], q_len=fp["qlen_tp"], nrows=2 * M).bind(src_pv, fp["kvidx_tp"], 0),
                      Group(o_lm, B, Lt, mask32, 0).bind(src_pv, ar, 2 * B),
                      Group(o_12, B, Lp, None, 0).bind(src_text, ar, 3 * B),
                      Group(o_8, B, Lt, None, B, q_row0=fp["row0_8"], q_len=fp["len_8"], nrows=B * Lt).bind(src_pv, ar, 3 * B)],
                     rows_dev=fp["rows_dev"])
        y, tape_lo, _ = self.stack_fwd("text_encoder.bert.", ct, range(f, n - 1), True, X6, g_lo, save)
        ntop = 6 * B + B * Lt + B * Lp
        Xtop = ops.gather_rows2(self._new(ntop, H), y, fp["idx_top"])
        skv_a = SelfKV(y[:o_lm])
        skv_b = SelfKV(y[o_8:], rows_dev=fp["mn_dev"])
        g_top = Batch([Group(0, 3 * B, 1, None, 3 * B, self_src=skv_a, skv_row0=fp["skv_row0_pv"], skv_len=fp["skv_len_pv"], skv_L=Lp).bind(src_text, fp["kvidx_pv"], 0),
                       Group(3 * B, 2 * B, 1, None, 2 * B, self_src=skv_a, skv_row0=fp["skv_row0_tx"], skv_len=fp["skv_len_tx"], skv_L=Lt).bind(src_pv, fp["kvidx_tp"], 0),
                       Group(5 * B, B, 1, None, B, self_src=skv_b, skv_row0=fp["row0_8"], skv_len=fp["len_8"], skv_L=Lt).bind(src_pv, ar, 3 * B),
                       Group(6 * B, B, Lt, mask32, 0).bind(src_pv, ar, 2 * B),
                       Group(6 * B + B * Lt, B, Lp, None, 0).bind(src_text, ar, 3 * B)])
        ytop, sv_top, _ = self._layer_fwd(f"text_encoder.bert.encoder.layer.{n - 1}.", ct, True, Xtop, g_top, save)
        return dict(fp=fp, ytop=ytop, sv_top=sv_top, g_top=g_top, skv=(skv_a, skv_b), g_lo=g_lo, tape_lo=tape_lo, src_text=src_text, src_pv=src_pv,
                    o_tp=o_tp, o_lm=o_lm, o_12=o_12, o_8=o_8, ntop=ntop, Rcap=Rcap)

    def _s6_backward_cls(self, T, dYtop, d_pe, d_te):
        S6, B, Lt, M = T["S6"], T["B"], T["Lt"], T["M"]
        cfg = self.cfg
        ct = cfg.text
        H, Lp, f, n = ct.hidden_size, cfg.n_props + 1, ct.fusion_layer, ct.num_hidden_layers
        fp, o_lm, o_8 = S6["fp"], S6["o_lm"], S6["o_8"]
        dkv_acc = {id(S6["src_text"]): d_te[:M], id(S6["src_pv"]): d_pe.view(B * Lp, H)}
        dX6 = self._new(S6["Rcap"], H)
        S6["skv"][0].dx = dX6[:o_lm]
        S6["skv"][1].dx = dX6[o_8:]
        dXtop = self._layer_bwd(f"text_encoder.bert.encoder.layer.{n - 1}.", ct, S6["sv_top"], dYtop, S6["g_top"], dkv_acc)
        if self.layer_done_cb is not None:
            self._layer_done(f"text_encoder.bert.encoder.layer.{n - 1}.")
        ops.add_rows_bf16(dX6, fp["idx_top"][:6 * B], dXtop[:6 * B])
        dX6[o_lm:o_8].copy_(dXtop[6 * B:])
        return self.stack_bwd("text_encoder.bert.", ct, range(f, n - 1), S6["tape_lo"], dX6, S6["g_lo"], dkv_acc=dkv_acc)

    def forward(self, prop: torch.Tensor, ids: torch.Tensor, mask: torch.Tensor, *, mpm_mask: Optional[torch.Tensor] = None,
                neg_idx: Optional[Tuple[torch.Tensor, torch.Tensor]] = None, gather: Optional[Callable] = None,
                save: bool = True, aux: Optional[dict] = None, n_tokens: Optional[int] = None) -> torch.Tensor:
        cfg, P = self.cfg, self.P
        ct, cp = cfg.text, cfg.prop
        H, E, Lp, f, n = ct.hidden_size, cfg.embed_dim, cfg.n_props + 1, ct.fusion_layer, ct.num_hidden_layers
        B, Lt = ids.shape
        if B % 4 or cfg.queue_size % 4:
            raise ValueError("batch size and queue size must be multiples of 4")
        self._salt = 0
        if self.train_mode:
            self.seed.add_(1)
        ops.zero_(self.step_zero)
        temp = P.w("temp").view(1)
        ops.clamp_scalar(temp, 0.01, 0.5)
        ids32 = ids.to(torch.int32).contiguous()
        mask32 = mask.to(torch.int32).contiguous()
        prop = prop.to(torch.float32).contiguous()
        if mpm_mask is None:
            mpm_mask = (torch.rand(B, cfg.n_props, device=self.dev) < 0.5).to(torch.float32)
        mpm_mask = mpm_mask.to(torch.float32).contiguous()

        self._one_stream = self.force_one_stream or B * Lt > STREAM_TOKENS_MAX
        pk = self._pack_plan(mask32, B, Lt, n_tokens) if (self.pack_text and aux is None and Lt <= ops.ATTN_MAXL) else None
        if n_tokens is not None:
            self.nan_flag.bitwise_or_(self.hint_bad)
        M = pk["M"] if pk else B * Lt
        ids2 = torch.cat([ids32, ids32])
        r32 = self.opt.resid_fp32 and aux is None
        f32 = (lambda t: t.float()) if r32 else (lambda t: None)
        side = self._fork()
        with self._on(side):
            x2, esv2 = self.embed_text("text_encoder.bert.", ct, ids2, 2 * B, Lt, save)
            x2_32 = f32(x2)
            if pk:
                x2d = x2
                x2 = ops.gather_rows2(self._new(M + B * Lt, H), x2d, pk["gidx2"])
                if r32:
                    x2_32 = torch.cat([x2_32[:B * Lt].index_select(0, pk["rows"]), x2_32[B * Lt:]])
                g2 = Batch([Group(0, B, Lt, None, B, q_row0=pk["row0"], q_len=pk["len"], nrows=M), Group(M, B, Lt, mask32, 0)])
            else:
                g2 = Batch([Group(0, 2 * B, Lt, torch.cat([mask32, mask32]), B)])
            y2, tape2, y2_32 = self.stack_fwd("text_encoder.bert.", ct, range(0, f), True, x2, g2, save, X32=x2_32)
            text_embeds, hidden10 = y2[:M], y2[M:]
            text_embeds_32, hidden10_32 = (y2_32[:M], y2_32[M:]) if r32 else (None, None)
        side_m = self._fork(1)
        ema_done = None
        with self._on(side_m):
            ops.ema_update(P.flat_m, P.flat, P.shadow_m, cfg.momentum)
            P.refresh_frag(True)
            if side_m is not None:
                ema_done = streams.mark(side_m)
            x4, _ = self.embed_text("text_encoder_m.bert.", ct, ids2, 2 * B, Lt, False)
            x4_32 = f32(x4)
            if pk:
                x4d = x4
                x4 = ops.gather_rows2(self._new(2 * M, H), x4d, pk["gidx4"])
                if r32:
                    x4_32 = torch.cat([x4_32[:B * Lt].index_select(0, pk["rows"]), x4_32[B * Lt:].index_select(0, pk["rows"])])
                g4 = Batch([g2.groups[0], Group(M, B, Lt, None, 0, q_row0=pk["row0"], q_len=pk["len"], nrows=M)])
            else:
                g4 = g2
            cls_m = bool(pk) and self.opt.cls_only_top and not r32 and f >= 1
            if cls_m:
                y4, _, _ = self.stack_fwd("text_encoder_m.bert.", ct, range(0, f - 1), True, x4, g4, False)
                x4t = ops.gather_rows2(self._new(B + M, H), y4, pk["idx_m"])
                g4t = Batch([Group(0, B, 1, None, B, self_src=SelfKV(y4[:M]), skv_row0=pk["row0"], skv_len=pk["len"], skv_L=Lt),
                             Group(B, B, Lt, None, 0, q_row0=pk["row0"], q_len=pk["len"], nrows=M)])
                y4t, _, _ = self._layer_fwd(f"text_encoder_m.bert.encoder.layer.{f - 1}.", ct, False, x4t, g4t, False)
                text_embeds_m, hidden9 = y4t[:B], y4t[B:]
            else:
                y4, _, y4_32 = self.stack_fwd("text_encoder_m.bert.", ct, range(0, f), True, x4, g4, False, X32=x4_32)
                text_embeds_m, hidden9 = y4[:M], y4[M:]
            text_embeds_m_32, hidden9_32 = (y4_32[:M], y4_32[M:]) if r32 else (None, None)
        x1, esv1 = self.embed_pv("property_encoder.", cp, prop, mpm_mask, 2 * B, B, save)
        g1 = Batch([Group(0, 2 * B, Lp, None, B)])
        y1, tape1, y1_32 = self.stack_fwd("property_encoder.", cp, range(cp.num_hidden_layers), False, x1, g1, save, X32=f32(x1))
        prop_embeds, prop_embeds_causal = y1[:B * Lp], y1[B * Lp:]
        prop_embeds_32, prop_embeds_causal_32 = (y1_32[:B * Lp], y1_32[B * Lp:]) if r32 else (None, None)
        if ema_done is not None:
            torch.cuda.current_stream().wait_event(ema_done)
        x3, _ = self.embed_pv("property_encoder_m.", cp, prop, mpm_mask, B, B, False)
# ... 274 lines not shown
```

Before: 2467 molecules/s.

## Project cross-attention K/V for all fusion layers in one segmented GEMM

Adds a segmented-weight GEMM, where each N-segment of output tiles selects its own weight and bias slice by stride, and uses it to compute cross-attention K/V projections for every fusion layer in a single launch before the stack runs. In backward, the per-layer input-gradient GEMMs for K/V are deferred and done once against a concatenated transposed weight, with segment sums and gathers writing into strided blocks. This cuts launch count and raises the GEMM's N for better occupancy. In exchange it needs more buffer memory, extra index arithmetic in the GEMM kernels, and is skipped when a layer-done callback is set.

Result: no change. 2466 molecules/s (-0.0%).

```diff
diff --git a/include/spmm_hip.h b/include/spmm_hip.h
--- a/include/spmm_hip.h
+++ b/include/spmm_hip.h
@@ -37,6 +37,10 @@
 int spmm_gemm_nt(const void* A, long lda, const void* W, long ldw, int M, int N, int K, int splits, const float* bias,
                  const float* div_ptr, float alpha, const void* R, long ldr, const void* G, long ldg, void* C, long ldc,
                  void* C2, long ldc2, int epi, float* colsum, int kernel, const int* M_dev, spmm_stream_t stream);
+int spmm_gemm_nt_seg(const void* A, long lda, const void* W, long ldw, int M, int N, int K, int splits, const float* bias,
+                     const float* div_ptr, float alpha, const void* R, long ldr, const void* G, long ldg, void* C, long ldc,
+                     void* C2, long ldc2, int epi, float* colsum, int kernel, const int* M_dev, int seg, long w_seg_stride,
+                     long b_seg_stride, spmm_stream_t stream);
 long spmm_gemm_tn_workspace_bytes(int M, int N, int K, int splits);
 int spmm_gemm_tn_splits(int M, int N, int K, int kernel);
 int spmm_gemm_tn(const void* A, long lda, const void* B, long ldb, int M, int N, int K, int splits, float alpha, float* C,
@@ -64,6 +68,8 @@
                    int nseq, int nH, int Lq, int Lkv, float attn_dropout_p, uint64_t salt_a, float hidden_dropout_p,
                    uint64_t salt_h, const uint64_t* seed_ptr, long row_base, spmm_stream_t stream);
 int spmm_segment_sum_bf16(const void* src, const int* start, const int* list, void* out, int U, long W, spmm_stream_t stream);
+int spmm_segment_sum_bf16_ld(const void* src, const int* start, const int* list, void* out, int U, long W, long rw, long ldo,
+                             spmm_stream_t stream);
 
 int spmm_ln_fwd(const void* x, const void* res, const float* gamma, const float* beta, void* y, void* zout, float* mean,
                 float* rstd, long rows, int H, float eps, float dropout_p, const uint64_t* seed_ptr, uint64_t salt,
@@ -134,6 +140,7 @@
 int spmm_acc_rows(float* dst, long ldd, const void* src, long lds, const long* idx, long rows, int H, int atomic,
                   spmm_stream_t stream);
 int spmm_gather_rows(void* dst, const void* src, const long* idx, long rows, int H, spmm_stream_t stream);
+int spmm_gather_rows_ld(void* dst, long ldd, const void* src, const long* idx, long rows, int H, spmm_stream_t stream);
 
 int spmm_gather_rows2(void* dst, const void* srcA, const void* srcB, const long* idx, long rows, int H, spmm_stream_t stream);
 int spmm_add_rows_bf16(void* dst, const long* idx, const void* src, long rows, int H, spmm_stream_t stream);
diff --git a/spmm_amd/csrc/gemm.hip b/spmm_amd/csrc/gemm.hip
--- a/spmm_amd/csrc/gemm.hip
+++ b/spmm_amd/csrc/gemm.hip
@@ -25,7 +25,20 @@
   float* colsum;
   int order;
   const int* M_ptr;
+  unsigned seg_magic;
+  unsigned w_delta_b32;
+  int b_delta32;
+  long w_delta, b_delta;
+  int nseg;
 };
+
+__device__ __forceinline__ long gemm_seg_of(const GemmP& p, int n0) { return (long)__umulhi((unsigned)n0 >> 7, p.seg_magic); }
+#define GEMM_SEG(P, N0)                                        \
+  do {                                                         \
+    const long s_ = gemm_seg_of((P), (N0));                    \
+    (P).W += s_ * (P).w_delta;                                 \
+    if ((P).bias) (P).bias += s_ * (P).b_delta;                \
+  } while (0)
 
 #define GEMM_DYN_M(P)                                          \
   do {                                                         \
@@ -257,6 +270,7 @@
   }
   const int tile_m = t / ntn, tile_n = t % ntn;
   const int m0 = tile_m * BM, n0 = tile_n * BN;
+  GEMM_SEG(p, n0);
   const int kbeg = blockIdx.z * p.ksplit;
   const int kend = min(p.K, kbeg + p.ksplit);
   const int nk = (kend - kbeg) / BK;
@@ -333,6 +347,7 @@
   }
   const int tile_m = t / ntn, tile_n = t % ntn;
   const int m0 = tile_m * BM, n0 = tile_n * BN;
+  GEMM_SEG(p, n0);
   const int kbeg = blockIdx.z * p.ksplit;
   const int kend = min(p.K, kbeg + p.ksplit);
   const int nk = (kend - kbeg) / BK;
@@ -473,6 +488,7 @@
   }
   const int tile_m = t / ntn, tile_n = t % ntn;
   const int m0 = tile_m * BM2, n0 = tile_n * BN;
+  GEMM_SEG(p, n0);
   const int nk = p.K / BK;
 
   f32x16 acc[2][2];
@@ -620,6 +636,7 @@
   int tile_m, tile_n;
   tile_of(t, ntm, ntn, p.order, tile_m, tile_n);
   const int m0 = tile_m * BM3, n0 = tile_n * BN3;
+  GEMM_SEG(p, n0);
   const int nk = p.K / BK;
 
   f32x16 acc[2][2][2];
@@ -907,6 +924,8 @@
     int tm_, tn_;                                                                                             \
     tile_of(t_, ntm, ntn, p.order, tm_, tn_);                                                                 \
     m0 = tm_ * BM3; n0 = tn_ * BN3;                                                                           \
+    uint32_t wd_ = 0;                                \
+    if constexpr (EPI == EPI_BF16) wd_ = __umulhi((uint32_t)n0 >> 7, p.seg_magic) * p.w_delta_b32;            \
     _Pragma("unroll") for (int h_ = 0; h_ < 2; ++h_)                                                          \
     _Pragma("unroll") for (int j_ = 0; j_ < 2; ++j_) {                                                        \
       int row_ = m0 + j_ * 128 + h_ * 64 + (tid >> 3);                                                        \
@@ -914,7 +933,7 @@
       offA[h_][j_] = (uint32_t)row_ * (uint32_t)(p.lda * 2) + ls16;                                                      \
       int col_ = n0 + (j_ * 2 + (tid >> 8)) * 64 + h_ * 32 + ((tid >> 3) & 31);                               \
       col_ = col_ < p.N ? col_ : p.N - 1;                                                                     \
-      offW[h_][j_] = (uint32_t)col_ * (uint32_t)(p.ldw * 2) + ls16;                                                      \
+      offW[h_][j_] = (uint32_t)col_ * (uint32_t)(p.ldw * 2) + ls16 + wd_;                                                \
     }                                                                                                         \
   } while (0)
   const char* gA = (const char*)p.A;
@@ -1063,6 +1082,9 @@
       int lane_e = lane;
       asm volatile("" : "+v"(lane_e));
       GemmP q = p;
+      if constexpr (EPI == EPI_BF16) {
+        if (q.bias) q.bias += (int)__umulhi((uint32_t)cn0 >> 7, q.seg_magic) * q.b_delta32;
+      }
       asm volatile("" : "+s"(q.C), "+s"(q.ldc), "+s"(q.C2), "+s"(q.ldc2));
       asm volatile("" : "+s"(q.R), "+s"(q.ldr), "+s"(q.G), "+s"(q.ldg));
       asm volatile("" : "+s"(q.bias), "+s"(q.colsum), "+s"(q.div_ptr), "+s"(q.alpha), "+s"(q.M), "+s"(q.N));
@@ -1216,9 +1238,12 @@
 }
 
 inline bool is_bf16_epi(int epi) { return epi_is_bf16(epi); }
+inline unsigned long w_span_bytes(const GemmP& p) {
+  return ((unsigned long)p.N * (unsigned long)p.ldw + (unsigned long)(p.nseg - 1) * (unsigned long)p.w_delta) * 2ul;
+}
 inline bool p8_ok(const GemmP& p, int epi) {
-  return is_bf16_epi(epi) && p.K % 128 == 0 && p.N % 8 == 0 && (unsigned long)p.M * (unsigned long)p.lda * 2ul < (1ul << 32) &&
-         (unsigned long)p.N * (unsigned long)p.ldw * 2ul < (1ul << 32);
+  return is_bf16_epi(epi) && p.K % 128 == 0 && p.N % 8 == 0 && (unsigned long)p.M * (unsigned long)p.lda * 2ul < (1ul << 32) && w_span_bytes(p) < (1ul << 32) &&
+         (p.nseg == 1 || epi == EPI_BF16);
 }
 
 int pick_tile(int M, int N, int epi) {
@@ -1240,10 +1265,11 @@
 
 }
 
-extern "C" int spmm_gemm_nt(const void* A, long lda, const void* W, long ldw, int M, int N, int K, int splits,
-                            const float* bias, const float* div_ptr, float alpha, const void* R, long ldr,
-                            const void* G, long ldg, void* C, long ldc, void* C2, long ldc2, int epi, float* colsum,
-                            int kernel, const int* M_dev, hipStream_t stream) {
+namespace {
+int gemm_nt_launch(const void* A, long lda, const void* W, long ldw, int M, int N, int K, int splits,
+                   const float* bias, const float* div_ptr, float alpha, const void* R, long ldr,
+                   const void* G, long ldg, void* C, long ldc, void* C2, long ldc2, int epi, float* colsum,
+                   int kernel, const int* M_dev, int seg, long w_seg_stride, long b_seg_stride, hipStream_t stream) {
   SPMM_CHECK_SHAPE(M > 0 && N > 0 && K > 0, "spmm_gemm_nt: empty problem M=%d N=%d K=%d", M, N, K);
   SPMM_CHECK_SHAPE(K % 64 == 0, "spmm_gemm_nt: K=%d must be a multiple of 64", K);
   SPMM_CHECK_SHAPE(N % 4 == 0, "spmm_gemm_nt: N=%d must be a multiple of 4", N);
@@ -1267,6 +1293,20 @@
   p.R = (const bf16*)R; p.ldr = ldr; p.G = (const bf16*)G; p.ldg = ldg; p.C = C; p.ldc = ldc;
   p.C2 = (bf16*)C2; p.ldc2 = ldc2; p.colsum = colsum;
   p.M_ptr = nullptr;
+  p.seg_magic = 0; p.w_delta = p.b_delta = 0; p.nseg = 1; p.w_delta_b32 = 0; p.b_delta32 = 0;
+  if (seg != 0) {
+    SPMM_CHECK_SHAPE(seg > 0 && seg % 256 == 0 && N % seg == 0, "spmm_gemm_nt_seg: seg=%d must be a multiple of 256 that divides N=%d", seg, N);
+    SPMM_CHECK_SHAPE(w_seg_stride >= (long)seg * ldw && w_seg_stride % 8 == 0 && (!bias || (b_seg_stride >= seg && b_seg_stride % 4 == 0)),
+                     "spmm_gemm_nt_seg: w_seg_stride=%ld (a multiple of 8, >= seg * ldw) / b_seg_stride=%ld (a multiple of 4, >= seg)", w_seg_stride, b_seg_stride);
+    SPMM_CHECK_SHAPE((unsigned long)(N / 128) * (unsigned long)(seg / 128) < (1ul << 32), "spmm_gemm_nt_seg: N=%d seg=%d out of range", N, seg);
+    p.seg_magic = (unsigned)(((1ul << 32) + (unsigned long)(seg / 128) - 1) / (unsigned long)(seg / 128));
+    p.w_delta = w_seg_stride - (long)seg * ldw;
+    p.b_delta = bias ? b_seg_stride - seg : 0;
+    p.nseg = N / seg;
+    p.w_delta_b32 = (unsigned)(p.w_delta * 2);
+    p.b_delta32 = (int)p.b_delta;
+    SPMM_CHECK_SHAPE((long)p.nseg * p.b_delta < (1l << 31), "spmm_gemm_nt_seg: b_seg_stride=%ld out of range", b_seg_stride);
+  }
   p.order = K > 1024 ? 0 : 2;
 
   int k = kernel == SPMM_GEMM_AUTO_TILES ? 0 : kernel;
@@ -1275,12 +1315,12 @@
     k = tile == 3 ? (p8_ok(p, epi) ? (kernel == SPMM_GEMM_AUTO_TILES ? 9 : 8) : 3) : tile;
     if (k == 2 && (epi == EPI_F32_ATOMIC || M < 512)) k = 1;
   }
-  const bool pc_fits = (unsigned long)p.M * (unsigned long)p.lda * 2ul < (1ul << 32) && (unsigned long)p.N * (unsigned long)p.ldw * 2ul < (1ul << 32);
+  const bool pc_fits = (unsigned long)p.M * (unsigned long)p.lda * 2ul < (1ul << 32) && w_span_bytes(p) < (1ul << 32);
   const long t128 = (long)((M + BM - 1) / BM) * ((N + BN - 1) / BN) * splits;
   if (k == 1 && kernel != 1 && pc_fits && PC_AUTO && t128 <= 256 && ksplit >= 4 * BK) k = 5;
   SPMM_CHECK_SHAPE(k == 1 || k == 2 || k == 3 || k == 5 || k == 8 || k == 9, "spmm_gemm_nt: unknown kernel selector %d", kernel);
   SPMM_CHECK_SHAPE(k != 5 || pc_fits, "spmm_gemm_nt: kernel 5 addresses its operands with 32-bit byte offsets (< 4 GiB each)");
-  SPMM_CHECK_SHAPE((k != 8 && k != 9) || p8_ok(p, epi), "spmm_gemm_nt: the 8-phase kernel needs a bf16-output epilogue, K %% 128 == 0, N %% 8 == 0 and operands < 4 GiB");
+  SPMM_CHECK_SHAPE((k != 8 && k != 9) || p8_ok(p, epi), "spmm_gemm_nt: the 8-phase kernel needs a bf16-output epilogue (the plain one with a segmented W), K %% 128 == 0, N %% 8 == 0 and operands < 4 GiB");
   SPMM_CHECK_SHAPE(k != 3 || is_bf16_epi(epi), "spmm_gemm_nt: the 256x256 kernel has bf16-output epilogues only");
   SPMM_CHECK_SHAPE(k != 2 || epi != EPI_F32_ATOMIC, "spmm_gemm_nt: the 256x128 kernel has no atomic epilogue");
   SPMM_CHECK_SHAPE(k == 1 || k == 5 || splits == 1, "spmm_gemm_nt: split-K runs on the 128x128 kernels only");
@@ -1296,3 +1336,20 @@
   SPMM_LAUNCH_CHECK("spmm_gemm_nt");
   return SPMM_OK;
 }
+}
+
+extern "C" int spmm_gemm_nt(const void* A, long lda, const void* W, long ldw, int M, int N, int K, int splits,
+                            const float* bias, const float* div_ptr, float alpha, const void* R, long ldr,
+                            const void* G, long ldg, void* C, long ldc, void* C2, long ldc2, int epi, float* colsum,
+                            int kernel, const int* M_dev, hipStream_t stream) {
+  return gemm_nt_launch(A, lda, W, ldw, M, N, K, splits, bias, div_ptr, alpha, R, ldr, G, ldg, C, ldc, C2, ldc2, epi, colsum, kernel, M_dev,
+                        0, 0, 0, stream);
+}
+
+extern "C" int spmm_gemm_nt_seg(const void* A, long lda, const void* W, long ldw, int M, int N, int K, int splits,
+                                const float* bias, const float* div_ptr, float alpha, const void* R, long ldr,
+                                const void* G, long ldg, void* C, long ldc, void* C2, long ldc2, int epi, float* colsum,
+                                int kernel, const int* M_dev, int seg, long w_seg_stride, long b_seg_stride, hipStream_t stream) {
+  return gemm_nt_launch(A, lda, W, ldw, M, N, K, splits, bias, div_ptr, alpha, R, ldr, G, ldg, C, ldc, C2, ldc2, epi, colsum, kernel, M_dev,
+                        seg, w_seg_stride, b_seg_stride, stream);
+}
diff --git a/spmm_amd/csrc/rowops.hip b/spmm_amd/csrc/rowops.hip
--- a/spmm_amd/csrc/rowops.hip
+++ b/spmm_amd/csrc/rowops.hip
@@ -566,7 +566,7 @@
   }
 }
 
-struct CtDesc { const float* src; bf16* dstT; int R, C; int tile0, ntc; };
+struct CtDesc { const float* src; bf16* dstT; int R, C; int tile0, ntc; long ldT; };
 __global__ __launch_bounds__(256) void cast_transpose_multi_kernel(const CtDesc* __restrict__ descs, int ndesc) {
   __shared__ bf16 tile[64][66];
   int lo = 0, hi = ndesc - 1;
@@ -587,7 +587,7 @@
 #pragma unroll
   for (int i = 0; i < 16; ++i) {
     const int c = c0 + ty * 16 + i, r = r0 + tx;
-    if (c < d.C && r < d.R) d.dstT[(long)c * d.R + r] = tile[tx][ty * 16 + i];
+    if (c < d.C && r < d.R) d.dstT[(long)c * d.ldT + r] = tile[tx][ty * 16 + i];
   }
 }
 
@@ -625,13 +625,13 @@
     }
   }
 }
-__global__ void gather_rows_kernel(bf16* __restrict__ dst, const bf16* __restrict__ src, const long* __restrict__ idx,
+__global__ void gather_rows_kernel(bf16* __restrict__ dst, long ldd, const bf16* __restrict__ src, const long* __restrict__ idx,
                                    long rows, int H) {
   const int h8 = H / 8;
   for (long i = (long)blockIdx.x * blockDim.x + threadIdx.x; i < rows * h8; i += (long)gridDim.x * blockDim.x) {
     const long r = i / h8;
     const int c = (int)(i - r * h8) * 8;
-    *(bf16x8*)(dst + r * H + c) = *(const bf16x8*)(src + idx[r] * H + c);
+    *(bf16x8*)(dst + r * ldd + c) = *(const bf16x8*)(src + idx[r] * H + c);
   }
 }
 
@@ -765,7 +765,8 @@
 
 namespace {
 __global__ __launch_bounds__(256) void segment_sum_kernel(const bf16* __restrict__ src, const int* __restrict__ start,
-                                                          const int* __restrict__ list, bf16* __restrict__ out, long W) {
+                                                          const int* __restrict__ list, bf16* __restrict__ out, long W, long rw,
+                                                          long ldo) {
   const int u = blockIdx.y;
   const long c = ((long)blockIdx.x * 256 + threadIdx.x) * 8;
   if (c >= W) return;
@@ -779,7 +780,8 @@
   bf16x8 o;
 #pragma unroll
   for (int e = 0; e < 8; ++e) o[e] = (bf16)acc[e];
-  *(bf16x8*)(out + (long)u * W + c) = o;
+  const long j = c / rw;
+  *(bf16x8*)(out + ((long)u * (W / rw) + j) * ldo + (c - j * rw)) = o;
 }
 }
 
@@ -787,8 +789,20 @@
   SPMM_CHECK_SHAPE(U > 0 && U <= 65535 && W > 0 && W % 8 == 0, "spmm_segment_sum_bf16: U=%d W=%ld (W %% 8 == 0)", U, W);
   SPMM_CHECK_SHAPE(src && start && list && out, "spmm_segment_sum_bf16: null src / start / list / out");
   hipLaunchKernelGGL(segment_sum_kernel, dim3((unsigned)((W / 8 + 255) / 256), U), dim3(256), 0, stream, (const bf16*)src, start, list,
-                     (bf16*)out, W);
+                     (bf16*)out, W, W, W);
   SPMM_LAUNCH_CHECK("spmm_segment_sum_bf16");
+  return SPMM_OK;
+}
+extern "C" int spmm_segment_sum_bf16_ld(const void* src, const int* start, const int* list, void* out, int U, long W, long rw, long ldo,
+                                        hipStream_t stream) {
+  SPMM_CHECK_SHAPE(U > 0 && U <= 65535 && W > 0 && W % 8 == 0, "spmm_segment_sum_bf16_ld: U=%d W=%ld (W %% 8 == 0)", U, W);
+  SPMM_CHECK_SHAPE(src && start && list && out, "spmm_segment_sum_bf16_ld: null src / start / list / out");
+  SPMM_CHECK_SHAPE(rw > 0 && rw % 8 == 0 && W % rw == 0 && ldo >= rw && ldo % 8 == 0 && (uintptr_t)out % 16 == 0,
+                   "spmm_segment_sum_bf16_ld: rw=%ld must be a multiple of 8 that divides W=%ld, ldo=%ld a multiple of 8 >= rw, out 16-byte aligned",
+                   rw, W, ldo);
+  hipLaunchKernelGGL(segment_sum_kernel, dim3((unsigned)((W / 8 + 255) / 256), U), dim3(256), 0, stream, (const bf16*)src, start, list,
+                     (bf16*)out, W, rw, ldo);
+  SPMM_LAUNCH_CHECK("spmm_segment_sum_bf16_ld");
   return SPMM_OK;
 }
 
@@ -847,8 +861,18 @@
 extern "C" int spmm_gather_rows(void* dst, const void* src, const long* idx, long rows, int H, hipStream_t stream) {
   SPMM_CHECK_SHAPE(rows > 0 && H > 0 && H % 8 == 0 && idx, "spmm_gather_rows: rows=%ld H=%d", rows, H);
   SPMM_CHECK_SHAPE(dst && src, "spmm_gather_rows: null dst / src");
-  hipLaunchKernelGGL(gather_rows_kernel, dim3(grid_for(rows * (H / 8), 256)), dim3(256), 0, stream, (bf16*)dst, (const bf16*)src,
+  hipLaunchKernelGGL(gather_rows_kernel, dim3(grid_for(rows * (H / 8), 256)), dim3(256), 0, stream, (bf16*)dst, (long)H,
+                     (const bf16*)src, idx, rows, H);
+  SPMM_LAUNCH_CHECK("spmm_gather_rows");
+  return SPMM_OK;
+}
+extern "C" int spmm_gather_rows_ld(void* dst, long ldd, const void* src, const long* idx, long rows, int H, hipStream_t stream) {
+  SPMM_CHECK_SHAPE(rows > 0 && H > 0 && H % 8 == 0 && idx, "spmm_gather_rows_ld: rows=%ld H=%d", rows, H);
+  SPMM_CHECK_SHAPE(dst && src, "spmm_gather_rows_ld: null dst / src");
+  SPMM_CHECK_SHAPE(ldd >= H && ldd % 8 == 0 && (uintptr_t)dst % 16 == 0,
+                   "spmm_gather_rows_ld: ldd=%ld must be a multiple of 8, at least H=%d, and dst 16-byte aligned", ldd, H);
+  hipLaunchKernelGGL(gather_rows_kernel, dim3(grid_for(rows * (H / 8), 256)), dim3(256), 0, stream, (bf16*)dst, ldd, (const bf16*)src,
                      idx, rows, H);
-  SPMM_LAUNCH_CHECK("spmm_gather_rows");
-  return SPMM_OK;
-}
+  SPMM_LAUNCH_CHECK("spmm_gather_rows_ld");
+  return SPMM_OK;
+}
diff --git a/spmm_amd/engine.py b/spmm_amd/engine.py
--- a/spmm_amd/engine.py
+++ b/spmm_amd/engine.py
@@ -29,6 +29,7 @@
         self._idx: List[torch.Tensor] = []
         self.nseq = 0
         self.start = self.list = None
+        self.defer = None
 
     def add(self, idx: torch.Tensor) -> int:
         off = self.nseq
@@ -48,6 +49,20 @@
         start[1:] = torch.cumsum(counts, 0)
         self.start, self.list = start, order.to(torch.int32)
         return self
+
+
+class DeferredKV:
+
+    def __init__(self, pfxs, buf, w):
+        self.pfxs, self.buf, self.w, self.written = pfxs, buf, w, set()
+
+    def block(self, pfx):
+        l = self.pfxs.index(pfx)
+        self.written.add(pfx)
+        return self.buf[:, l * self.w:(l + 1) * self.w]
+
+
+XKV_DGRAD_KERNEL = 0
 
 
 @dataclass
@@ -465,6 +480,30 @@
         if key not in done:
             done[key] = ops.gemm_nt(kv, Wkv, self._new(kv.shape[0], Wkv.shape[0]), bias=bkv)
         return done[key]
+
+    def xkv_project(self, pfxs, sources):
+        P, H, L = self.P, self.cfg.text.hidden_size, len(pfxs)
+        W0 = P.fused(pfxs[0] + ".self.", ("key", "value"), "weight")
+        b0 = P.fused(pfxs[0] + ".self.", ("key", "value"), "bias", what="w")
+        ws = P.fused_stride([p + ".self." for p in pfxs], ("key", "value"), "weight")
+        bs = P.fused_stride([p + ".self." for p in pfxs], ("key", "value"), "bias")
+        for src in sources:
+            KV = ops.gemm_nt_seg(src.kv, W0, self._new(src.kv.shape[0], L * 2 * H), nseg=L, w_seg_stride=ws, bias=b0, b_seg_stride=bs)
+            src.proj = {p: KV[:, l * 2 * H:(l + 1) * 2 * H] for l, p in enumerate(pfxs)}
+
+    def xkv_defer(self, pfxs, sources):
+        H = self.cfg.text.hidden_size
+        P = self.P
+        for src in sources:
+            src.defer = DeferredKV(list(pfxs), self._new(src.kv.shape[0], len(pfxs) * 2 * H), 2 * H)
+        return P.wT_cat(pfxs[0] + ".self.kv*", [(p + ".self.kv", P.fused(p + ".self.", ("key", "value"), "weight", what="w")) for p in pfxs])
+
+    def xkv_dgrad(self, WT, sources, dkv_acc):
+        for src in sources:
+            d, src.defer = src.defer, None
+            if len(d.written) != len(d.pfxs):
+                raise RuntimeError(f"deferred key/value gradient: blocks {sorted(set(d.pfxs) - d.written)} were never written")
+            ops.gemm_nt(d.buf, WT, dkv_acc[id(src)], epi=ops.EPI_F32_ACC, kernel=XKV_DGRAD_KERNEL)
 
     def _xattn_core_fwd(self, c, Qc, kv_of, groups, save, salts):
         H, nH = c.hidden_size, c.num_attention_heads
@@ -569,11 +608,17 @@
                     ops.gemm_nt(dKV, WkvT, dkv_acc[i], epi=ops.EPI_F32_ACC)
             for src, dKV in pool.values():
                 W = src.Lkv * 2 * H
-                dKVu = ops.segment_sum_bf16(dKV.view(src.nseq, W), src.start, src.list, self._new(src.U, W)).view(-1, 2 * H)
+                blk = None if src.defer is None else src.defer.block(pfx)
                 if src.pack_idx is not None:
-                    dKVu = ops.gather_rows(self._new(src.pack_idx.numel(), 2 * H), dKVu, src.pack_idx)
+                    dKVu = ops.segment_sum_bf16(dKV.view(src.nseq, W), src.start, src.list, self._new(src.U, W)).view(-1, 2 * H)
+                    dKVu = ops.gather_rows(self._new(src.pack_idx.numel(), 2 * H) if blk is None else blk, dKVu, src.pack_idx)
+                elif blk is None:
+                    dKVu = ops.segment_sum_bf16(dKV.view(src.nseq, W), src.start, src.list, self._new(src.U, W)).view(-1, 2 * H)
+                else:
+                    dKVu = ops.segment_sum_bf16_ld(dKV.view(src.nseq, W), src.start, src.list, blk)
                 self._wgrad(dKVu, src.kv, gWkv, gbkv)
-                ops.gemm_nt(dKVu, WkvT, dkv_acc[id(src)], epi=ops.EPI_F32_ACC)
+                if blk is None:
+                    ops.gemm_nt(dKVu, WkvT, dkv_acc[id(src)], epi=ops.EPI_F32_ACC)
             self._wgrad(dQc, X, P.g(pfx + ".self.query.weight"), P.g(pfx + ".self.query.bias"), md=md)
             ops.gemm_nt(dQc, self._wT(pfx + ".self.query", P.w(pfx + ".self.query.weight")), dX, R=dz, M_dev=md)
         return dX
diff --git a/spmm_amd/ops.py b/spmm_amd/ops.py
--- a/spmm_amd/ops.py
+++ b/spmm_amd/ops.py
@@ -93,6 +93,18 @@
     return C
 
 
+def gemm_nt_seg(A, W0, C, *, nseg, w_seg_stride, bias=None, b_seg_stride=0, kernel=0, M_dev=None):
+    if kernel == 0:
+        kernel = _nt_auto
+    M, K = A.shape
+    seg = W0.shape[0]
+    N = nseg * seg
+    assert A.dtype == BF16 and W0.dtype == BF16 and C.dtype == BF16 and W0.shape[1] == K and C.shape[0] >= M and C.shape[1] >= N
+    _call("spmm_gemm_nt_seg", _p(A), _row_stride(A), _p(W0), _row_stride(W0), M, N, K, 1, _p(bias), None, 1.0, None, 0, None, 0,
+          _p(C), _row_stride(C), None, 0, EPI_BF16, None, int(kernel), _p(M_dev), seg, int(w_seg_stride), int(b_seg_stride), _st())
+    return C
+
+
 def gemm_tn(A, B, C, *, alpha=1.0, splits=None, kernel=0, M_dev=None):
     M, N = A.shape
     K = B.shape[1]
@@ -225,7 +237,11 @@
 
 def gather_rows(dst, src, idx):
     rows, H = dst.shape
-    _call("spmm_gather_rows", _p(dst), _p(src), _p(idx), rows, H, _st())
+    if dst.is_contiguous():
+        _call("spmm_gather_rows", _p(dst), _p(src), _p(idx), rows, H, _st())
+    else:
+        assert src.is_contiguous() and src.shape[1] == H
+        _call("spmm_gather_rows_ld", _p(dst), _row_stride(dst), _p(src), _p(idx), rows, H, _st())
     return dst
 
 
@@ -621,6 +637,15 @@
     assert src.dtype == BF16 and out.dtype == BF16 and src.shape[1] == W and src.is_contiguous() and out.is_contiguous()
     assert start.dtype == torch.int32 and lst.dtype == torch.int32 and start.numel() == U + 1
     _call("spmm_segment_sum_bf16", _p(src), _p(start), _p(lst), _p(out), U, W, _st())
+    return out
+
+
+def segment_sum_bf16_ld(src, start, lst, out):
+    rows, rw = out.shape
+    U, W = start.numel() - 1, src.shape[1]
+    assert src.dtype == BF16 and out.dtype == BF16 and src.is_contiguous() and W % rw == 0 and rows == U * (W // rw)
+    assert start.dtype == torch.int32 and lst.dtype == torch.int32
+    _call("spmm_segment_sum_bf16_ld", _p(src), _p(start), _p(lst), _p(out), U, W, rw, _row_stride(out), _st())
     return out
 
 
diff --git a/spmm_amd/options.py b/spmm_amd/options.py
--- a/spmm_amd/options.py
+++ b/spmm_amd/options.py
@@ -11,6 +11,7 @@
     "wgrad_stream": ("SPMM_WGRAD_STREAM", lambda s: s != "0"),
     "pv_wgrad_inline": ("SPMM_PV_WGRAD_INLINE", int),
     "ln_from_y": ("SPMM_LN_FROM_Y", lambda s: s != "0"),
+    "xkv_once": ("SPMM_XKV_ONCE", lambda s: s != "0"),
     "resid_fp32": ("SPMM_RESID_FP32", lambda s: s == "1"),
     "fused_xattn": ("SPMM_FUSED_XATTN", lambda s: {"0": "off", "1": "all"}.get(s, s)),
     "grad_overlap": ("SPMM_GRAD_OVERLAP", lambda s: s != "0"),
@@ -31,6 +32,7 @@
     wgrad_stream: bool = True
     pv_wgrad_inline: int = 4
     ln_from_y: bool = True
+    xkv_once: bool = True
     fused_xattn: str = "nograd"
     resid_fp32: bool = False
     grad_overlap: bool = True
diff --git a/spmm_amd/params.py b/spmm_amd/params.py
--- a/spmm_amd/params.py
+++ b/spmm_amd/params.py
@@ -17,9 +17,10 @@
     for src, dstT in pairs:
         R, C = src.shape
         ntr, ntc = (R + 63) // 64, (C + 63) // 64
-        blob += struct.pack("<QQiiii", src.data_ptr(), dstT.data_ptr(), R, C, tile0, ntc)
+        assert tuple(dstT.shape) == (C, R) and (R == 1 or dstT.stride(1) == 1) and src.is_contiguous()
+        blob += struct.pack("<QQiiiiq", src.data_ptr(), dstT.data_ptr(), R, C, tile0, ntc, dstT.stride(0) if C > 1 else R)
         tile0 += ntr * ntc
-    assert len(blob) == len(pairs) * 32
+    assert len(blob) == len(pairs) * 40
     return blob, tile0
 
 
@@ -121,6 +122,13 @@
         full = (rows,) + tuple(shp[1:])
         return buf[self.offset[base]: self.offset[base] + int(math.prod(full))].view(full)
 
+    def fused_stride(self, prefixes, names, kind: str) -> int:
+        offs = [self.offset[self._resolve(f"{p}{names[0]}.{kind}")[1]] for p in prefixes]
+        strides = {b - a for a, b in zip(offs, offs[1:])}
+        rows = self.fused(prefixes[0], names, kind).numel()
+        assert len(strides) == 1 and min(strides) >= rows and min(strides) % ALIGN == 0, (prefixes, kind, offs)
+        return strides.pop()
+
     def wT(self, key: str, src: Optional[torch.Tensor] = None) -> torch.Tensor:
         if key not in self._wT:
             assert src is not None
@@ -129,6 +137,24 @@
             self._wT_src = getattr(self, "_wT_src", {})
             self._wT_src[key] = src
             ops.cast_transpose(src, None, self._wT[key])
+        return self._wT[key]
+
+    def wT_cat(self, key: str, parts) -> torch.Tensor:
+        if key not in self._wT:
+            C = parts[0][1].shape[1]
+            cat = torch.empty(C, sum(src.shape[0] for _, src in parts), dtype=torch.bfloat16, device=self.device)
+            self._wT_src = getattr(self, "_wT_src", {})
+            o, new = 0, []
+            for k, src in parts:
+                assert src.shape[1] == C
+                self._wT[k] = cat[:, o:o + src.shape[0]]
+                self._wT_src[k] = src
+                new.append((src, self._wT[k]))
+                o += src.shape[0]
+            self._wT[key] = cat
+            self._ct_n = -1
+            blob, tiles = ct_descriptor_table(new)
+            ops.cast_transpose_multi(torch.frombuffer(bytearray(blob), dtype=torch.uint8).to(self.device), len(new), tiles)
         return self._wT[key]
 
     def wT_padded(self, key: str, name: str, cols: int) -> torch.Tensor:
diff --git a/spmm_amd/step.py b/spmm_amd/step.py
--- a/spmm_amd/step.py
+++ b/spmm_amd/step.py
@@ -29,6 +29,8 @@
                       Group(o_12, B, Lp, None, 0).bind(src_text, ar, 3 * B),
                       Group(o_8, B, Lt, None, B, q_row0=fp["row0_8"], q_len=fp["len_8"], nrows=B * Lt).bind(src_pv, ar, 3 * B)],
                      rows_dev=fp["rows_dev"])
+        if self.opt.xkv_once and n - f >= 2:
+            self.xkv_project([f"text_encoder.bert.encoder.layer.{l}.crossattention" for l in range(f, n)], (src_text, src_pv))
         y, tape_lo, _ = self.stack_fwd("text_encoder.bert.", ct, range(f, n - 1), True, X6, g_lo, save)
         ntop = 6 * B + B * Lt + B * Lp
         Xtop = ops.gather_rows2(self._new(ntop, H), y, fp["idx_top"])
@@ -53,12 +55,19 @@
         dX6 = self._new(S6["Rcap"], H)
         S6["skv"][0].dx = dX6[:o_lm]
         S6["skv"][1].dx = dX6[o_8:]
+        srcs = (S6["src_text"], S6["src_pv"])
+        once = self.opt.xkv_once and self.layer_done_cb is None and n - f >= 2
+        if once:
+            WT = self.xkv_defer([f"text_encoder.bert.encoder.layer.{l}.crossattention" for l in range(f, n)], srcs)
         dXtop = self._layer_bwd(f"text_encoder.bert.encoder.layer.{n - 1}.", ct, S6["sv_top"], dYtop, S6["g_top"], dkv_acc)
         if self.layer_done_cb is not None:
             self._layer_done(f"text_encoder.bert.encoder.layer.{n - 1}.")
         ops.add_rows_bf16(dX6, fp["idx_top"][:6 * B], dXtop[:6 * B])
         dX6[o_lm:o_8].copy_(dXtop[6 * B:])
-        return self.stack_bwd("text_encoder.bert.", ct, range(f, n - 1), S6["tape_lo"], dX6, S6["g_lo"], dkv_acc=dkv_acc)
+        dX6 = self.stack_bwd("text_encoder.bert.", ct, range(f, n - 1), S6["tape_lo"], dX6, S6["g_lo"], dkv_acc=dkv_acc)
+        if once:
+            self.xkv_dgrad(WT, srcs, dkv_acc)
+        return dX6
 
     def forward(self, prop: torch.Tensor, ids: torch.Tensor, mask: torch.Tensor, *, mpm_mask: Optional[torch.Tensor] = None,
                 neg_idx: Optional[Tuple[torch.Tensor, torch.Tensor]] = None, gather: Optional[Callable] = None,
```
